# glgerard/MDBN

Measured on AMD Instinct MI355X. Metric: CD-k Gibbs steps/sec (samples/sec), GRBM 4096->1024 CD-1, higher is better.
Workload: dtype f32; 1 GPU; GRBM 4096->1024 CD-1, batch 512 per GPU, fp32, N(0,1) rows resident in HBM (BASELINE configs[1]); global_batch=512, k=1, n_data=32768, parallelism=dp1

## Files before the change

include/mdbn_hip.h:

```cpp
#ifndef MDBN_HIP_H
#define MDBN_HIP_H

#include <stddef.h>
#include <stdint.h>

#ifdef __cplusplus
extern "C" {
#endif

#define MDBN_OK       0
#define MDBN_EINVAL  (-1)
#define MDBN_EHIP    (-2)
#define MDBN_ENOSPC  (-3)

#define MDBN_VERSION 2

typedef struct mdbn_ctx mdbn_ctx;

typedef struct mdbn_rng {
    uint64_t seed;
    uint32_t stream_id;
    uint32_t step;
    uint32_t draw;
    uint32_t reserved;
    uint64_t row_offset;
} mdbn_rng;

typedef struct mdbn_cd_args {
    uint64_t     struct_size;
    const float *data;
    int64_t      n_data;
    const void  *indexes;
    int32_t      index_is_64;
    int32_t      gauss;
    int32_t      add_noise;
    int32_t      sample_stats;
    int32_t      keep_f32;
    int32_t      k;
    int64_t      B, V, H;
    int64_t      ldv, ldh;
    const float *W, *hbias, *vbias;
    float       *persistent;
    float       *V2;
    float       *P2;
    float       *hs;
    float       *vs;
    float       *stats;
    void        *workspace;
    int64_t      workspace_bytes;
    mdbn_rng     rng;
    float       *trace_h;
    float       *trace_v;
    void        *planes;
    int64_t      planes_bytes;
    void        *W_planes;
    int32_t      W_planes_valid;
    int32_t      comm_cus;
    const void  *next_indexes;
    void        *planes_alt;
    int32_t      x_buffer;
    int32_t      v0_ready;
    int32_t     *ahead_done;
} mdbn_cd_args;

typedef struct mdbn_update_args {
    uint64_t struct_size;
    float *W, *W_speed;
    const float *W0;
    float *hbias, *hbias_speed;
    float *vbias, *vbias_speed;
    int64_t V, H, ldv, ldh;
    const float *stats;
    float lr, lambda_1, lambda_2, weightcost, momentum;
    float batch_size;
    float n_rows;
    float cost_scale;
    float *cost_out;
    void *W_planes;
    int32_t phase;
    int32_t reserved;
} mdbn_update_args;

int  mdbn_version(void);
int  mdbn_last_error(char *buf, size_t n);
int  mdbn_source_hash(char *buf, size_t n);

int  mdbn_ctx_create(mdbn_ctx **out, int device);
int  mdbn_ctx_destroy(mdbn_ctx *ctx);

int  mdbn_bal_segment(int32_t tiles, int32_t stages, int32_t workgroups, int32_t w, int32_t k, int32_t *out);
int  mdbn_set_option(mdbn_ctx *ctx, const char *name, int64_t value);

int  mdbn_kernel_timing(mdbn_ctx *ctx, int enable);
int  mdbn_kernel_timing_read(mdbn_ctx *ctx, int64_t *n_launches, double *total_ms);
int  mdbn_kernel_timing_detail(mdbn_ctx *ctx, int64_t cap, double *ms, double *alg_flop,
                               double *pipe_flop, int32_t *kind, int64_t *n_launches);
int  mdbn_narrow_deep_launches(mdbn_ctx *ctx, int64_t *n_launches);

#define MDBN_MIN_WORKSPACE_BYTES 278528
int  mdbn_workspace_bytes(int64_t B, int64_t V, int64_t H, int64_t *bytes);
int  mdbn_workspace_bytes_ctx(mdbn_ctx *ctx, int64_t B, int64_t V, int64_t H, int64_t *bytes);
int  mdbn_workspace_bytes_ld(int64_t B, int64_t V, int64_t H, int64_t ldv, int64_t ldh, int64_t *bytes);
int  mdbn_workspace_bytes_ld_ctx(mdbn_ctx *ctx, int64_t B, int64_t V, int64_t H, int64_t ldv, int64_t ldh, int64_t *bytes);
int  mdbn_min_workspace_bytes(int64_t *bytes);
int  mdbn_padded_ld(int64_t cols, int64_t *ld);
int  mdbn_planes_bytes(int64_t B, int64_t ldv, int64_t ldh, int64_t *bytes);
int  mdbn_planes_alt_bytes(int64_t B, int64_t ldv, int64_t *bytes);
int  mdbn_ahead_bytes_ctx(mdbn_ctx *ctx, int64_t B, int64_t V, int64_t H, int64_t ldv, int64_t ldh, int64_t *bytes);
int  mdbn_planes_eligible(int64_t B, int64_t V, int64_t H, int64_t ldv, int64_t ldh, int32_t *eligible);
int  mdbn_planes_eligible_ctx(mdbn_ctx *ctx, int64_t B, int64_t V, int64_t H, int64_t ldv, int64_t ldh, int32_t *eligible);
int  mdbn_split_planes(mdbn_ctx *ctx, void *stream, const float *x, int64_t rows, int64_t ld, void *planes);
int  mdbn_stats_floats(int64_t V, int64_t ldv, int64_t ldh, int64_t *n);

int  mdbn_gather_rows(mdbn_ctx *ctx, void *stream, const float *src, int64_t n_rows,
                      int64_t cols, int64_t ld_src, const void *indexes, int index_is_64,
                      int64_t n_idx, float *dst, int64_t ld_dst);

int  mdbn_gather_rows_host(mdbn_ctx *ctx, void *stream, const float *src, int64_t n_rows,
                           int64_t cols, int64_t ld_src, const void *indexes, int index_is_64,
                           int64_t n_idx, float *dst, int64_t ld_dst, int workgroups, int threads);

int  mdbn_host_gather_rows(const float *table, int64_t n_rows, int64_t cols, int64_t ld,
                           const int64_t *indexes, int64_t n, float *out, int64_t ld_out, int threads);

typedef struct mdbn_feeder mdbn_feeder;
int  mdbn_feeder_create(mdbn_ctx *ctx, const float *table, int64_t n_rows, int64_t cols, int64_t ld,
                        int64_t max_rows, int slots, float *const *device_slots, int64_t ld_device,
                        int threads, mdbn_feeder **out);
int  mdbn_feeder_submit(mdbn_feeder *f, const int64_t *indexes, int64_t n, int64_t *ticket);
int  mdbn_feeder_acquire(mdbn_feeder *f, int64_t ticket, void *stream, int *slot);
int  mdbn_feeder_release(mdbn_feeder *f, int64_t ticket, void *stream);
int  mdbn_feeder_stats(mdbn_feeder *f, double *out5);
int  mdbn_feeder_cancel(mdbn_feeder *f);
int  mdbn_feeder_destroy(mdbn_feeder *f);

int  mdbn_propup_sample(mdbn_ctx *ctx, void *stream, const float *v, int64_t B, int64_t ldv,
                        const float *W, int64_t V, int64_t H, int64_t ldh, const float *hbias,
                        float *pre, float *mean, float mean_scale, float *sample,
                        const mdbn_rng *rng, void *workspace, int64_t workspace_bytes);

int  mdbn_propdown_sample(mdbn_ctx *ctx, void *stream, const float *h, int64_t B, int64_t ldh,
                          const float *W, int64_t V, int64_t H, int64_t ldv, const float *vbias,
                          int gauss, int add_noise, float *pre, float *mean, float *sample,
                          const mdbn_rng *rng, const float *v0, float *cost_sum,
                          void *workspace, int64_t workspace_bytes);

int  mdbn_comm_unique_id(char *id128);
int  mdbn_comm_init_rank(mdbn_ctx *ctx, const char *id128, int nranks, int rank);
int  mdbn_allreduce_stats(mdbn_ctx *ctx, void *stream, float *stats, int64_t n);
int  mdbn_comm_destroy(mdbn_ctx *ctx);

int  mdbn_gibbs_chain(mdbn_ctx *ctx, void *stream, float *v, int64_t B, int64_t ldv, const float *W,
                      int64_t V, int64_t H, int64_t ldh, const float *hbias, const float *vbias, int gauss,
                      int add_noise, int64_t n_steps, float *pre_h, float *h_mean, float *h_sample,
                      float *pre_v, float *v_mean, const mdbn_rng *rng, void *workspace,
                      int64_t workspace_bytes);

int  mdbn_cd_stats(mdbn_ctx *ctx, void *stream, const float *V2, const float *P2, int64_t B,
                   int64_t V, int64_t H, int64_t ldv, int64_t ldh, float *stats,
                   void *workspace, int64_t workspace_bytes);

int  mdbn_apply_update(mdbn_ctx *ctx, void *stream, const mdbn_update_args *a);

int  mdbn_cd_step(mdbn_ctx *ctx, void *stream, const mdbn_cd_args *a);

int  mdbn_cd_forward(mdbn_ctx *ctx, void *stream, const mdbn_cd_args *a);
int  mdbn_cd_statistics(mdbn_ctx *ctx, void *stream, const mdbn_cd_args *a, const mdbn_update_args *deferred);

int  mdbn_cd_train_step(mdbn_ctx *ctx, void *stream, const mdbn_cd_args *a,
                        const mdbn_update_args *upd);

int  mdbn_free_energy(mdbn_ctx *ctx, void *stream, const float *x, int64_t N, int64_t ldv,
                      const float *W, int64_t V, int64_t H, int64_t ldh, const float *hbias,
                      const float *vbias, int gauss, float *out,
                      void *workspace, int64_t workspace_bytes);

int  mdbn_ais_workspace_bytes(mdbn_ctx *ctx, int64_t M, int64_t V, int64_t H, int64_t n_betas, int path, int64_t *bytes);
int  mdbn_ais_run(mdbn_ctx *ctx, void *stream, const float *W, int64_t V, int64_t H, int64_t ldh,
                  const float *hbias, const float *vbias, const float *base_vbias, int gauss,
                  const float *betas, int64_t n_betas, int64_t M, int64_t ldv, float *v_state,
// ... 179 lines not shown
```

mdbn_amd/_lib.py:

```python
import ctypes as C
import os

HERE = os.path.dirname(os.path.abspath(__file__))
LIB_PATH = os.path.join(HERE, "libmdbn_hip.so")


class MdbnError(RuntimeError):
    pass


class Rng(C.Structure):
    _fields_ = [("seed", C.c_uint64), ("stream_id", C.c_uint32), ("step", C.c_uint32),
                ("draw", C.c_uint32), ("reserved", C.c_uint32), ("row_offset", C.c_uint64)]


class _Sized(C.Structure):

    def __init__(self, *a, **kw):
        super(_Sized, self).__init__(*a, **kw)
        self.struct_size = C.sizeof(type(self))


class CdArgs(_Sized):
    _fields_ = [("struct_size", C.c_uint64), ("data", C.c_void_p), ("n_data", C.c_int64), ("indexes", C.c_void_p),
                ("index_is_64", C.c_int32), ("gauss", C.c_int32), ("add_noise", C.c_int32),
                ("sample_stats", C.c_int32), ("keep_f32", C.c_int32), ("k", C.c_int32), ("B", C.c_int64), ("V", C.c_int64), ("H", C.c_int64),
                ("ldv", C.c_int64), ("ldh", C.c_int64),
                ("W", C.c_void_p), ("hbias", C.c_void_p), ("vbias", C.c_void_p),
                ("persistent", C.c_void_p),
                ("V2", C.c_void_p), ("P2", C.c_void_p), ("hs", C.c_void_p), ("vs", C.c_void_p),
                ("stats", C.c_void_p), ("workspace", C.c_void_p), ("workspace_bytes", C.c_int64),
                ("rng", Rng), ("trace_h", C.c_void_p), ("trace_v", C.c_void_p),
                ("planes", C.c_void_p), ("planes_bytes", C.c_int64), ("W_planes", C.c_void_p),
                ("W_planes_valid", C.c_int32), ("comm_cus", C.c_int32),
                ("next_indexes", C.c_void_p), ("planes_alt", C.c_void_p), ("x_buffer", C.c_int32),
                ("v0_ready", C.c_int32), ("ahead_done", C.POINTER(C.c_int32))]


class UpdateArgs(_Sized):
    _fields_ = [("struct_size", C.c_uint64), ("W", C.c_void_p), ("W_speed", C.c_void_p), ("W0", C.c_void_p),
                ("hbias", C.c_void_p), ("hbias_speed", C.c_void_p),
                ("vbias", C.c_void_p), ("vbias_speed", C.c_void_p),
                ("V", C.c_int64), ("H", C.c_int64), ("ldv", C.c_int64), ("ldh", C.c_int64),
                ("stats", C.c_void_p),
                ("lr", C.c_float), ("lambda_1", C.c_float), ("lambda_2", C.c_float),
                ("weightcost", C.c_float), ("momentum", C.c_float),
                ("batch_size", C.c_float), ("n_rows", C.c_float),
                ("cost_scale", C.c_float), ("cost_out", C.c_void_p), ("W_planes", C.c_void_p),
                ("phase", C.c_int32), ("reserved", C.c_int32)]


_i64, _i32, _f32, _vp = C.c_int64, C.c_int, C.c_float, C.c_void_p
_rngp = C.POINTER(Rng)

SIGNATURES = {
    "mdbn_version": [],
    "mdbn_last_error": [C.c_char_p, C.c_size_t],
    "mdbn_source_hash": [C.c_char_p, C.c_size_t],
    "mdbn_ctx_create": [C.POINTER(_vp), _i32],
    "mdbn_ctx_destroy": [_vp],
    "mdbn_set_option": [_vp, C.c_char_p, _i64],
    "mdbn_bal_segment": [_i32, _i32, _i32, _i32, _i32, C.POINTER(_i32)],
    "mdbn_kernel_timing": [_vp, _i32],
    "mdbn_kernel_timing_read": [_vp, C.POINTER(_i64), C.POINTER(C.c_double)],
    "mdbn_narrow_deep_launches": [_vp, C.POINTER(_i64)],
    "mdbn_kernel_timing_detail": [_vp, _i64, C.POINTER(C.c_double), C.POINTER(C.c_double),
                                  C.POINTER(C.c_double), C.POINTER(C.c_int32), C.POINTER(_i64)],
    "mdbn_workspace_bytes": [_i64, _i64, _i64, C.POINTER(_i64)],
    "mdbn_workspace_bytes_ctx": [_vp, _i64, _i64, _i64, C.POINTER(_i64)],
    "mdbn_workspace_bytes_ld": [_i64, _i64, _i64, _i64, _i64, C.POINTER(_i64)],
    "mdbn_workspace_bytes_ld_ctx": [_vp, _i64, _i64, _i64, _i64, _i64, C.POINTER(_i64)],
    "mdbn_min_workspace_bytes": [C.POINTER(_i64)],
    "mdbn_padded_ld": [_i64, C.POINTER(_i64)],
    "mdbn_planes_bytes": [_i64, _i64, _i64, C.POINTER(_i64)],
    "mdbn_planes_alt_bytes": [_i64, _i64, C.POINTER(_i64)],
    "mdbn_ahead_bytes_ctx": [_vp, _i64, _i64, _i64, _i64, _i64, C.POINTER(_i64)],
    "mdbn_planes_eligible": [_i64, _i64, _i64, _i64, _i64, C.POINTER(_i32)],
    "mdbn_planes_eligible_ctx": [_vp, _i64, _i64, _i64, _i64, _i64, C.POINTER(_i32)],
    "mdbn_split_planes": [_vp, _vp, _vp, _i64, _i64, _vp],
    "mdbn_stats_floats": [_i64, _i64, _i64, C.POINTER(_i64)],
    "mdbn_gather_rows": [_vp, _vp, _vp, _i64, _i64, _i64, _vp, _i32, _i64, _vp, _i64],
    "mdbn_gather_rows_host": [_vp, _vp, _vp, _i64, _i64, _i64, _vp, _i32, _i64, _vp, _i64, _i32, _i32],
    "mdbn_host_gather_rows": [_vp, _i64, _i64, _i64, _vp, _i64, _vp, _i64, _i32],
    "mdbn_feeder_create": [_vp, _vp, _i64, _i64, _i64, _i64, _i32, C.POINTER(_vp), _i64, _i32, C.POINTER(_vp)],
    "mdbn_feeder_submit": [_vp, _vp, _i64, C.POINTER(_i64)],
    "mdbn_feeder_acquire": [_vp, _i64, _vp, C.POINTER(_i32)],
    "mdbn_feeder_release": [_vp, _i64, _vp],
    "mdbn_feeder_stats": [_vp, C.POINTER(C.c_double)],
    "mdbn_feeder_cancel": [_vp],
    "mdbn_feeder_destroy": [_vp],
    "mdbn_propup_sample": [_vp, _vp, _vp, _i64, _i64, _vp, _i64, _i64, _i64, _vp,
                           _vp, _vp, _f32, _vp, _rngp, _vp, _i64],
    "mdbn_propdown_sample": [_vp, _vp, _vp, _i64, _i64, _vp, _i64, _i64, _i64, _vp, _i32, _i32,
                             _vp, _vp, _vp, _rngp, _vp, _vp, _vp, _i64],
    "mdbn_comm_unique_id": [C.c_char_p],
    "mdbn_comm_init_rank": [_vp, C.c_char_p, _i32, _i32],
    "mdbn_allreduce_stats": [_vp, _vp, _vp, _i64],
    "mdbn_comm_destroy": [_vp],
    "mdbn_gibbs_chain": [_vp, _vp, _vp, _i64, _i64, _vp, _i64, _i64, _i64, _vp, _vp, _i32, _i32, _i64,
                         _vp, _vp, _vp, _vp, _vp, _rngp, _vp, _i64],
    "mdbn_cd_stats": [_vp, _vp, _vp, _vp, _i64, _i64, _i64, _i64, _i64, _vp, _vp, _i64],
    "mdbn_apply_update": [_vp, _vp, C.POINTER(UpdateArgs)],
    "mdbn_cd_step": [_vp, _vp, C.POINTER(CdArgs)],
    "mdbn_cd_forward": [_vp, _vp, C.POINTER(CdArgs)],
    "mdbn_cd_statistics": [_vp, _vp, C.POINTER(CdArgs), C.POINTER(UpdateArgs)],
    "mdbn_cd_train_step": [_vp, _vp, C.POINTER(CdArgs), C.POINTER(UpdateArgs)],
    "mdbn_free_energy": [_vp, _vp, _vp, _i64, _i64, _vp, _i64, _i64, _i64, _vp, _vp, _i32, _vp,
                         _vp, _i64],
    "mdbn_ais_workspace_bytes": [_vp, _i64, _i64, _i64, _i64, _i32, C.POINTER(_i64)],
    "mdbn_ais_run": [_vp, _vp, _vp, _i64, _i64, _i64, _vp, _vp, _vp, _i32, _vp, _i64, _i64, _i64, _vp,
                     _vp, _vp, _vp, _i32, _rngp, _vp, _i64],
    "mdbn_ais_run_grouped": [_vp, _vp, _vp, _i64, _i64, _i64, _vp, _vp, _vp, _i32, _vp, _i64, _i64, _i64, _vp,
                             _vp, _vp, _vp, _i32, _rngp, _vp, _i64, _vp, _vp, _i64],
    "mdbn_ais_cond_workspace_bytes": [_vp, _i64, _i64, _i64, _i64, _i64, _i32, C.POINTER(_i64)],
    "mdbn_ais_cond_run": [_vp, _vp, _vp, _i64, _i64, _i64, _vp, _vp, _vp, _i32, _vp, _i64, _vp, _vp, _i64, _i64, _i64, _i64,
                          _vp, _vp, _vp, _vp, _i32, _rngp, _vp, _i64],
    "mdbn_ais_cond_run_grouped": [_vp, _vp, _vp, _i64, _i64, _i64, _vp, _vp, _vp, _vp, _i64, _vp, _vp, _i64, _i64, _i64, _i64,
                                  _vp, _vp, _vp, _vp, _i32, _rngp, _vp, _i64, _vp, _vp, _i64],
    "mdbn_gibbs_clamped_workspace_bytes": [_vp, _i64, _i64, _i64, _i32, C.POINTER(_i64)],
    "mdbn_gibbs_clamped": [_vp, _vp, _vp, _vp, _vp, _i64, _i64, _i64, _vp, _i64, _i64, _i64, _vp, _vp, _i32, _i32, _i64,
                           _i64, _vp, _vp, _vp, _vp, _vp, _vp, _vp, _i32, _i64, _rngp, _vp, _i64],
    "mdbn_gibbs_clamped_grouped": [_vp, _vp, _vp, _vp, _vp, _i64, _i64, _i64, _vp, _i64, _i64, _i64, _vp, _vp, _i64,
                                   _i64, _vp, _vp, _vp, _vp, _vp, _vp, _vp, _i32, _i64, _rngp, _vp, _i64, _vp, _vp, _i64],
    "mdbn_pt_workspace_bytes": [_vp, _i64, _i64, _i64, _i64, _i32, C.POINTER(_i64)],
    "mdbn_pt_run": [_vp, _vp, _vp, _i64, _i64, _i64, _vp, _vp, _vp, _i32, _vp, _i64, _i64, _i64, _vp, _vp, _vp,
                    _i64, _i64, _i64, _vp, _vp, _vp, _vp, _vp, _vp, _i32, _i64, _rngp, _vp, _i64],
    "mdbn_pt_run_z_workspace_bytes": [_vp, _i64, _i64, _i64, _i64, _i32, C.POINTER(_i64)],
    "mdbn_pt_run_z": [_vp, _vp, _vp, _i64, _i64, _i64, _vp, _vp, _vp, _i32, _vp, _i64, _i64, _i64, _vp, _vp, _vp,
                      _i64, _i64, _i64, _vp, _vp, _vp, _vp, _vp, _vp, _i32, _i64, _rngp, _vp, _i64, _vp, _vp],
    "mdbn_pt_run_grouped": [_vp, _vp, _vp, _i64, _i64, _i64, _vp, _vp, _vp, _i32, _vp, _i64, _i64, _i64, _vp, _vp, _vp,
                            _i64, _i64, _i64, _vp, _vp, _vp, _vp, _vp, _vp, _i32, _i64, _rngp, _vp, _i64, _vp, _vp,
                            _vp, _vp, _i64],
    "mdbn_rowll_workspace_bytes": [_vp, _i64, _i64, _i64, C.POINTER(_i64)],
    "mdbn_propdown_rowll": [_vp, _vp, _vp, _i64, _i64, _vp, _i64, _i64, _vp, _vp, _i64, _i64, _i32, _vp, _vp, _i64],
    "mdbn_rowll_grouped_workspace_bytes": [_vp, _i64, _i64, _i64, C.POINTER(_i64)],
    "mdbn_propdown_rowll_grouped": [_vp, _vp, _vp, _i64, _i64, _vp, _i64, _i64, _vp, _vp, _i64, _i64, _vp, _vp, _i64,
                                    _vp, _vp, _i64],
    "mdbn_sample_replicas": [_vp, _vp, _vp, _i64, _i64, _i64, _i64, _vp, _vp, _rngp],
    "mdbn_center_workspace_bytes": [_vp, _i64, _i64, C.POINTER(_i64)],
    "mdbn_center_offsets": [_vp, _vp, _vp, _i64, _vp, _i64, _i64, _i64, _i64, _f32, _vp, _vp],
    "mdbn_center_stats": [_vp, _vp, _vp, _i64, _i64, _i64, _i64, _vp, _vp, _f32, _vp, _i64],
    "mdbn_sparsity_activity": [_vp, _vp, _vp, _i64, _vp, _i64, _i64, _i64, _i64, _f32, _vp, _vp],
    "mdbn_sparsity_stats": [_vp, _vp, _vp, _i64, _i64, _i64, _i64, _vp, _vp, _f32, _f32, _f32],
    "mdbn_sigma_workspace_bytes": [_vp, _i64, _i64, C.POINTER(_i64)],
    "mdbn_sigma_scale_rows": [_vp, _vp, _vp, _i64, _i64, _vp, _i32, _i64, _i64, _vp, _f32, _vp, _i64],
    "mdbn_sigma_update": [_vp, _vp, _vp, _i64, _vp, _i64, _i64, _i64, _i64, _f32, _f32, _f32, _f32, _vp, _vp, _vp, _i64],
    "mdbn_group_softmax_workspace_bytes": [_vp, _i64, _i64, C.POINTER(_i64)],
    "mdbn_group_softmax_sample": [_vp, _vp, _vp, _i64, _i64, _i64, _vp, _vp, _i64, _vp, _vp, _vp, _rngp, _vp, _vp, _vp, _i64],
# ... 85 lines not shown
```

mdbn_amd/csrc/mdbn_capi.hip:

```cpp
#include <hip/hip_runtime.h>
#include <algorithm>
#include <cstdint>
#include <initializer_list>
#include <cstdarg>
#include <cstdio>
#include <cstdlib>
#include <cstring>
#include <string>
#include <utility>
#include <vector>
#include "mdbn_capi_internal.h"
#include "mdbn_kernels.h"
#include "mdbn_small.h"
#include "mdbn_thin.h"
#include "mdbn_gchain.h"

using namespace mdbn;
using namespace mdbn::capi;

static const Options g_default_options;
static GemmTiming g_no_timing;
static thread_local const Options* t_opt = &g_default_options;
static thread_local GemmTiming* t_timing = &g_no_timing;
#define g_timing (*t_timing)
// ... 26 lines not shown
#define g_opt_fused_finalize (t_opt->fused_finalize)
#define kMinSplitK (t_opt->min_splitk)

struct Plan {
    int tiles_m, tiles_n, splitk, kchunk, bn, bk;
    int skinny = 0;
    int mi = 1;
    int ni = 1;
    int cw = 1;
    int x6 = 0;
    int64_t slab_floats(int64_t M, int64_t ldc) const { return (int64_t)splitk * M * ldc; }
    void fill(GemmArgs& g) const
    {
        g.kchunk = kchunk; g.splitk = splitk; g.tiles_m = tiles_m; g.tiles_n = tiles_n; g.bn = bn; g.bk = bk;
        g.inner_m = tiles_m <= tiles_n;
        g.skinny = skinny; g.mi = mi; g.ni = ni; g.fused = 0; g.cw = cw; g.fin_enabled = 0; g.x6 = x6; g.x6_pw = g_opt_x6_pw;
    }
};

Plan plan_gemm(int64_t M, int64_t N, int64_t K)
{
    Plan p;
    p.tiles_m = (int)((M + 127) / 128);
    const int64_t t128 = (int64_t)p.tiles_m * ((N + 127) / 128);
    p.bn = (t128 * std::max<int64_t>(1, K / kMinSplitK) >= kTargetJobs) ? 128 : 64;
    p.tiles_n = (int)((N + p.bn - 1) / p.bn);
    const int64_t tiles = (int64_t)p.tiles_m * p.tiles_n;
    int64_t want = std::max<int64_t>(1, kTargetJobs / std::max<int64_t>(tiles, 1));
    int64_t maxsplit = std::max<int64_t>(1, K / kMinSplitK);
    int64_t sk = std::min(want, maxsplit);
    p.bk = (p.bn == 128 && g_opt_gemm_bk != 32 && (K + sk - 1) / sk >= 128) ? 64 : 32;
    int64_t kchunk = ((K + sk - 1) / sk + p.bk - 1) / p.bk * p.bk;
    if (kchunk < p.bk) kchunk = p.bk;
    sk = std::max<int64_t>(1, (K + kchunk - 1) / kchunk);
    p.splitk = (int)sk;
    p.kchunk = (int)kchunk;
    p.cw = g_opt_gemm_cw ? g_opt_gemm_cw : (p.bn == 128 && p.kchunk / p.bk <= 8 ? 2 : 1);
    return p;
}

#define g_opt_skinny_gemm (t_opt->skinny_gemm)
constexpr int kSkinnyTargetBlocks = 512;
constexpr int kSkinnyMinK = 256;
#define g_opt_skinny_fused_max_k (t_opt->skinny_fused_max_k)
#define g_opt_skinny_max_macs (t_opt->skinny_max_macs)

Plan plan_skinny(int64_t M, int64_t K, int64_t ldo, bool allow_split)
{
    Plan p;
    p.skinny = 1;
    p.mi = M <= 32 ? 1 : 2;
    p.tiles_m = (int)((M + 32 * p.mi - 1) / (32 * p.mi));
    p.tiles_n = (int)((ldo + 31) / 32);
    p.bn = 32; p.bk = 8;
    const int64_t blocks = (int64_t)p.tiles_m * p.tiles_n;
    const int64_t want = std::max<int64_t>(1, kSkinnyTargetBlocks / blocks);
    const bool one_launch = !allow_split || (K <= g_opt_skinny_fused_max_k && K <= 64 * blocks);
    const int64_t sk = one_launch ? 1 : std::min(want, std::max<int64_t>(1, K / kSkinnyMinK));
    int64_t kchunk = ((K + sk - 1) / sk + 63) / 64 * 64;
    p.kchunk = (int)kchunk;
    p.splitk = (int)std::max<int64_t>(1, (K + kchunk - 1) / kchunk);
    return p;
}

bool prefer_skinny(int64_t M, int64_t N, int64_t K)
{
    if (!g_opt_skinny_gemm) return false;
    if (M <= 64) return true;
    if (K > g_opt_skinny_fused_max_k) return false;
    const int64_t tiles_m = (M + 63) / 64, strips = (N + 31) / 32;
    if (K > 64 * tiles_m * strips) return false;
    return M * N * K <= (K <= 512 ? 3 : 1) * g_opt_skinny_max_macs;
}


#define g_opt_gemm_bf16x6 (t_opt->gemm_bf16x6)
#define g_opt_small_fused (t_opt->small_fused)
#define g_opt_thin_fused (t_opt->thin_fused)
#define g_opt_gchain (t_opt->gchain)
#define g_opt_gemm_planes (t_opt->gemm_planes)
#define g_opt_planes_mfma (t_opt->planes_mfma)
#define g_opt_early_w (t_opt->early_w)
#define g_opt_narrow_tiles (t_opt->narrow_tiles)
#define g_opt_slab_tail (t_opt->slab_tail)
#define g_opt_narrow_deep (t_opt->narrow_deep)
#define g_opt_feed_copy_streams (t_opt->feed_copy_streams)
#define g_opt_gather_ahead (t_opt->gather_ahead)
#define g_opt_bf16_inputs (t_opt->bf16_inputs)
#define g_opt_planes_min_work (t_opt->planes_min_work)
#define g_opt_comm_cus (t_opt->comm_cus)
#define g_opt_bal_blocks (t_opt->bal_blocks)
constexpr int kMaxBalBlocks = 256;

bool try_bf16x6(Plan& p, int64_t M, int64_t N, int64_t K, bool unsplit = false)
{
    if (p.skinny || K < 64) return false;
    const int64_t tm = (M + 127) / 128, tn = (N + 127) / 128, tiles = tm * tn;
    int64_t sk = 1;
    if (!unsplit) {
        sk = std::min(std::max<int64_t>(1, kTargetJobs / tiles), std::max<int64_t>(1, K / kMinSplitK));
    } else if (p.splitk != 1) {
        return false;
    }
    if (tiles * sk < g_opt_x6_min_jobs) return false;
    int64_t kchunk = ((K + sk - 1) / sk + 31) / 32 * 32;
    sk = (K + kchunk - 1) / kchunk;
    p.x6 = 1;
    p.bn = 128; p.bk = 32; p.cw = 1;
    p.tiles_m = (int)tm; p.tiles_n = (int)tn;
    p.splitk = (int)sk; p.kchunk = (int)kchunk;
    return true;
}

#define g_opt_stream_x6 (t_opt->stream_x6)
#define g_opt_stream_max_macs (t_opt->stream_max_macs)
#define g_opt_stream_mi (t_opt->stream_mi)
#define g_opt_stream_ni (t_opt->stream_ni)
constexpr int64_t kStreamMinTiles = 192;

bool stream_ok(int64_t M, int64_t N, int64_t K)
{
    return g_opt_stream_x6 && M > 64 && K >= 64 && M * N * K <= g_opt_stream_max_macs;
}

Plan plan_stream(int64_t M, int64_t K, int64_t ldo)
{
    Plan p = plan_skinny(M, K, ldo, false);
    const int64_t tiles32 = ((M + 31) / 32) * ((ldo + 31) / 32);
    p.mi = tiles32 >= 2 * kStreamMinTiles ? 2 : 1;
    p.ni = tiles32 >= 4 * kStreamMinTiles ? 2 : 1;
    if (g_opt_stream_mi) p.mi = g_opt_stream_mi;
    if (g_opt_stream_ni) p.ni = g_opt_stream_ni;
    if (p.ni == 2) p.mi = 2;
    p.tiles_m = (int)((M + 32 * p.mi - 1) / (32 * p.mi));
    p.x6 = 1;
    return p;
}

Plan plan_forward(int64_t M, int64_t N, int64_t K, int64_t ldo, bool stream = true)
{
    if (prefer_skinny(M, N, K)) {
        if (stream && g_opt_stream_x6 >= 2 && stream_ok(M, N, K)) return plan_stream(M, K, ldo);
        return plan_skinny(M, K, ldo, M <= 64);
    }
    if (stream && stream_ok(M, N, K)) return plan_stream(M, K, ldo);
    Plan p = plan_gemm(M, N, K);
    if (g_opt_gemm_bf16x6 & 2) try_bf16x6(p, M, N, K);
    return p;
}

Plan plan_stats(int64_t V, int64_t H, int64_t K2, int64_t ldh, bool stream = true)
{
    if (prefer_skinny(V, H, K2) && V > 64) {
        if (stream && g_opt_stream_x6 >= 2 && stream_ok(V, H, K2)) return plan_stream(V, K2, ldh);
        return plan_skinny(V, K2, ldh, false);
    }
    if (stream && stream_ok(V, H, K2)) return plan_stream(V, K2, ldh);
    Plan p = plan_gemm(V, H, K2);
    if (g_opt_gemm_bf16x6 & 1) try_bf16x6(p, V, H, K2, p.splitk == 1);
    return p;
}

static unsigned long long* g_stamps = nullptr;

template <class Launch>
hipError_t timed_launch(const GemmTiming::Meta& m, hipStream_t s, Launch launch)
// ... 46 lines not shown

static WsSizes ws_sizes_dense(int64_t B, int64_t V, int64_t H)
{
    const int64_t ldv = padded_ld(V), ldh = padded_ld(H);
    WsSizes s;
    const Plan up = plan_gemm(B, H, V), down = plan_gemm(B, V, H), st = plan_gemm(V, H, 2 * B);
    s.slab = std::max(up.slab_floats(B, ldh), down.slab_floats(B, ldv));
    {
        const Plan ups = plan_forward(B, H, V, ldh), downs = plan_forward(B, V, H, ldv);
        s.slab = std::max(s.slab, std::max(ups.slab_floats(B, ldh), downs.slab_floats(B, ldv)));
    }
    if (st.splitk > 1) s.slab = std::max(s.slab, st.slab_floats(V, ldh));
    {
        const Plan st2 = plan_stats(V, H, 2 * B, ldh);
        if (st2.splitk > 1) s.slab = std::max(s.slab, st2.slab_floats(V, ldh));
    }
    if (B % 128 == 0 && V % 128 == 0 && H % 128 == 0) {
        const int64_t tu = (B / 128) * (H / 128), td = (B / 128) * (V / 128);
        s.slab = std::max(s.slab, (kMaxBalBlocks / tu + 2) * B * ldh);
        s.slab = std::max(s.slab, (kMaxBalBlocks / td + 2) * B * ldv);
        s.slab = std::max<int64_t>(s.slab, (int64_t)kMaxBalBlocks * 2 * 16384);
    }
    if (small_shape_ok(B, V, H, 0) || small_shape_ok(B, V, H, 1))
        s.slab = std::max<int64_t>(s.slab, (int64_t)small_blocks(B) * ((V + 63) & ~int64_t(63)) * ldh);
    int64_t thin_cost = 0;
    {
        ThinGeom tg;
        if (thin_geom(B, V, H, ldv, ldh, kTargetJobs, tg)) {
            s.slab = std::max<int64_t>(s.slab, (int64_t)tg.G * tg.Bq * ldh);
            thin_cost = tg.G;
        }
    }
    int64_t gc_cost = 0;
    {
        GChainGeom gg;
        if (gchain_geom(B, V, H, ldv, ldh, 0, kTargetJobs, gg)) {
            s.slab = std::max<int64_t>(s.slab, gg.xbuf_floats);
            gc_cost = (int64_t)gg.nslab * gg.g;
        }
    }
    s.slab = std::max<int64_t>(s.slab, 4 * std::max(ldv, ldh) * 8);
    s.cost = cost_floats_for(B, std::max(ldv, ldh));
    if (small_shape_ok(B, V, H, 0) || small_shape_ok(B, V, H, 1)) s.cost = std::max<int64_t>(s.cost, (int64_t)small_blocks(B) * SM_NW + 64);
    s.cost = std::max<int64_t>(s.cost, thin_cost + 64);
    s.cost = std::max<int64_t>(s.cost, gc_cost + 64);
    const int ng = row_groups(B);
    s.colP = 2 * (int64_t)ng * ldh;
    s.colV = (int64_t)ng * ldv;
    return s;
}

WsSizes ws_sizes(int64_t B, int64_t V, int64_t H, int64_t ldv = 0, int64_t ldh = 0)
{
    WsSizes s = ws_sizes_dense(B, V, H);
    if (H % 128 != 0) {
        const WsSizes p = ws_sizes_dense(B, V, (H + 127) & ~int64_t(127));
        s.slab = std::max(s.slab, p.slab); s.cost = std::max(s.cost, p.cost);
        s.colP = std::max(s.colP, p.colP); s.colV = std::max(s.colV, p.colV);
    }
    const int64_t ng = row_groups(B);
    if (ldh > 0) {
        s.colP = std::max(s.colP, 2 * ng * ldh);
        const Plan st = plan_stats(V, H, 2 * B, ldh);
        if (st.splitk > 1) s.slab = std::max(s.slab, st.slab_floats(V, ldh));
    }
    if (ldv > 0) s.colV = std::max(s.colV, ng * ldv);
    if (ldv > 0 || ldh > 0) s.cost = std::max(s.cost, cost_floats_for(B, std::max(ldv, ldh)));
    return s;
}

hipError_t timed_gemm_planes(int la, int lb, const PlaneGemmArgs& g_in, hipStream_t s)
{
    PlaneGemmArgs g = g_in;
    g.stamps = g_stamps;
    g.ms = g_opt_planes_mfma;
    if (g_opt_bf16_inputs) g.ap = 0;
    g.slab_tail = g.slab_tail && g.ms == 16 && g.ap != 0;
    if (g.slab_tail && !slab_tail_ok(g, la, lb)) return hipErrorInvalidValue;
    const int pipe = g.ap == 3 ? 1 : (g.ap == 1 ? 2 : 3);
    return timed_launch(gemm_meta((g.bal ? 3000 : 2000) + 100 * pipe + 10 * g.fused + 2 * la + lb, pipe, g.M, g.N, g.K), s,
                        [&]() { return g.bal ? launch_gemm_planes_bal(la, lb, g, s) : launch_gemm_planes(la, lb, g, s); });
}

struct PlaneStep {
    unsigned short *Xp, *Pp, *hsp, *vsp;
    int64_t px, pp;
    unsigned short *Xother = nullptr, *Wp = nullptr;
    bool keep = false;
};
inline int64_t planes_elems(int64_t B, int64_t ldv, int64_t ldh) { return 6 * B * ldv + 6 * B * ldh + B * ldh + B * ldv; }

bool plane_plan(const Plan& p, int64_t M, int64_t N, int64_t K)
{
    return p.x6 && !p.skinny && M % 128 == 0 && N % 128 == 0 && p.kchunk % 32 == 0 && (int64_t)p.kchunk * p.splitk == K;
}

bool plane_shape_ok(int64_t B, int64_t V, int64_t H, int64_t ldv, int64_t ldh)
{
    if (!g_opt_gemm_planes) return false;
    if (B <= 0 || B % 128 || V % 128 || ldh % 128 || ldv != V || H > ldh || ldh - H >= 128 || B > 65535) return false;
    const int64_t He = ldh;
    if (g_opt_planes_min_work > 0 && (B * V * He < g_opt_planes_min_work || V * He < ((int64_t)1 << 21))) return false;
    return plane_plan(plan_forward(B, He, V, He, false), B, He, V) && plane_plan(plan_forward(B, V, He, V, false), B, V, He) &&
           plane_plan(plan_stats(V, He, 2 * B, He, false), V, He, 2 * B);
}

bool planes_eligible(const mdbn_cd_args* a)
{
    if (!a->planes || !a->W_planes) return false;
    if (a->persistent || a->sample_stats || (a->gauss && a->add_noise)) return false;
    const int64_t B = a->B, V = a->V, H = a->H;
    if (!plane_shape_ok(B, V, H, a->ldv, a->ldh)) return false;
    return a->planes_bytes >= 2 * planes_elems(B, a->ldv, a->ldh) && aligned16(a->planes) && aligned16(a->W_planes);
}

int bal_blocks(const mdbn_ctx* ctx, int comm_cus, int64_t tiles, int64_t stages)
{
    if (comm_cus <= 0) comm_cus = g_opt_comm_cus;
    if ((comm_cus <= 0 && g_opt_bal_blocks <= 0) || g_opt_planes_mfma != 16) return 0;
    int P = g_opt_bal_blocks > 0 ? g_opt_bal_blocks : std::min(ctx->num_cu - comm_cus, kMaxBalBlocks);
    if (P < 1) return 0;
    if (tiles < P && P % tiles != 0 && g_opt_bal_blocks <= 0) {
        const int aligned = (int)(tiles * (P / tiles));
        if (4ll * P <= 5ll * aligned) P = aligned;
    }
    return tiles * stages >= 4 * (int64_t)P ? P : 0;
}

int run_affine_planes(mdbn_ctx* ctx, int comm_cus, const unsigned short* A, int64_t lda, int64_t pa, int ap, int dir,
                      const unsigned short* Wp, int64_t V, int64_t H, int64_t ncols, int64_t rows, EpiArgs e, bool want_cost,
                      const Workspace& ws, hipStream_t s, int* n_cost_out)
{
    const int64_t Kdim = dir == 0 ? V : H, Ndim = dir == 0 ? H : V;
    PlaneGemmArgs g{};
    g.A = A; g.lda = lda; g.pa = pa; g.ap = ap;
    g.B = Wp; g.ldb = H; g.pb = V * H;
    g.M = (int)rows; g.N = (int)Ndim; g.K = (int)Kdim;
    g.tiles_m = (int)(rows / 128); g.tiles_n = (int)(Ndim / 128);
    {
        const Plan p = plan_forward(rows, Ndim, Kdim, e.ld, false);
        g.splitk = p.splitk; g.kchunk = p.kchunk;
    }
    int bal = bal_blocks(ctx, comm_cus, (int64_t)g.tiles_m * g.tiles_n, Kdim / 32), bal_slabs = 0;
    if (bal) {
        bal_slabs = bal_max_segments(g.tiles_m * g.tiles_n, (int)(Kdim / 32), bal);
        if ((int64_t)bal_slabs * rows * e.ld > ws.slab_floats) bal = 0;
        if ((int64_t)bal_slabs * rows * e.ld * 4 >= (int64_t)1 << 31) bal = 0;
    }
    if (!bal && g_opt_narrow_tiles && g_opt_fused_epilogue && dir == 1 && g.splitk == 2 && Ndim % 64 == 0 && g_opt_planes_mfma == 16 &&
        !g_opt_bf16_inputs && (ap == 1 || ap == 3) && (int64_t)g.tiles_m * (Ndim / 64) <= 2 * ctx->num_cu &&
        (!e.target || (e.ld_target % 4 == 0 && ((uintptr_t)e.target & 15) == 0))) {
        g.bn = 64; g.tiles_n = (int)(Ndim / 64); g.splitk = 1; g.kchunk = (int)Kdim;
        g.fused = 1; g.ms = 16;
        g.deep = g_opt_narrow_deep && narrow_deep_ok(g, LAY_K, LAY_K);
        if (g.deep) ++ctx->narrow_deep_launches;
    }
    const bool fuse = !bal && g_opt_fused_epilogue && g.splitk == 1;
    const int nb = fuse ? g.tiles_m * g.tiles_n : epilogue_blocks(rows, e.ld);
    e.rows = (int)rows; e.cols = (int)ncols;
    e.cost_partials = nullptr;
    if (want_cost) {
        if (nb > ws.cost_floats) return fail(MDBN_ENOSPC, "cost scratch exhausted");
        e.cost_partials = ws.cost_partials;
        if (n_cost_out) *n_cost_out = nb;
    }
    const int lb = dir == 0 ? LAY_MN : LAY_K;
    if (bal) {
        g.bal = bal; g.fused = 0; g.C = ws.slabs; g.ldc = e.ld; g.slab_stride = rows * e.ld;
        g.xcd_group = bal >= 4 * g.tiles_m * g.tiles_n ? 0 : 1;
        g.splitk = 1; g.kchunk = (int)Kdim; g.c_bytes = (int64_t)bal_slabs * rows * e.ld * 4;
        e.slabs = ws.slabs; e.slab_stride = g.slab_stride; e.nsplit = bal_slabs;
        e.bal_P = bal; e.bal_S = (int)(Kdim / 32); e.bal_tiles_m = g.tiles_m; e.bal_tiles_n = g.tiles_n;
        {
            const int tiles = g.tiles_m * g.tiles_n;
            bool uniform = true;
            for (int t = 0; t < tiles && uniform; ++t) uniform = bal_tile_slabs(t, tiles, e.bal_S, bal) == bal_slabs;
            if (uniform) e.bal_P = 0;
        }
        HIP_OK(timed_gemm_planes(LAY_K, lb, g, s));
        HIP_OK(launch_act_epilogue(e, s));
    } else if (fuse) {
        g.fused = 1; g.epi = e;
        HIP_OK(timed_gemm_planes(LAY_K, lb, g, s));
    } else {
        REQUIRE((int64_t)g.splitk * rows * e.ld <= ws.slab_floats, "internal: plane GEMM slabs exceed the workspace");
        g.fused = 0; g.C = ws.slabs; g.ldc = e.ld; g.slab_stride = rows * e.ld;
        e.slabs = ws.slabs; e.slab_stride = g.slab_stride; e.nsplit = g.splitk;
        g.slab_tail = g_opt_slab_tail && dir == 0;
        HIP_OK(timed_gemm_planes(LAY_K, lb, g, s));
        HIP_OK(launch_act_epilogue(e, s));
    }
    return MDBN_OK;
}

enum class StepPart { Whole, Forward, Statistics };

struct StatsView {
    float *S, *s_h, *s_v, *cost;
    StatsView(float* stats, int64_t V, int64_t ldv, int64_t ldh) : S(stats), s_h(S + V * ldh), s_v(s_h + ldh), cost(s_v + ldv) {}
};

bool plain_cd(const mdbn_cd_args* a) { return !a->persistent && !a->sample_stats && !(a->gauss && a->add_noise); }
bool keeps_f32(const mdbn_cd_args* a) { return a->keep_f32 != 0 || a->trace_h != nullptr || a->trace_v != nullptr; }

hipError_t launch_whole_update(const mdbn_update_args& u, hipStream_t s)
{
    return launch_update(u, s, nullptr, 1, 0, reinterpret_cast<unsigned short*>(u.W_planes));
}
mdbn_update_args whole_rule(const mdbn_update_args& u) { mdbn_update_args w = u; w.phase = 0; return w; }

int planes_setup(const mdbn_cd_args* a, PlaneStep& pb)
{
    const int64_t B = a->B, ldv = a->V, ldh = a->ldh;
    unsigned short* q = reinterpret_cast<unsigned short*>(a->planes);
    pb.Xp = q; pb.px = 2 * B * ldv; q += 6 * B * ldv;
    pb.Pp = q; pb.pp = 2 * B * ldh; q += 6 * B * ldh;
    pb.hsp = q; q += B * ldh;
    pb.vsp = q;
    if (a->planes_alt) {
        REQUIRE(aligned16(a->planes_alt), "planes_alt not 16-byte aligned");
        unsigned short* alt = reinterpret_cast<unsigned short*>(a->planes_alt);
        if (a->x_buffer) { pb.Xother = pb.Xp; pb.Xp = alt; } else pb.Xother = alt;
    } else {
        REQUIRE(a->x_buffer == 0, "x_buffer = 1 needs planes_alt");
    }
    pb.Wp = reinterpret_cast<unsigned short*>(a->W_planes);
    pb.keep = keeps_f32(a);
    return MDBN_OK;
}

int planes_forward(mdbn_ctx* ctx, hipStream_t s, const mdbn_cd_args* a, const Workspace& ws, const PlaneStep& pb, int* n_cost)
{
    const int64_t B = a->B, V = a->V, Hlive = a->H, ldv = V, ldh = a->ldh;
    const int64_t H = ldh;
    unsigned short* const Wp = pb.Wp;  const bool keep = pb.keep;
    float *v0 = a->V2, *nv = a->V2 + B * ldv, *ph = a->P2, *nh = a->P2 + B * ldh;
    if (!(a->v0_ready && !keep))
        HIP_OK(launch_gather_planes(a->data, a->n_data, ldv, ldv, a->indexes, a->index_is_64, B, keep ? v0 : nullptr, ldv, pb.Xp,
                                    pb.px, s));

    auto key = [&](uint32_t draw) { PhiloxKey k = make_key(a->rng, draw); return k; };
    {
        EpiArgs e{};
        e.ld = ldh; e.bias = a->hbias; e.mean = keep ? ph : nullptr; e.sample = keep ? a->hs : nullptr; e.mean_scale = 1.0f; e.gauss = 0;
        e.colsum = ws.colPpos; e.colsum_kind = 0; e.rng = key(0);
        e.mean_planes = pb.Pp; e.plane_stride = pb.pp; e.sample_plane = pb.hsp;
        CHECK(run_affine_planes(ctx, a->comm_cus, pb.Xp, ldv, pb.px, 3, 0, Wp, V, H, Hlive, B, e, false, ws, s, nullptr));
        if (a->trace_h) HIP_OK(hipMemcpyAsync(a->trace_h, a->hs, sizeof(float) * B * ldh, hipMemcpyDeviceToDevice, s));
    }
    for (int t = 1; t <= a->k; ++t) {
        const bool last = t == a->k;
        {
            EpiArgs e{};
            e.ld = ldv; e.bias = a->vbias; e.mean = keep ? nv : nullptr; e.mean_scale = 1.0f; e.gauss = a->gauss;
            e.sample = (a->gauss || !keep) ? nullptr : a->vs; e.rng = key((uint32_t)(2 * t - 1));
            e.mean_planes = pb.Xp + B * ldv; e.plane_stride = pb.px;
            e.sample_plane = a->gauss ? nullptr : pb.vsp;
            if (last) {
                e.colsum = ws.colV; e.colsum_kind = 1;
                if (keep) { e.target = v0; e.ld_target = ldv; }
                else {
                    e.target = a->data; e.ld_target = ldv; e.target_rows = a->n_data;
                    e.target_idx = a->indexes; e.target_idx64 = a->index_is_64;
                }
            }
            CHECK(run_affine_planes(ctx, a->comm_cus, pb.hsp, ldh, B * ldh, 1, 1, Wp, V, H, V, B, e, last, ws, s, last ? n_cost : nullptr));
            if (a->trace_v && !a->gauss)
                HIP_OK(hipMemcpyAsync(a->trace_v + (int64_t)(t - 1) * B * ldv, a->vs, sizeof(float) * B * ldv,
                                      hipMemcpyDeviceToDevice, s));
        }
        {
            const bool need_sample = !last;
            EpiArgs e{};
            e.ld = ldh; e.bias = a->hbias; e.mean = keep ? nh : nullptr; e.mean_scale = -1.0f; e.gauss = 0;
            e.sample = (need_sample && keep) ? a->hs : nullptr; e.rng = key((uint32_t)(2 * t));
            e.mean_planes = pb.Pp + B * ldh; e.plane_stride = pb.pp;
            e.sample_plane = need_sample ? pb.hsp : nullptr;
            if (last) { e.colsum = ws.colPneg; e.colsum_kind = 0; }
            if (a->gauss) CHECK(run_affine_planes(ctx, a->comm_cus, pb.Xp + B * ldv, ldv, pb.px, 3, 0, Wp, V, H, Hlive, B, e, false, ws, s, nullptr));
            else CHECK(run_affine_planes(ctx, a->comm_cus, pb.vsp, ldv, B * ldv, 1, 0, Wp, V, H, Hlive, B, e, false, ws, s, nullptr));
            if (a->trace_h && need_sample)
                HIP_OK(hipMemcpyAsync(a->trace_h + (int64_t)t * B * ldh, a->hs, sizeof(float) * B * ldh, hipMemcpyDeviceToDevice, s));
        }
    }
    return MDBN_OK;
}

int planes_statistics(mdbn_ctx* ctx, hipStream_t s, const mdbn_cd_args* a, const Workspace& ws, const PlaneStep& pb, int n_cost,
                      const mdbn_update_args* upd, const mdbn_update_args* defer)
{
    const int64_t B = a->B, V = a->V, Hlive = a->H, ldv = V, ldh = a->ldh, H = ldh;
    const StatsView st(a->stats, V, ldv, ldh);
    const Plan sp = plan_stats(V, H, 2 * B, ldh, false);
    PlaneGemmArgs g{};
    g.A = pb.Xp; g.lda = ldv; g.pa = pb.px; g.ap = 3;
    g.B = pb.Pp; g.ldb = ldh; g.pb = pb.pp;
    g.M = (int)V; g.N = (int)H; g.K = (int)(2 * B);
    g.tiles_m = (int)(V / 128); g.tiles_n = (int)(H / 128); g.splitk = sp.splitk; g.kchunk = sp.kchunk;
    g.fin_enabled = 0;
    int bal = sp.splitk == 1 ? bal_blocks(ctx, a->comm_cus, (int64_t)g.tiles_m * g.tiles_n, 2 * B / 32) : 0;
    if (bal && ((int64_t)bal * 2 * 16384 > ws.slab_floats || V * ldh * 4 >= (int64_t)1 << 31)) bal = 0;
    const bool fuse_upd = !bal && upd != nullptr && g_opt_fused_update && sp.splitk == 1;
    auto set_gather_ahead = [&]() {
        if (g.upd.early && g_opt_gather_ahead && a->next_indexes && pb.Xother && !pb.keep) {
            const int nwg = g.tiles_m * g.tiles_n, nt = (int)(2 * B / 32);
            const int rpw = (int)((B + nwg - 1) / nwg), passes = (int)((ldv / 8 + 255) / 256);
            if (rpw * passes <= 4 && 16 / (nt >= 20 ? 1 : 2) + 4 + 1 <= nt - 3) {
                g.ga.src = a->data; g.ga.n_rows = a->n_data; g.ga.ld_src = ldv;
                g.ga.idx = a->next_indexes; g.ga.idx64 = a->index_is_64;
                g.ga.B = (int)B; g.ga.rpw = rpw; g.ga.passes = passes;
                g.ga.P = pb.Xother; g.ga.plane_stride = pb.px; g.ga.ld = ldv;
                if (a->ahead_done) *a->ahead_done = 1;
            }
        }
    };
    if (fuse_upd) {
        BiasUpd bu;
        fill_bias_upd(bu, *upd, Hlive);
        g.fused = 2;
        g.fin_enabled = 1;
        g.fin = make_fin_args(ws.colPpos, ws.colPneg, ws.colV, row_groups(B), ldh, ldv, ws.cost_partials, n_cost, st.s_h, st.s_v,
                              st.cost, &bu);
        fill_upd(g.upd, *upd, V, ldh, pb.Wp);
        g.upd.early = g_opt_early_w && upd->lambda_1 == 0.f && (upd->weightcost == 0.f || upd->W0 != nullptr) &&
                      2 * B / 32 >= 12 && g_opt_planes_mfma == 16 && !g_opt_bf16_inputs;
        g.stats_tail = g_opt_slab_tail && g.upd.early == 1 && ldh < ((int64_t)1 << 21);
        set_gather_ahead();
        HIP_OK(timed_gemm_planes(LAY_MN, LAY_MN, g, s));
        return MDBN_OK;
    }
    if (sp.splitk == 1 && g_opt_fused_finalize) {
        g.fin_enabled = 1;
        g.fin = make_fin_args(ws.colPpos, ws.colPneg, ws.colV, row_groups(B), ldh, ldv, ws.cost_partials, n_cost, st.s_h, st.s_v,
                              st.cost, nullptr);
    } else {
        HIP_OK(launch_finalize_stats(ws.colPpos, ws.colPneg, ws.colV, row_groups(B), ldh, ldv, ws.cost_partials, n_cost, st.s_h,
                                     st.s_v, st.cost, nullptr, s));
    }
    g.fused = 0; g.ldc = ldh; g.slab_stride = V * ldh;
    if (defer) {
        const bool splitphase = g_opt_early_w && g_opt_planes_mfma == 16 && !g_opt_bf16_inputs && defer->phase == 3 &&
                                defer->lambda_1 == 0.f && (defer->weightcost == 0.f || defer->W0 != nullptr) &&
                                defer->stats != a->stats;
        const int64_t flat = bal ? (((V * ldh / 4 + bal - 1) / bal + 511) / 512) * 512 : 0;
        const bool inside = splitphase && (bal ? (flat <= 16 * 512 && (int64_t)g.tiles_m * g.tiles_n * (2 * B / 32) / bal >= 20)
                                               : (sp.splitk == 1 && 2 * B / 32 >= 20));
        g.upd.flat_per_wg = flat;
        if (inside) {
            fill_upd(g.upd, *defer, V, ldh, reinterpret_cast<unsigned short*>(defer->W_planes));
            g.upd.l1 = 0.f; g.upd.Sprev = defer->stats; g.upd.early = 2;
            const StatsView prev(const_cast<float*>(defer->stats), V, ldv, ldh);
            DeferredBias& d = g.db;
            d.on = 1; d.hb = defer->hbias; d.hbs = defer->hbias_speed; d.vb = defer->vbias; d.vbs = defer->vbias_speed;
            d.s_h = prev.s_h; d.s_v = prev.s_v; d.cost_sum = prev.cost; d.H = Hlive; d.V = V;
            d.lr = defer->lr; d.mu = defer->momentum; d.inv_rows = 1.0f / defer->n_rows;
            d.cost_scale = defer->cost_scale; d.cost_out = defer->cost_out;
            if (!bal) set_gather_ahead();
        } else {
            HIP_OK(launch_whole_update(*defer, s));
        }
    }
    if (bal) {
        g.xcd_group = 1;
        g.C = st.S; g.bal = bal; g.fused = 4; g.kchunk = (int)(2 * B); g.c_bytes = V * ldh * 4;
        g.scratch = ws.slabs;
        HIP_OK(timed_gemm_planes(LAY_MN, LAY_MN, g, s));
    } else if (sp.splitk == 1) {
        g.C = st.S;
        HIP_OK(timed_gemm_planes(LAY_MN, LAY_MN, g, s));
    } else {
        REQUIRE(sp.slab_floats(V, ldh) <= ws.slab_floats, "internal: statistic slabs exceed workspace");
        g.C = ws.slabs;
        HIP_OK(timed_gemm_planes(LAY_MN, LAY_MN, g, s));
        if (upd && g_opt_fused_update) {
            HIP_OK(launch_update(whole_rule(*upd), s, ws.slabs, sp.splitk, g.slab_stride, pb.Wp));
            return MDBN_OK;
        }
        HIP_OK(launch_sum_slabs(ws.slabs, sp.splitk, g.slab_stride, V * ldh, st.S, s));
    }
    if (upd) HIP_OK(launch_update(whole_rule(*upd), s, nullptr, 1, 0, pb.Wp));
    return MDBN_OK;
}

}

namespace mdbn {
namespace capi {

int fail(int code, const char* fmt, ...)
{
    char buf[512];
    va_list ap;
    va_start(ap, fmt);
    vsnprintf(buf, sizeof buf, fmt, ap);
    va_end(ap);
    g_err = buf;
    return code;
}

PhiloxKey make_key(const mdbn_rng& r, uint32_t draw)
{
    PhiloxKey k;
    k.k0 = (uint32_t)r.seed;
    k.k1 = (uint32_t)(r.seed >> 32) ^ r.stream_id;
    k.step = r.step;
    k.draw = draw;
    k.row_offset = r.row_offset;
    return k;
}

int64_t dense_workspace_bytes(int64_t B, int64_t V, int64_t H) { return ws_sizes(B, V, H).total_bytes(); }

constexpr int64_t kPropCostFloats = 1 << 16;
constexpr int64_t kPropMinBytes = 4 * (kPropCostFloats + 4096);
static_assert(kPropMinBytes == MDBN_MIN_WORKSPACE_BYTES, "mdbn_hip.h states the minimum of the propagation calls");

int carve(void* ws, int64_t bytes, int64_t B, int64_t V, int64_t H, Workspace& out, bool need_stats, int64_t ldv, int64_t ldh)
{
    REQUIRE(ws != nullptr && aligned16(ws), "workspace must be a 16-byte aligned device pointer");
    const WsSizes s = ws_sizes(B, V, H, ldv, ldh);
// ... 105 lines not shown
    e.mu = u.momentum; e.inv_bs = 1.0f / u.batch_size;
    e.Wp = Wp; e.wp_stride = V * ldh;
}

void fill_bias_upd(BiasUpd& b, const mdbn_update_args& u, int64_t H)
{
    b.hb = u.hbias; b.hbs = u.hbias_speed; b.vb = u.vbias; b.vbs = u.vbias_speed;
    b.H = H; b.V = u.V; b.lr = u.lr; b.mu = u.momentum; b.inv_rows = 1.0f / u.n_rows;
    b.cost_scale = u.cost_scale; b.cost_out = u.cost_out;
}

}
}

extern "C" {

int mdbn_version(void) { return MDBN_VERSION; }

#ifndef MDBN_SRC_HASH
#define MDBN_SRC_HASH "unknown"
#endif
static const char mdbn_source_hash_tag[] __attribute__((used)) = "MDBN_SOURCE_HASH_TAG=" MDBN_SRC_HASH;
int mdbn_source_hash(char* buf, size_t n)
{
    if (!buf || n == 0) return MDBN_EINVAL;
    snprintf(buf, n, "%s", mdbn_source_hash_tag + sizeof("MDBN_SOURCE_HASH_TAG=") - 1);
    return MDBN_OK;
}

int mdbn_last_error(char* buf, size_t n)
{
    if (!buf || n == 0) return MDBN_EINVAL;
    snprintf(buf, n, "%s", g_err.c_str());
    return MDBN_OK;
}

int mdbn_ctx_create(mdbn_ctx** out, int device)
{
    REQUIRE(out != nullptr, "out is NULL");
    int count = 0;
    HIP_OK(hipGetDeviceCount(&count));
    REQUIRE(device >= 0 && device < count, "device %d out of range (%d visible)", device, count);
    hipDeviceProp_t prop;
    HIP_OK(hipGetDeviceProperties(&prop, device));
    if (strncmp(prop.gcnArchName, "gfx950", 6) != 0)
        return fail(MDBN_EHIP, "device %d is %s; this library is built for gfx950 only", device, prop.gcnArchName);
    mdbn_ctx* c = new mdbn_ctx;
    c->device = device;
    c->num_cu = prop.multiProcessorCount;
    if (const char* e = getenv("MDBN_NARROW_DEEP")) c->opt.narrow_deep = atoi(e) != 0;
    *out = c;
    return MDBN_OK;
}

int mdbn_ctx_destroy(mdbn_ctx* ctx)
{
    CtxScope ctx_scope(ctx);
    if (ctx) {
        if (ctx->ev_fork) (void)hipEventDestroy(ctx->ev_fork);
        if (ctx->ev_join) (void)hipEventDestroy(ctx->ev_join);
        if (ctx->side) (void)hipStreamDestroy(ctx->side);
        if (ctx->comm) (void)mdbn_comm_destroy(ctx);
        if (ctx->gc_flags) (void)hipFree(ctx->gc_flags);
    }
    delete ctx;
    return MDBN_OK;
}

#ifdef MDBN_STAMP
int mdbn_debug_set_stamps(void* p) { g_stamps = (unsigned long long*)p; return MDBN_OK; }
#endif

int mdbn_bal_segment(int32_t tiles, int32_t stages, int32_t workgroups, int32_t w, int32_t k, int32_t* out)
{
    REQUIRE(out != nullptr, "out is NULL");
    int tile, s0, s1, nseg, nt;
    if (bal_segment_host(tiles, stages, workgroups, w, k, &tile, &s0, &s1, &nseg, &nt) != 0)
        return fail(MDBN_EINVAL, "bad arguments");
    out[0] = tile; out[1] = s0; out[2] = s1; out[3] = nseg; out[4] = nt;
    out[5] = tile >= 0 ? bal_tile_slabs(tile, tiles, stages, workgroups) : 0;
    return MDBN_OK;
}

static bool set_plane_kernel_option(mdbn_ctx* ctx, const char* name, int64_t value)
{
    if (strcmp(name, "slab_tail") == 0) {
        ctx->opt.slab_tail = value != 0;
        return true;
    }
    return false;
}

int mdbn_set_option(mdbn_ctx* ctx, const char* name, int64_t value)
{
    CtxScope ctx_scope(ctx);
    REQUIRE(ctx != nullptr && name != nullptr, "NULL argument");
    if (set_plane_kernel_option(ctx, name, value)) return MDBN_OK;
    if (strcmp(name, "gemm_bk") == 0) {
        REQUIRE(value == 0 || value == 32 || value == 64, "gemm_bk must be 0 (auto), 32 or 64");
        ctx->opt.gemm_bk = (int)value;
        return MDBN_OK;
    }
    if (strcmp(name, "epilogue_threads") == 0) {
        if (value != 0 && value != 64 && value != 128 && value != 256) return fail(MDBN_EINVAL, "epilogue_threads must be 0, 64, 128 or 256");
        ctx->opt.epilogue_threads = (int)value;
        return MDBN_OK;
    }
    if (strcmp(name, "epilogue_cw") == 0) {
        REQUIRE(value == 0 || value == 1 || value == 2 || value == 4, "epilogue_cw must be 0 (auto), 1, 2 or 4");
        ctx->opt.epilogue_cw = (int)value;
        return MDBN_OK;
    }
    if (strcmp(name, "skinny_gemm") == 0) {
        ctx->opt.skinny_gemm = value != 0;
        return MDBN_OK;
    }
    if (strcmp(name, "thin_fused") == 0) {
        ctx->opt.thin_fused = value != 0;
        return MDBN_OK;
    }
    if (strcmp(name, "gchain") == 0) {
        ctx->opt.gchain = value != 0;
        return MDBN_OK;
    }
    if (strcmp(name, "skinny_fused_max_k") == 0) {
        REQUIRE(value >= 0 && value <= INT32_MAX, "skinny_fused_max_k must be in [0, 2^31)");
        ctx->opt.skinny_fused_max_k = (int)value;
        return MDBN_OK;
    }
    if (strcmp(name, "x6_min_jobs") == 0) {
        REQUIRE(value >= 0 && value <= INT32_MAX, "x6_min_jobs must be in [0, 2^31)");
        ctx->opt.x6_min_jobs = (int)value;
        return MDBN_OK;
    }
    if (strcmp(name, "x6_producer_waves") == 0) {
        if (value != 2 && value != 4) return fail(MDBN_EINVAL, "x6_producer_waves must be 2 or 4");
        ctx->opt.x6_pw = (int)value;
        return MDBN_OK;
    }
    if (strcmp(name, "gemm_min_splitk") == 0) {
        if (value < 32 || value > INT32_MAX) return fail(MDBN_EINVAL, "gemm_min_splitk must be in [32, 2^31)");
        ctx->opt.min_splitk = (int)value;
        return MDBN_OK;
    }
    if (strcmp(name, "gemm_cw") == 0) {
        if (value < 0 || value > 2) return fail(MDBN_EINVAL, "gemm_cw must be 0 (auto), 1 or 2");
        ctx->opt.gemm_cw = (int)value;
        return MDBN_OK;
    }
    if (strcmp(name, "stream_x6") == 0) {
        REQUIRE(value == 0 || value == 1 || value == 2, "stream_x6 must be 0, 1 or 2");
        ctx->opt.stream_x6 = (int)value;
        return MDBN_OK;
    }
    if (strcmp(name, "stream_max_macs") == 0) {
        REQUIRE(value >= 0, "stream_max_macs must be >= 0");
        ctx->opt.stream_max_macs = value;
        return MDBN_OK;
    }
    if (strcmp(name, "stream_mi") == 0) {
        REQUIRE(value == 0 || value == 1 || value == 2, "stream_mi must be 0, 1 or 2");
        ctx->opt.stream_mi = (int)value;
        return MDBN_OK;
    }
    if (strcmp(name, "stream_ni") == 0) {
        REQUIRE(value == 0 || value == 1 || value == 2, "stream_ni must be 0, 1 or 2");
        ctx->opt.stream_ni = (int)value;
        return MDBN_OK;
    }
    if (strcmp(name, "skinny_max_macs") == 0) {
        REQUIRE(value >= 0 && value < ((int64_t)1 << 61), "skinny_max_macs must be in [0, 2^61)");
        ctx->opt.skinny_max_macs = value;
        return MDBN_OK;
    }
    if (strcmp(name, "gemm_bf16x6") == 0) {
        REQUIRE(value >= 0 && value <= 3, "gemm_bf16x6 must be in 0..3 (bit 0 statistics, bit 1 forward passes)");
        ctx->opt.gemm_bf16x6 = (int)value;
        return MDBN_OK;
    }
    if (strcmp(name, "planes_min_work") == 0) {
// ... 2 lines not shown
        return MDBN_OK;
    }
    if (strcmp(name, "bf16_inputs") == 0) {
        ctx->opt.bf16_inputs = value != 0;
        return MDBN_OK;
    }
    if (strcmp(name, "planes_mfma") == 0) {
        if (value != 16 && value != 32) return fail(MDBN_EINVAL, "planes_mfma must be 16 or 32");
        ctx->opt.planes_mfma = (int)value;
        return MDBN_OK;
    }
    if (strcmp(name, "narrow_tiles") == 0) {
        ctx->opt.narrow_tiles = value != 0;
        return MDBN_OK;
    }
    if (strcmp(name, "feed_copy_streams") == 0) {
        REQUIRE(value == 1 || value == 2, "feed_copy_streams must be 1 or 2");
        ctx->opt.feed_copy_streams = value;
        return MDBN_OK;
    }
    if (strcmp(name, "gather_ahead") == 0) {
        ctx->opt.gather_ahead = value != 0;
        return MDBN_OK;
    }
    if (strcmp(name, "early_w") == 0) {
        ctx->opt.early_w = value != 0;
        return MDBN_OK;
    }
    if (strcmp(name, "bal_blocks") == 0) {
        if (value < 0 || value > kMaxBalBlocks) return fail(MDBN_EINVAL, "bal_blocks must be in [0, %d]", kMaxBalBlocks);
        ctx->opt.bal_blocks = (int)value;
        return MDBN_OK;
    }
    if (strcmp(name, "comm_cus") == 0) {
        if (value < 0 || value > 192) return fail(MDBN_EINVAL, "comm_cus must be in [0, 192]");
        ctx->opt.comm_cus = (int)value;
        return MDBN_OK;
    }
    if (strcmp(name, "small_fin_lanes") == 0) {
        REQUIRE(value == 0 || value == 1 || value == 2 || value == 4 || value == 8 || value == 16, "small_fin_lanes must be 0, 1, 2, 4, 8 or 16");
        ctx->opt.small_fin_lanes = (int)value;
        return MDBN_OK;
    }
    if (strcmp(name, "small_fused") == 0) {
        ctx->opt.small_fused = value != 0;
        return MDBN_OK;
    }
    if (strcmp(name, "gemm_planes") == 0) {
        ctx->opt.gemm_planes = value != 0;
        return MDBN_OK;
    }
    if (strcmp(name, "fused_finalize") == 0) {
        ctx->opt.fused_finalize = value != 0;
        return MDBN_OK;
    }
    if (strcmp(name, "fused_update") == 0) {
        ctx->opt.fused_update = value != 0;
        return MDBN_OK;
    }
    if (strcmp(name, "fused_epilogue") == 0) {
        ctx->opt.fused_epilogue = value != 0;
        return MDBN_OK;
    }
    if (strcmp(name, "update_overlap") == 0) {
        ctx->opt.update_overlap = value != 0;
        return MDBN_OK;
    }
    return fail(MDBN_EINVAL, "unknown option %s", name);
}

int mdbn_kernel_timing(mdbn_ctx* ctx, int enable)
{
    CtxScope ctx_scope(ctx);
    REQUIRE(ctx != nullptr, "ctx is NULL");
    g_timing.enabled = enable != 0;
    g_timing.used = 0;
    return MDBN_OK;
}

int mdbn_narrow_deep_launches(mdbn_ctx* ctx, int64_t* n_launches)
{
    REQUIRE(ctx && n_launches, "NULL argument");
    *n_launches = ctx->narrow_deep_launches;
    return MDBN_OK;
}

int mdbn_kernel_timing_read(mdbn_ctx* ctx, int64_t* n_launches, double* total_ms)
{
    CtxScope ctx_scope(ctx);
    REQUIRE(ctx && n_launches && total_ms, "NULL argument");
    double tot = 0.0;
    for (size_t i = 0; i < g_timing.used; ++i) {
        HIP_OK(hipEventSynchronize(g_timing.pool[i].second));
        float ms = 0.f;
        HIP_OK(hipEventElapsedTime(&ms, g_timing.pool[i].first, g_timing.pool[i].second));
        tot += ms;
    }
    *n_launches = (int64_t)g_timing.used;
    *total_ms = tot;
    return MDBN_OK;
}

int mdbn_kernel_timing_detail(mdbn_ctx* ctx, int64_t cap, double* ms, double* alg_flop, double* pipe_flop,
                              int32_t* kind, int64_t* n_launches)
{
    CtxScope ctx_scope(ctx);
    REQUIRE(ctx && n_launches && (cap == 0 || (ms && alg_flop && pipe_flop && kind)), "NULL argument");
    const int64_t n = std::min<int64_t>(cap, (int64_t)g_timing.used);
    for (int64_t i = 0; i < n; ++i) {
        HIP_OK(hipEventSynchronize(g_timing.pool[i].second));
        float t = 0.f;
        HIP_OK(hipEventElapsedTime(&t, g_timing.pool[i].first, g_timing.pool[i].second));
        ms[i] = t;
        alg_flop[i] = g_timing.meta[i].alg_flop;
        pipe_flop[i] = g_timing.meta[i].pipe_flop;
        kind[i] = g_timing.meta[i].kind;
    }
    *n_launches = (int64_t)g_timing.used;
    return MDBN_OK;
}

int mdbn_workspace_bytes(int64_t B, int64_t V, int64_t H, int64_t* bytes)
{
    REQUIRE(bytes != nullptr && B > 0 && V > 0 && H > 0, "bad arguments");
    *bytes = std::max(ws_sizes(B, V, H).total_bytes(), kPropMinBytes);
    return MDBN_OK;
}

int mdbn_workspace_bytes_ld(int64_t B, int64_t V, int64_t H, int64_t ldv, int64_t ldh, int64_t* bytes)
{
    REQUIRE(bytes != nullptr && B > 0 && V > 0 && H > 0, "bad arguments");
    REQUIRE(ldv >= V && ldh >= H && ldv % 4 == 0 && ldh % 4 == 0, "leading dims must be multiples of 4, >= V / H");
    *bytes = std::max(ws_sizes(B, V, H, ldv, ldh).total_bytes(), kPropMinBytes);
    return MDBN_OK;
}

int mdbn_min_workspace_bytes(int64_t* bytes)
{
    REQUIRE(bytes != nullptr, "bytes is NULL");
    *bytes = kPropMinBytes;
    return MDBN_OK;
}

int mdbn_workspace_bytes_ld_ctx(mdbn_ctx* ctx, int64_t B, int64_t V, int64_t H, int64_t ldv, int64_t ldh, int64_t* bytes)
{
    CtxScope ctx_scope(ctx);
    REQUIRE(ctx != nullptr, "ctx is NULL");
    return mdbn_workspace_bytes_ld(B, V, H, ldv, ldh, bytes);
}

int mdbn_workspace_bytes_ctx(mdbn_ctx* ctx, int64_t B, int64_t V, int64_t H, int64_t* bytes)
{
    CtxScope ctx_scope(ctx);
    REQUIRE(ctx != nullptr, "ctx is NULL");
    return mdbn_workspace_bytes(B, V, H, bytes);
}

int mdbn_padded_ld(int64_t cols, int64_t* ld)
{
    REQUIRE(ld != nullptr && cols > 0, "bad arguments");
    *ld = padded_ld(cols);
    return MDBN_OK;
}

int mdbn_planes_bytes(int64_t B, int64_t ldv, int64_t ldh, int64_t* bytes)
{
// ... 495 lines not shown
    const bool fuse_upd = upd && !overlap && g_opt_fused_update && p.splitk == 1;
    BiasUpd bu;
    if (fuse_upd) fill_bias_upd(bu, u, H);
    const bool fin_in_gemm = !overlap && g_opt_fused_finalize;
    if (!overlap && !fin_in_gemm)
        HIP_OK(launch_finalize_stats(ws.colPpos, ws.colPneg, ws.colV, row_groups(B), ldh, ldv, ws.cost_partials,
                                     n_cost, st.s_h, st.s_v, st.cost, fuse_upd ? &bu : nullptr, s));
    GemmArgs g{};
    g.A = a->V2; g.lda = ldv; g.B = a->P2; g.ldb = ldh;
    g.ldc = ldh; g.slab_stride = V * ldh;
    g.M = (int)V; g.N = (int)H; g.K = (int)(2 * B); g.Nst = (int)ldh;
    p.fill(g);
    g.fin_enabled = fin_in_gemm;
    if (fin_in_gemm)
        g.fin = make_fin_args(ws.colPpos, ws.colPneg, ws.colV, row_groups(B), ldh, ldv, ws.cost_partials, n_cost,
                              st.s_h, st.s_v, st.cost, fuse_upd ? &bu : nullptr);
    if (fuse_upd) {
        g.C = nullptr;
        g.fused = 2;
        fill_upd(g.upd, u, V, ldh, reinterpret_cast<unsigned short*>(u.W_planes));
        HIP_OK(timed_gemm(LAY_MN, LAY_MN, g, s));
        return MDBN_OK;
    }
    if (p.splitk == 1) {
        g.C = st.S;
        HIP_OK(timed_gemm(LAY_MN, LAY_MN, g, s));
    } else {
        REQUIRE(p.slab_floats(V, ldh) <= ws.slab_floats, "internal: statistic slabs exceed workspace");
        g.C = ws.slabs;
        HIP_OK(timed_gemm(LAY_MN, LAY_MN, g, s));
        if (upd && !overlap && g_opt_fused_update) {
            HIP_OK(launch_update(whole_rule(u), s, ws.slabs, p.splitk, g.slab_stride, reinterpret_cast<unsigned short*>(u.W_planes)));
            return MDBN_OK;
        }
        HIP_OK(launch_sum_slabs(ws.slabs, p.splitk, g.slab_stride, V * ldh, st.S, s));
    }
    if (upd && !overlap) HIP_OK(launch_whole_update(whole_rule(u), s));
    if (overlap) {
        HIP_OK(hipStreamWaitEvent(s, ctx->ev_join, 0));
        u.phase = 1;
        HIP_OK(launch_update(u, s, nullptr, 1, 0, nullptr));
    }
    return MDBN_OK;
}

enum class StepPath { OneLaunch, Thin, Planes, GroupChain, Dense };

static int cd_step_impl(mdbn_ctx* ctx, void* stream, const mdbn_cd_args* a, const mdbn_update_args* upd, StepPart part,
                        const mdbn_update_args* defer)
{
    REQUIRE(ctx != nullptr && a != nullptr, "NULL argument");
    REQUIRE(a->struct_size == sizeof(mdbn_cd_args),
            "mdbn_cd_args.struct_size is %llu, this library's struct has %llu bytes (built against another mdbn_hip.h?)",
            (unsigned long long)a->struct_size, (unsigned long long)sizeof(mdbn_cd_args));
    const int64_t B = a->B, V = a->V, H = a->H, ldv = a->ldv, ldh = a->ldh;
    REQUIRE(B > 0 && V > 0 && H > 0 && a->k >= 1, "bad shape / k");
    REQUIRE(a->comm_cus >= 0 && a->comm_cus <= 192, "comm_cus must be in [0, 192]");
    REQUIRE(ldv >= V && ldh >= H && ldv % 4 == 0 && ldh % 4 == 0, "leading dims must be multiples of 4, >= V / H");
    CHECK(check_mat(a->data, ldv, V, "data"));
    CHECK(check_mat(a->W, ldh, H, "W"));
    CHECK(check_mat(a->V2, ldv, V, "V2"));
    CHECK(check_mat(a->P2, ldh, H, "P2"));
    CHECK(check_mat(a->hs, ldh, H, "hs"));
    REQUIRE(a->hbias && a->vbias, "bias pointers are NULL");
    REQUIRE(a->stats != nullptr && aligned16(a->stats), "stats not aligned");
    REQUIRE(a->gauss || a->vs != nullptr, "Bernoulli RBM needs the vs buffer");
    REQUIRE(!(a->sample_stats && a->gauss && a->add_noise), "sample statistics of a noisy GRBM are not supported");
    REQUIRE(a->vs == nullptr || aligned16(a->vs), "vs not aligned");
    REQUIRE(a->persistent == nullptr || aligned16(a->persistent), "persistent not aligned");
    REQUIRE(a->indexes != nullptr || B <= a->n_data, "identity minibatch longer than data");
    Workspace ws;
    CHECK(carve(a->workspace, a->workspace_bytes, B, V, H, ws, true, ldv, ldh));
    hipStream_t s = (hipStream_t)stream;
    if (a->ahead_done) *a->ahead_done = 0;
    if (upd) {
        REQUIRE(upd->stats == a->stats && upd->W == a->W && upd->ldh == ldh && upd->ldv == ldv && upd->V == V && upd->H == H,
                "update arguments do not match the step's buffers");
        REQUIRE(upd->W_planes == nullptr || upd->W_planes == a->W_planes, "update and step disagree about W_planes");
    }
    if (a->W_planes && !a->W_planes_valid) {
        REQUIRE(aligned16(a->W_planes), "W_planes not 16-byte aligned");
        HIP_OK(launch_split_planes(a->W, V, ldh, reinterpret_cast<unsigned short*>(a->W_planes), V * ldh, s));
    }
    int n_cost = 0;
    if (part == StepPart::Statistics) {
        REQUIRE(ctx->pending_stats == a->stats && ctx->pending_n_cost >= 0, "mdbn_cd_statistics must follow mdbn_cd_forward of the same step");
        n_cost = ctx->pending_n_cost;
    }
    ctx->pending_n_cost = -1; ctx->pending_stats = nullptr;
    if (defer) {
        REQUIRE(upd == nullptr && part != StepPart::Forward, "a deferred update goes with the statistics half of a step without its own update");
        REQUIRE(defer->W == a->W && defer->ldh == ldh && defer->ldv == ldv && defer->V == V && defer->H == H,
                "deferred update does not match the step's parameters");
    }
    const bool overlap_upd = upd && g_opt_update_overlap;
    StepPath path = StepPath::Dense;
    ThinStep thin;  PlaneStep planes;  GChainGeom gg;
    if (!overlap_upd && small_eligible(a, ws)) path = StepPath::OneLaunch;
    else if (!overlap_upd && thin_eligible(ctx, a, ws, thin.tg)) { path = StepPath::Thin; CHECK(thin_setup(a, thin)); }
    else if (!overlap_upd && planes_eligible(a)) { path = StepPath::Planes; CHECK(planes_setup(a, planes)); }
    else if (gchain_eligible(ctx, a, ws, gg)) path = StepPath::GroupChain;

    if (part != StepPart::Statistics) {
        switch (path) {
        case StepPath::OneLaunch:  CHECK(small_forward(s, a, ws, &n_cost)); break;
        case StepPath::Thin:       CHECK(thin_forward(s, a, ws, thin, &n_cost)); break;
        case StepPath::Planes:     CHECK(planes_forward(ctx, s, a, ws, planes, &n_cost)); break;
        case StepPath::GroupChain: CHECK(gchain_forward(ctx, s, a, ws, gg, &n_cost)); break;
        case StepPath::Dense:      CHECK(dense_forward(s, a, ws, &n_cost)); break;
        }
    }
    if (part == StepPart::Forward) {
        ctx->pending_n_cost = n_cost; ctx->pending_stats = a->stats;
        return MDBN_OK;
    }
    if (defer && path != StepPath::Planes) HIP_OK(launch_whole_update(*defer, s));
    switch (path) {
    case StepPath::OneLaunch:  return small_statistics(s, a, ws, n_cost, upd);
    case StepPath::Thin:       return thin_statistics(s, a, ws, thin, n_cost, upd);
    case StepPath::Planes:     return planes_statistics(ctx, s, a, ws, planes, n_cost, upd, defer);
    case StepPath::GroupChain:
    case StepPath::Dense:      break;
    }
    return dense_statistics(ctx, s, a, ws, n_cost, upd);
}

int mdbn_cd_step(mdbn_ctx* ctx, void* stream, const mdbn_cd_args* a)
{
    CtxScope ctx_scope(ctx);
    return cd_step_impl(ctx, stream, a, nullptr, StepPart::Whole, nullptr);
}

int mdbn_cd_forward(mdbn_ctx* ctx, void* stream, const mdbn_cd_args* a)
{
    CtxScope ctx_scope(ctx);
    return cd_step_impl(ctx, stream, a, nullptr, StepPart::Forward, nullptr);
}

int mdbn_cd_statistics(mdbn_ctx* ctx, void* stream, const mdbn_cd_args* a, const mdbn_update_args* deferred)
{
    CtxScope ctx_scope(ctx);
    if (deferred) {
        CHECK(check_update_args(deferred));
        REQUIRE(deferred->phase == 3 || deferred->phase == 0, "a deferred update is phase 3 (or the whole rule, phase 0)");
    }
    return cd_step_impl(ctx, stream, a, nullptr, StepPart::Statistics, deferred);
}

int mdbn_cd_train_step(mdbn_ctx* ctx, void* stream, const mdbn_cd_args* a, const mdbn_update_args* upd)
{
    CtxScope ctx_scope(ctx);
    REQUIRE(upd != nullptr, "update arguments are NULL");
    CHECK(check_update_args(upd));
    return cd_step_impl(ctx, stream, a, upd, StepPart::Whole, nullptr);
}

int mdbn_free_energy(mdbn_ctx* ctx, void* stream, const float* x, int64_t N, int64_t ldv, const float* W,
                     int64_t V, int64_t H, int64_t ldh, const float* hbias, const float* vbias, int gauss,
                     float* out, void* workspace, int64_t workspace_bytes)
{
    CtxScope ctx_scope(ctx);
    REQUIRE(ctx != nullptr, "ctx is NULL");
    REQUIRE(N > 0 && V > 0 && H > 0, "bad shape");
    CHECK(check_mat(x, ldv, V, "x"));
    CHECK(check_mat(W, ldh, H, "W"));
    REQUIRE(hbias && vbias && out, "NULL pointer");
    Workspace ws;
    CHECK(carve(workspace, workspace_bytes, N, V, H, ws, false));
    hipStream_t s = (hipStream_t)stream;
    int64_t r0 = 0;
    while (r0 < N) {
        int64_t R = N - r0;
        Plan p = plan_gemm(R, H, V);
        while (p.slab_floats(R, ldh) > ws.slab_floats) {
            if (R <= 4) return fail(MDBN_ENOSPC, "workspace cannot hold one 4-row slab");
            R = std::max<int64_t>(4, (R / 2 + 3) & ~int64_t(3));
            p = plan_gemm(R, H, V);
        }
        GemmArgs g{};
        g.A = x + r0 * ldv; g.lda = ldv; g.B = W; g.ldb = ldh; g.C = ws.slabs; g.ldc = ldh;
        g.slab_stride = R * ldh;
        g.M = (int)R; g.N = (int)H; g.K = (int)V; g.Nst = (int)ldh;
        p.fill(g);
        g.fused = 0;
        HIP_OK(timed_gemm(LAY_K, LAY_MN, g, s));
        HIP_OK(launch_free_energy(ws.slabs, p.splitk, g.slab_stride, ldh, (int)H, hbias, x + r0 * ldv, ldv,
                                  (int)V, vbias, gauss, R, out + r0, s));
        r0 += R;
    }
    return MDBN_OK;
}

int mdbn_round_flip(mdbn_ctx* ctx, void* stream, const float* x, int64_t rows, int64_t cols, int64_t ld, int64_t flip_col,
                    float* out)
{
    CtxScope ctx_scope(ctx);
    REQUIRE(ctx && x && out && rows >= 0 && cols > 0 && ld >= cols && flip_col < cols, "bad arguments");
    HIP_OK(launch_round_flip(x, out, rows, cols, ld, flip_col, (hipStream_t)stream));
    return MDBN_OK;
}

int mdbn_pl_cost(mdbn_ctx* ctx, void* stream, const float* fe, const float* fe_flip, int64_t rows, int64_t n_visible,
                 float* cost_out)
// ... 74 lines not shown
```

mdbn_amd/csrc/mdbn_capi_internal.h:

```cpp
#pragma once
#include <hip/hip_runtime.h>
#include <cstdint>
#include <utility>
#include <vector>
#include "mdbn_kernels.h"

namespace mdbn {
struct UpdownGeom;

namespace capi {

struct Options {
    int gemm_bk = 0;
    int x6_min_jobs = 48;
    int x6_pw = 4;
    int gemm_cw = 0;
    int update_overlap = 0;
    int fused_epilogue = 1;
    int fused_update = 1;
    int fused_finalize = 1;
    int skinny_gemm = 1;
    int skinny_fused_max_k = 1024;
    int64_t skinny_max_macs = 32ll << 20;
    int stream_x6 = 2;
    int64_t stream_max_macs = (int64_t)1 << 30;
    int stream_mi = 0;
    int stream_ni = 0;
    int gemm_bf16x6 = 3;
    int small_fused = 1;
    int thin_fused = 1;
    int gchain = 0;
    int gemm_planes = 1;
    int planes_mfma = 16;
    int early_w = 1;
    int narrow_tiles = 1;
    int slab_tail = 1;
    int narrow_deep = 1;
    int feed_copy_streams = 1;
    int gather_ahead = 1;
    int bf16_inputs = 0;
    int64_t planes_min_work = (int64_t)1 << 30;
    int comm_cus = 0;
    int bal_blocks = 0;
    int min_splitk = 128;
    int epilogue_cw = 0;
    int epilogue_threads = 0;
    int small_fin_lanes = 0;
};

struct GemmTiming {
    bool enabled = false;
    std::vector<std::pair<hipEvent_t, hipEvent_t>> pool;
    struct Meta { int kind; double alg_flop, pipe_flop; };
    std::vector<Meta> meta;
    size_t used = 0;
};

}
}

struct mdbn_ctx {
    int device;
    int num_cu;
    mdbn::capi::Options opt;
    mdbn::capi::GemmTiming timing;
    int64_t narrow_deep_launches = 0;
    int pending_n_cost = -1;
    const void* pending_stats = nullptr;
    void* comm = nullptr;
    int comm_ranks = 0;
    hipStream_t side = nullptr;
    hipEvent_t ev_fork = nullptr, ev_join = nullptr;
    unsigned* gc_flags = nullptr;
    unsigned gc_seq = 1;
};

namespace mdbn {
namespace capi {

struct CtxScope {
    const Options* prev_opt; GemmTiming* prev_timing;
    explicit CtxScope(mdbn_ctx* c);
    ~CtxScope();
    CtxScope(const CtxScope&) = delete;
    CtxScope& operator=(const CtxScope&) = delete;
};

int fail(int code, const char* fmt, ...) __attribute__((format(printf, 2, 3)));

#define HIP_OK(expr)                                                                    \
    do {                                                                                \
        hipError_t _e = (expr);                                                         \
        if (_e != hipSuccess)                                                           \
            return fail(MDBN_EHIP, "%s failed: %s (%s:%d)", #expr, hipGetErrorString(_e), \
                        __FILE__, __LINE__);                                            \
    } while (0)

#define REQUIRE(cond, ...)                                 \
    do {                                                   \
        if (!(cond)) return fail(MDBN_EINVAL, __VA_ARGS__); \
    } while (0)

#define CHECK(expr) do { int _rc = (expr); if (_rc != MDBN_OK) return _rc; } while (0)

constexpr int kTargetJobs = 256;

inline int64_t ru4(int64_t x) { return (x + 3) & ~int64_t(3); }
inline int64_t padded_ld(int64_t cols) { return ru4(cols); }
inline int64_t ru64(int64_t x) { return (x + 63) & ~int64_t(63); }
inline bool aligned16(const void* p) { return (reinterpret_cast<uintptr_t>(p) & 15u) == 0; }

int check_mat(const void* p, int64_t ld, int64_t cols, const char* name);
int check_groups(const int32_t* dev, const int32_t* host, int64_t n_groups, int64_t V, int& lo, int& hi);
PhiloxKey make_key(const mdbn_rng& r, uint32_t draw);

struct Workspace {
    float* slabs;
    int64_t slab_floats;
    float* cost_partials;
    int64_t cost_floats;
    float* colPpos;
    float* colPneg;
    float* colV;
};

int64_t dense_workspace_bytes(int64_t B, int64_t V, int64_t H);
int carve(void* ws, int64_t bytes, int64_t B, int64_t V, int64_t H, Workspace& out, bool need_stats, int64_t ldv = 0, int64_t ldh = 0);

struct Affine {
    const float* x = nullptr; int64_t rows = 0, ldx = 0;
    const float* W = nullptr; int64_t V = 0, H = 0, ldw = 0;
    int dir = 0;
    const float* bias = nullptr;
    float* pre = nullptr; float* mean = nullptr; float* sample = nullptr; int64_t ldo = 0;
    float mean_scale = 1.0f; int gauss = 0;
    const float* target = nullptr; int64_t ld_target = 0;
    bool want_cost = false;
    const mdbn_rng* rng = nullptr; uint32_t draw = 0u;
    float* colsum = nullptr; int colsum_kind = 0;
    bool x_binary = false;
    Affine(const float* x, int64_t rows, int64_t ldx, const float* W, int64_t V, int64_t H, int64_t ldw, const float* hbias)
        : x(x), rows(rows), ldx(ldx), W(W), V(V), H(H), ldw(ldw), dir(0), bias(hbias), ldo(ldw) {}
    Affine(const float* x, int64_t rows, int64_t ldx, const float* W, int64_t V, int64_t H, int64_t ldw, const float* vbias,
           int64_t ldo, int gauss) : x(x), rows(rows), ldx(ldx), W(W), V(V), H(H), ldw(ldw), dir(1), bias(vbias), ldo(ldo), gauss(gauss) {}
};

int run_affine(const Affine& a, const Workspace& ws, hipStream_t s, int* n_cost_out);

void fill_upd(UpdEpi& e, const mdbn_update_args& u, int64_t V, int64_t ldh, unsigned short* Wp);
void fill_bias_upd(BiasUpd& b, const mdbn_update_args& u, int64_t H);
// ... 13 lines not shown
```

mdbn_amd/csrc/mdbn_device.h:

```cpp
#pragma once
#include <hip/hip_runtime.h>
#include <stdint.h>
#include "philox.h"
#include "mdbn_kernels.h"

namespace mdbn {

__device__ __forceinline__ float comp(const float4& v, int j)
{
    return j == 0 ? v.x : j == 1 ? v.y : j == 2 ? v.z : v.w;
}
__device__ __forceinline__ void setc(float4& v, int j, float x)
{
    if (j == 0) v.x = x; else if (j == 1) v.y = x; else if (j == 2) v.z = x; else v.w = x;
}

__device__ __forceinline__ float upd_grad(float st, float inv_bs, float wc, float w0)
{
#pragma clang fp contract(off)
    const float a = st * inv_bs, b = wc * w0;
    return a - b;
}
__device__ __forceinline__ float upd_speed(float g, float sp, float mu)
{
#pragma clang fp contract(off)
    const float d = sp - g;
    const float e = d * mu;
    return g + e;
}
__device__ __forceinline__ float upd_param(float w, float m, float sp, float lr)
{
#pragma clang fp contract(off)
    const float a = w * m, b = sp * lr;
    return a + b;
}
__device__ __forceinline__ float upd_scale(float x, float s)
{
#pragma clang fp contract(off)
    return x * s;
}
__device__ __forceinline__ float upd_decay(float lr, float l2)
{
#pragma clang fp contract(off)
    const float a = 2.0f * lr;
    const float b = a * l2;
    return 1.0f - b;
}
__device__ __forceinline__ float upd_two_lr_l1(float lr, float l1)
{
#pragma clang fp contract(off)
    const float a = 2.0f * lr;
    return a * l1;
}
__device__ __forceinline__ float upd_shrink(float two_lr_l1, float w)
{
#pragma clang fp contract(off)
    const float d = fabsf(w) + 0.001f;
    const float q = __fdiv_rn(two_lr_l1, d);
    return 1.0f + q;
}

__device__ __forceinline__ void update_rule4(const float4& w, const float4& sp, const float4& st, const float4& wc0,
                                             float inv_bs, float wc, float decay, float l1, float two_lr_l1,
                                             float mu, float lr, float4& wn, float4& sn)
{
#pragma unroll
    for (int j = 0; j < 4; ++j) {
        const float wj = comp(w, j), spj = comp(sp, j);
        float g = upd_grad(comp(st, j), inv_bs, wc, comp(wc0, j));
        float m = decay;
        if (l1 != 0.0f) {
            const float shrink = upd_shrink(two_lr_l1, wj);
            g = __fdiv_rn(g, shrink);
            m = __fdiv_rn(decay, shrink);
        }
        setc(sn, j, upd_speed(g, spj, mu));
        setc(wn, j, upd_param(wj, m, spj, lr));
    }
}

__device__ __forceinline__ int fin_units(const FinArgs& f) { return (int)((f.ldh + f.ldv + 15) / 16); }

__device__ __forceinline__ void finalize_column(const FinArgs& f, int64_t i, float t)
{
    if (i < f.ldh) f.s_h[i] = t;
    else if (i < f.ldh + f.ldv) f.s_v[i - f.ldh] = t;
    if (f.do_bias) {
        const BiasUpd& bu = f.bu;
        if (i < bu.H) {
            const float sp = bu.hbs[i], p0 = bu.hb[i];
            bu.hbs[i] = upd_speed(upd_scale(t, bu.inv_rows), sp, bu.mu);
            bu.hb[i] = upd_param(p0, 1.0f, sp, bu.lr);
        } else if (i >= f.ldh && i - f.ldh < bu.V) {
            const int64_t j = i - f.ldh;
            const float sp = bu.vbs[j], p0 = bu.vb[j];
            bu.vbs[j] = upd_speed(upd_scale(t, bu.inv_rows), sp, bu.mu);
            bu.vb[j] = upd_param(p0, 1.0f, sp, bu.lr);
        }
    }
}

__device__ __forceinline__ void finalize_unit(const FinArgs& f, int unit, int lane)
{
    const int n_units = fin_units(f);
    if (unit < n_units) {
        const int cl = lane >> 2, qd = lane & 3;
        const int64_t i = (int64_t)unit * 16 + cl;
        const int per = (f.ngroups + 3) / 4;
        const int gbeg = qd * per, gend = min(f.ngroups, gbeg + per);
        float a = 0.f;
#ifndef MDBN_FIN_BATCH
#define MDBN_FIN_BATCH 0
#endif
#if !MDBN_FIN_BATCH
        if (i < f.ldh) {
#pragma unroll 16
            for (int g = gbeg; g < gend; ++g) a += f.posP[(int64_t)g * f.ldh + i] + f.negP[(int64_t)g * f.ldh + i];
        } else if (i < f.ldh + f.ldv) {
            const int64_t j = i - f.ldh;
#pragma unroll 16
            for (int g = gbeg; g < gend; ++g) a += f.partV[(int64_t)g * f.ldv + j];
        }
#else
        if (i < f.ldh) {
            for (int g0 = gbeg; g0 < gend; g0 += 8) {
                float p[8], q[8];
#pragma unroll
                for (int u = 0; u < 8; ++u) {
                    const int64_t g = min(g0 + u, gend - 1);
                    p[u] = f.posP[g * f.ldh + i]; q[u] = f.negP[g * f.ldh + i];
                }
#pragma unroll
                for (int u = 0; u < 8; ++u) a += g0 + u < gend ? p[u] + q[u] : 0.f;
            }
        } else if (i < f.ldh + f.ldv) {
            const int64_t j = i - f.ldh;
            for (int g0 = gbeg; g0 < gend; g0 += 8) {
                float p[8];
#pragma unroll
                for (int u = 0; u < 8; ++u) p[u] = f.partV[(int64_t)min(g0 + u, gend - 1) * f.ldv + j];
#pragma unroll
                for (int u = 0; u < 8; ++u) a += g0 + u < gend ? p[u] : 0.f;
            }
        }
#endif
        const int l0 = lane & ~3;
        const float r0 = __shfl(a, l0, 64), r1 = __shfl(a, l0 + 1, 64), r2 = __shfl(a, l0 + 2, 64), r3 = __shfl(a, l0 + 3, 64);
        const float t = (r0 + r1) + (r2 + r3);
        if (qd == 0) finalize_column(f, i, t);
    } else if (unit == n_units && f.cost_partials) {
        float a = 0.f;
        for (int k0 = lane; k0 < f.n_cost; k0 += 64 * 8) {
            float v[8];
#pragma unroll
            for (int u = 0; u < 8; ++u) v[u] = k0 + 64 * u < f.n_cost ? f.cost_partials[k0 + 64 * u] : 0.f;
#pragma unroll
            for (int u = 0; u < 8; ++u) a += v[u];
        }
#pragma unroll
        for (int off = 32; off > 0; off >>= 1) a += __shfl_down(a, off, 64);
        if (lane == 0) {
            f.cost[0] = a; f.cost[1] = 0.f; f.cost[2] = 0.f; f.cost[3] = 0.f;
            if (f.do_bias && f.bu.cost_out) f.bu.cost_out[0] = a * f.bu.cost_scale;
        }
    }
}


__device__ __forceinline__ int64_t epi_target_row(const EpiArgs& e, int64_t row)
{
    if (!e.target_idx) return row;
    int64_t s = e.target_idx64 ? reinterpret_cast<const int64_t*>(e.target_idx)[row]
                               : (int64_t)reinterpret_cast<const int32_t*>(e.target_idx)[row];
    if (s < 0) s += e.target_rows;
    return s < 0 ? 0 : (s >= e.target_rows ? e.target_rows - 1 : s);
}

__device__ __forceinline__ void epi_target_rows4(const EpiArgs& e, int r0, int64_t (&srow)[4])
{
    int64_t raw[4];
#pragma unroll
    for (int j = 0; j < 4; ++j) raw[j] = r0 + j < e.rows ? r0 + j : e.rows - 1;
    if (!e.target_idx) {
#pragma unroll
        for (int j = 0; j < 4; ++j) srow[j] = raw[j];
        return;
    }
    if (e.target_idx64) {
        const int64_t* ix = reinterpret_cast<const int64_t*>(e.target_idx);
#pragma unroll
        for (int j = 0; j < 4; ++j) raw[j] = ix[raw[j]];
    } else {
        const int32_t* ix = reinterpret_cast<const int32_t*>(e.target_idx);
#pragma unroll
        for (int j = 0; j < 4; ++j) raw[j] = (int64_t)ix[raw[j]];
    }
// ... 30 lines not shown
    if (lane == 0) red[wave] = v;
    __syncthreads();
    float t = 0.f;
    const int nw = (blockDim.x + 63) >> 6;
    for (int k = 0; k < nw; ++k) t += red[k];
    return t;
}

__device__ __forceinline__ void philox_rows4(const PhiloxKey& k, uint32_t draw, uint64_t g0,
                                             uint32_t col, uint32_t (&w)[4])
{
    uint32_t lo[4];
    philox4x32_10(col, (uint32_t)(g0 >> 2), draw, k.step, k.k0, k.k1, lo);
    const uint32_t ph = (uint32_t)(g0 & 3);
    if (ph == 0) {
        w[0] = lo[0]; w[1] = lo[1]; w[2] = lo[2]; w[3] = lo[3];
    } else {
        uint32_t hi[4];
        philox4x32_10(col, (uint32_t)(g0 >> 2) + 1u, draw, k.step, k.k0, k.k1, hi);
#pragma unroll
        for (int r = 0; r < 4; ++r) {
            uint32_t v = 0;
#pragma unroll
            for (int j = 0; j < 8; ++j) {
                const uint32_t cand = j < 4 ? lo[j & 3] : hi[j & 3];
                v = (ph + (uint32_t)r == (uint32_t)j) ? cand : v;
            }
            w[r] = v;
        }
    }
}

__device__ __forceinline__ void split3(float a, unsigned short& p1, unsigned short& p2, unsigned short& p3)
{
    const unsigned ua = __builtin_bit_cast(unsigned, a);
    const float ra = a - __builtin_bit_cast(float, ua & 0xffff0000u);
    const unsigned va = __builtin_bit_cast(unsigned, ra);
    const float sa = ra - __builtin_bit_cast(float, va & 0xffff0000u);
    p1 = (unsigned short)(ua >> 16); p2 = (unsigned short)(va >> 16);
    p3 = (unsigned short)(__builtin_bit_cast(unsigned, sa) >> 16);
}

__device__ __forceinline__ void store_planes4(unsigned short* P, int64_t plane_stride, int64_t off, const float4& v)
{
    unsigned short q[3][4];
    split3(v.x, q[0][0], q[1][0], q[2][0]);
    split3(v.y, q[0][1], q[1][1], q[2][1]);
    split3(v.z, q[0][2], q[1][2], q[2][2]);
    split3(v.w, q[0][3], q[1][3], q[2][3]);
#pragma unroll
    for (int p = 0; p < 3; ++p) {
        uint2 w;
        w.x = q[p][0] | ((unsigned)q[p][1] << 16);
        w.y = q[p][2] | ((unsigned)q[p][3] << 16);
        *reinterpret_cast<uint2*>(P + p * plane_stride + off) = w;
    }
}

__device__ __forceinline__ void act_quad_targets(const EpiArgs& e, int r0, int col, bool live, float (&tg4)[4])
{
#pragma unroll
    for (int j = 0; j < 4; ++j) tg4[j] = 0.f;
    if (e.target && live) {
        int64_t srow[4];
        epi_target_rows4(e, r0, srow);
#pragma unroll
        for (int j = 0; j < 4; ++j) tg4[j] = e.target[srow[j] * e.ld_target + col];
    }
}

template <int MODE = -1>
__device__ __forceinline__ void act_quad_tg(const EpiArgs& e, float x0, float x1, float x2, float x3, int r0, int col, bool live, float& cost,
                                            const float (&tg4)[4])
{
    const bool is_gauss = MODE < 0 ? e.gauss != 0 : (MODE & 2) != 0;
    const bool need_u = MODE < 0 ? (e.sample != nullptr || e.sample_plane != nullptr) : (MODE & 1) != 0;
    const bool need_z = need_u && is_gauss;
    uint32_t wa[4] = {0u, 0u, 0u, 0u}, wb[4] = {0u, 0u, 0u, 0u};
    if (need_u) {
        const uint64_t g0 = e.rng.row_offset + (uint64_t)r0;
        philox_rows4(e.rng, e.rng.draw, g0, (uint32_t)col, wa);
        if (need_z) philox_rows4(e.rng, e.rng.draw | MDBN_NORMAL_BIT, g0, (uint32_t)col, wb);
    }
    float csum = 0.f;
#pragma unroll
    for (int j = 0; j < 4; ++j) {
        const int row = r0 + j;
        float xj = j == 0 ? x0 : (j == 1 ? x1 : (j == 2 ? x2 : x3));
        if (row < e.rows) {
            const int64_t off = (int64_t)row * e.ld + col;
            float m, sv = 0.f;
            if (is_gauss) {
                m = xj;
                if (need_u) {
                    const float u1 = philox_u01(wa[j]), u2 = philox_u01(wb[j]);
                    sv = m + sqrtf(-2.0f * logf(u1)) * cosf(6.28318530717958647692f * u2);
                }
            } else {
                m = sigmoidf_(xj);
                if (need_u) sv = philox_u01(wa[j]) < m ? 1.0f : 0.0f;
            }
            float tg = 0.f;
            if (e.target && live) {
                tg = tg4[j];
                if (is_gauss) { const float d = sigmoidf_(xj) - tg; cost += d * d; }
                else cost += tg * softplusf_(-xj) + (1.0f - tg) * softplusf_(xj);
            }
            if (!live) { m = 0.f; sv = 0.f; xj = 0.f; }
            const float ms = m * e.mean_scale;
            if (e.pre) e.pre[off] = xj;
            if (e.mean) e.mean[off] = ms;
            if (e.sample) e.sample[off] = sv;
            if (e.mean_planes) {
                unsigned short p1, p2, p3;
                split3(ms, p1, p2, p3);
                e.mean_planes[off] = p1; e.mean_planes[e.plane_stride + off] = p2; e.mean_planes[2 * e.plane_stride + off] = p3;
            }
            if (e.sample_plane) e.sample_plane[off] = (unsigned short)(__builtin_bit_cast(unsigned, sv) >> 16);
            if (live) csum += e.colsum_kind == 0 ? ms : (e.colsum_kind == 1 ? tg - m : tg - sv);
        }
    }
    if (e.colsum) e.colsum[(int64_t)(r0 >> 2) * e.ld + col] = csum;
}

template <int MODE = -1>
__device__ __forceinline__ void act_quad(const EpiArgs& e, float x0, float x1, float x2, float x3, int r0, int col, bool live, float& cost)
{
    float tg4[4];
    act_quad_targets(e, r0, col, live, tg4);
    act_quad_tg<MODE>(e, x0, x1, x2, x3, r0, col, live, cost, tg4);
}

template <int BM, int BN, int NT = 512>
__device__ __forceinline__ void fused_tile_epilogue(const EpiArgs& e, float* T, int m0, int n0, int cost_slot = -1)
{
    constexpr int LDT = BN + 8;
    const int c = threadIdx.x & (BN - 1), rg0 = threadIdx.x / BN;
    const int col = n0 + c;
    const bool live = col < e.cols, incol = col < (int)e.ld;
    const float bias = live ? e.bias[col] : 0.f;
    float cost = 0.f;
#pragma unroll 1
    for (int rg = rg0; rg < BM / 4; rg += NT / BN) {
        const int r0 = m0 + 4 * rg;
        if (r0 >= e.rows || !incol) continue;
        float x[4];
#pragma unroll
        for (int j = 0; j < 4; ++j) x[j] = T[(4 * rg + j) * LDT + c] + bias;
        act_quad(e, x[0], x[1], x[2], x[3], r0, col, live, cost);
    }
    if (e.cost_partials) {
        const float tot = block_sum(cost, T + BM * LDT);
        if (threadIdx.x == 0) e.cost_partials[cost_slot < 0 ? (int)blockIdx.x : cost_slot] = tot;
    }
}


template <int NT, bool GAUSS, bool SAMPLE>
__device__ __forceinline__ void fused_tile_epilogue_4x4_t(const EpiArgs& e, float* T, int m0, int n0,
                                                          unsigned long long* stamps )
{
    constexpr int BM = 128, BN = 64, LDT = BN + 8;
    static_assert(NT == 512, "one 4 x 4 block per thread");
    const int cq = threadIdx.x & 15, rg = threadIdx.x >> 4;
    const int col0 = n0 + 4 * cq, r0 = m0 + 4 * rg;
    float cost = 0.f;
    if (r0 < e.rows && col0 < (int)e.ld) {
        float4 tg[4];
        const bool want_tg = e.target != nullptr;
        if (want_tg) {
            int64_t srow[4];
            epi_target_rows4(e, r0, srow);
#pragma unroll
            for (int j = 0; j < 4; ++j) tg[j] = *reinterpret_cast<const float4*>(e.target + srow[j] * e.ld_target + col0);
        }
        const float4 b4 = make_float4(col0 < e.cols ? e.bias[col0] : 0.f, col0 + 1 < e.cols ? e.bias[col0 + 1] : 0.f,
                                      col0 + 2 < e.cols ? e.bias[col0 + 2] : 0.f, col0 + 3 < e.cols ? e.bias[col0 + 3] : 0.f);
        float4 x[4];
#pragma unroll
        for (int j = 0; j < 4; ++j) {
            x[j] = *reinterpret_cast<const float4*>(T + (4 * rg + j) * LDT + 4 * cq);
            x[j].x += b4.x; x[j].y += b4.y; x[j].z += b4.z; x[j].w += b4.w;
        }
        constexpr bool need_u = SAMPLE, need_z = SAMPLE && GAUSS;
        float4 ms[4], sv[4], pre[4];
        float4 cs = make_float4(0.f, 0.f, 0.f, 0.f);
        if (stamps && threadIdx.x == 0) {
            asm volatile("s_waitcnt vmcnt(0) lgkmcnt(0)" ::: "memory");
            stamps[0] = wall_clock64();
        }
#pragma unroll
        for (int c = 0; c < 4; ++c) {
            const int col = col0 + c;
            const bool live = col < e.cols;
            uint32_t wa[4] = {0u, 0u, 0u, 0u}, wb[4] = {0u, 0u, 0u, 0u};
            if constexpr (need_u) {
                const uint64_t g0 = e.rng.row_offset + (uint64_t)r0;
                philox_rows4(e.rng, e.rng.draw, g0, (uint32_t)col, wa);
                if constexpr (need_z) philox_rows4(e.rng, e.rng.draw | MDBN_NORMAL_BIT, g0, (uint32_t)col, wb);
            }
            float csum = 0.f;
#pragma unroll
            for (int j = 0; j < 4; ++j) {
                float xj = comp(x[j], c);
                float m, s1 = 0.f;
                if constexpr (GAUSS) {
                    m = xj;
                    if constexpr (need_u) {
                        const float u1 = philox_u01(wa[j]), u2 = philox_u01(wb[j]);
                        s1 = m + sqrtf(-2.0f * logf(u1)) * cosf(6.28318530717958647692f * u2);
                    }
                } else {
                    m = sigmoidf_(xj);
                    if constexpr (need_u) s1 = philox_u01(wa[j]) < m ? 1.0f : 0.0f;
                }
                float t1 = 0.f;
                if (want_tg && live && r0 + j < e.rows) {
                    t1 = comp(tg[j], c);
                    if constexpr (GAUSS) { const float d = sigmoidf_(xj) - t1; cost += d * d; }
                    else cost += t1 * softplusf_(-xj) + (1.0f - t1) * softplusf_(xj);
                }
                if (!live) { m = 0.f; s1 = 0.f; xj = 0.f; }
                const float m1 = m * e.mean_scale;
                setc(ms[j], c, m1); setc(sv[j], c, s1); setc(pre[j], c, xj);
                if (live && r0 + j < e.rows) csum += e.colsum_kind == 0 ? m1 : (e.colsum_kind == 1 ? t1 - m : t1 - s1);
            }
            setc(cs, c, csum);
        }
        if (stamps && threadIdx.x == 0) { asm volatile("" :: "v"(cs.x), "v"(ms[3].w)); stamps[1] = wall_clock64(); }
#pragma unroll
        for (int j = 0; j < 4; ++j) {
            if (r0 + j >= e.rows) break;
            const int64_t off = (int64_t)(r0 + j) * e.ld + col0;
            if (e.pre) *reinterpret_cast<float4*>(e.pre + off) = pre[j];
            if (e.mean) *reinterpret_cast<float4*>(e.mean + off) = ms[j];
            if (e.sample) *reinterpret_cast<float4*>(e.sample + off) = sv[j];
            if (e.mean_planes) store_planes4(e.mean_planes, e.plane_stride, off, ms[j]);
            if (e.sample_plane) {
                uint2 w;
                w.x = (__builtin_bit_cast(unsigned, sv[j].x) >> 16) | (__builtin_bit_cast(unsigned, sv[j].y) & 0xffff0000u);
                w.y = (__builtin_bit_cast(unsigned, sv[j].z) >> 16) | (__builtin_bit_cast(unsigned, sv[j].w) & 0xffff0000u);
                *reinterpret_cast<uint2*>(e.sample_plane + off) = w;
            }
        }
        if (e.colsum) *reinterpret_cast<float4*>(e.colsum + (int64_t)(r0 >> 2) * e.ld + col0) = cs;
        if (stamps && threadIdx.x == 0) {
            asm volatile("s_waitcnt vmcnt(0)" ::: "memory");
            stamps[2] = wall_clock64();
        }
    }
    if (e.cost_partials) {
        const float tot = block_sum(cost, T + BM * LDT);
        if (threadIdx.x == 0) e.cost_partials[blockIdx.x] = tot;
    }
}

template <int NT = 512>
__device__ __forceinline__ void fused_tile_epilogue_4x4(const EpiArgs& e, float* T, int m0, int n0,
                                                        unsigned long long* stamps = nullptr)
{
    const bool sample = e.sample != nullptr || e.sample_plane != nullptr;
    if (e.gauss) {
        if (sample) fused_tile_epilogue_4x4_t<NT, true, true>(e, T, m0, n0, stamps);
        else fused_tile_epilogue_4x4_t<NT, true, false>(e, T, m0, n0, stamps);
    } else {
        if (sample) fused_tile_epilogue_4x4_t<NT, false, true>(e, T, m0, n0, stamps);
        else fused_tile_epilogue_4x4_t<NT, false, false>(e, T, m0, n0, stamps);
    }
}

#ifndef FUSED_UPD_RB
#define FUSED_UPD_RB 4
#endif
template <int BM, int BN, int NT = 512>
__device__ __forceinline__ void fused_update_epilogue(const UpdEpi& u, const float* T, int m0, int n0)
{
    constexpr int LDT = BN + 8, C4 = BN / 4, RSTEP = NT / C4, RB = FUSED_UPD_RB;
    const int c4 = threadIdx.x % C4, rr = threadIdx.x / C4;
    const int col = n0 + 4 * c4;
    if (col >= (int)u.ld) return;
    const float two_lr_l1 = upd_two_lr_l1(u.lr, u.l1);
    const float decay = upd_decay(u.lr, u.l2);
#pragma unroll 1
    for (int r = rr; r < BM; r += RSTEP * RB) {
        float4 w[RB], sp[RB], w0[RB];
        const float* w0base = u.W0 ? u.W0 : u.W;
#pragma unroll
        for (int b = 0; b < RB; ++b) {
            const int rowc = min(m0 + min(r + b * RSTEP, BM - 1), u.rows - 1);
            const int64_t off = (int64_t)rowc * u.ld + col;
            w[b] = *reinterpret_cast<const float4*>(u.W + off);
            sp[b] = *reinterpret_cast<const float4*>(u.Ws + off);
            w0[b] = *reinterpret_cast<const float4*>(w0base + off);
        }
        __builtin_amdgcn_sched_barrier(0);
#pragma unroll
        for (int b = 0; b < RB; ++b) {
            const int row = m0 + r + b * RSTEP;
            if (r + b * RSTEP < BM && row < u.rows) {
                const int64_t off = (int64_t)row * u.ld + col;
                const float4 st = *reinterpret_cast<const float4*>(T + (r + b * RSTEP) * LDT + 4 * c4);
                float4 wn, sn;
                update_rule4(w[b], sp[b], st, w0[b], u.inv_bs, u.wc, decay, u.l1, two_lr_l1, u.mu, u.lr, wn, sn);
                *reinterpret_cast<float4*>(u.W + off) = wn;
                *reinterpret_cast<float4*>(u.Ws + off) = sn;
                if (u.Wp) store_planes4(u.Wp, u.wp_stride, off, wn);
            }
        }
    }
}

}
```

mdbn_amd/csrc/mdbn_kernels.h:

```cpp
#pragma once
#include <hip/hip_runtime.h>
#include <stdint.h>
#include "philox.h"
#include "../../include/mdbn_hip.h"

namespace mdbn {

enum { LAY_K = 0, LAY_MN = 1 };

struct EpiArgs {
    const float* slabs;
    int64_t slab_stride;
    int nsplit;
    int rows, cols;
    int64_t ld;
    const float* bias;
    float* pre;
    float* mean;
    float* sample;
    float mean_scale;
    int gauss;
    const float* target;
    int64_t ld_target;
    const void* target_idx;
    int target_idx64;
    int64_t target_rows;
    float* cost_partials;
    float* colsum;
    int colsum_kind;
    PhiloxKey rng;
    unsigned short* mean_planes;
    int64_t plane_stride;
    unsigned short* sample_plane;
    int bal_P, bal_S, bal_tiles_m, bal_tiles_n;
};

struct UpdEpi {
    float* W; float* Ws; const float* W0;
    int64_t ld;
    int rows;
    float lr, l1, l2, wc, mu, inv_bs;
    unsigned short* Wp;
    int64_t wp_stride;
    const float* Sprev;
    int64_t flat_per_wg;
    int early;
};

struct DeferredBias {
    int on;
    float* hb; float* hbs; float* vb; float* vbs;
    const float* s_h; const float* s_v; const float* cost_sum;
    int64_t H, V;
    float lr, mu, inv_rows, cost_scale;
    float* cost_out;
};

struct BiasUpd {
    float* hb; float* hbs; float* vb; float* vbs;
    int64_t H, V;
    float lr, mu, inv_rows, cost_scale;
    float* cost_out;
};

struct FinArgs {
    const float* posP; const float* negP; const float* partV;
    int ngroups;
    int64_t ldh, ldv;
    const float* cost_partials; int n_cost;
    float* s_h; float* s_v; float* cost;
    BiasUpd bu; int do_bias;
};

struct GemmArgs {
    const float* A;
    const float* B;
    float* C;
    int64_t lda, ldb, ldc;
    int64_t slab_stride;
    int M, N, K;
    int Nst;
    int kchunk;
    int splitk, tiles_m, tiles_n;
    int bn;
    int bk;
    int inner_m;
    int x6;
    int x6_pw;
    int cw;
    unsigned long long* stamps;
    int skinny;
    int mi;
    int ni;
    int fused;
    EpiArgs epi;
    UpdEpi upd;
    int fin_enabled;
    FinArgs fin;
};



struct GatherAhead {
    const float* src; int64_t n_rows, ld_src;
    const void* idx; int idx64;
    int B, rpw, passes;
    unsigned short* P; int64_t plane_stride, ld;
};

struct PlaneGemmArgs {
    const unsigned short* A; int64_t lda, pa;
    const unsigned short* B; int64_t ldb, pb;
    float* C; int64_t ldc, slab_stride;
    int M, N, K, kchunk, splitk, tiles_m, tiles_n;
    int ap;
    int ms;
    int bn;
    int fused;
    int slab_tail;
    unsigned long long* stamps;
    int bal;
    int xcd_group;
    float* scratch;
    int64_t c_bytes;
    EpiArgs epi;
    UpdEpi upd;
    int fin_enabled;
    int stats_tail;
    int deep;
    FinArgs fin;
    GatherAhead ga;
    DeferredBias db;
};

__host__ __device__ inline int bal_first_unit(int w, int P, int64_t U) { return (int)(((int64_t)w * U) / P); }
__host__ __device__ inline int bal_block_of(int64_t u, int P, int64_t U) { return (int)(((u + 1) * P - 1) / U); }
__host__ __device__ inline int bal_rem_blocks(int tiles, int S, int P)
{
    const int64_t Ur = (int64_t)(tiles - (tiles / P) * P) * S;
    return Ur < P ? (int)Ur : P;
}
__host__ __device__ inline int bal_tile_slabs(int t, int tiles, int S, int P)
{
    const int Tf = (tiles / P) * P;
    if (t < Tf) return 1;
    const int64_t Ur = (int64_t)(tiles - Tf) * S, u0 = (int64_t)(t - Tf) * S;
    const int Pr = bal_rem_blocks(tiles, S, P);
    return bal_block_of(u0 + S - 1, Pr, Ur) - bal_block_of(u0, Pr, Ur) + 1;
}
hipError_t launch_gemm_planes(int la, int lb, const PlaneGemmArgs& g, hipStream_t s);
bool slab_tail_ok(const PlaneGemmArgs& g, int la, int lb);
bool stats_tail_ok(const PlaneGemmArgs& g, int la, int lb);
bool narrow_deep_ok(const PlaneGemmArgs& g, int la, int lb);
hipError_t launch_gemm_planes_bal(int la, int lb, const PlaneGemmArgs& g, hipStream_t s);
int bal_max_segments(int tiles, int stages, int P);
int bal_segment_host(int tiles, int S, int P, int w, int k, int* tile, int* s0, int* s1, int* nseg, int* nt);
hipError_t launch_split_planes(const float* X, int64_t rows, int64_t ld, unsigned short* P, int64_t plane_stride, hipStream_t s);
hipError_t launch_gather_planes(const float* src, int64_t n_rows, int64_t cols_ld, int64_t ld_src, const void* idx, int idx64,
                                int64_t n_idx, float* dst, int64_t ld_dst, unsigned short* P, int64_t plane_stride, hipStream_t s);

int epilogue_blocks(int64_t rows, int64_t ld);
int epilogue_cw(int64_t rows, int64_t ld);
void set_epilogue_cw(int cw);
void set_epilogue_threads(int t);
inline int row_groups(int64_t B) { return (int)((B + 3) / 4); }

hipError_t launch_gemm(int la, int lb, const GemmArgs& g, hipStream_t s);
hipError_t launch_act_epilogue(const EpiArgs& e, hipStream_t s);
hipError_t launch_sum_slabs(const float* slabs, int nsplit, int64_t slab_stride, int64_t n,
                            float* out, hipStream_t s);
hipError_t launch_gather_slim(const float* src, int64_t n_rows, int64_t cols_ld, int64_t ld_src, const void* idx, int idx64,
                              int64_t n_idx, float* dst, int64_t ld_dst, int blocks, int threads, hipStream_t s);
hipError_t launch_gather(const float* src, int64_t n_rows, int64_t cols_ld, int64_t ld_src,
                         const void* idx, int idx64, int64_t n_idx, float* dst, int64_t ld_dst,
                         hipStream_t s);
hipError_t launch_colsum_groups(const float* X, const float* Y, int rows, int64_t ld, float* out, hipStream_t s);
FinArgs make_fin_args(const float* posP, const float* negP, const float* partV, int ngroups, int64_t ldh, int64_t ldv,
                      const float* cost_partials, int n_cost, float* s_h, float* s_v, float* cost,
                      const BiasUpd* bias_update);
hipError_t launch_finalize_stats(const float* posP, const float* negP, const float* partV, int ngroups,
                                 int64_t ldh, int64_t ldv, const float* cost_partials, int n_cost,
                                 float* s_h, float* s_v, float* cost, const BiasUpd* bias_update, hipStream_t s);
hipError_t launch_update(const mdbn_update_args& a, hipStream_t s, const float* slabs = nullptr, int nslab = 1,
                         int64_t slab_stride = 0, unsigned short* Wp = nullptr);
hipError_t launch_free_energy(const float* slabs, int nsplit, int64_t slab_stride, int64_t ldh, int H,
                              const float* hbias, const float* x, int64_t ldv, int V, const float* vbias,
                              int gauss, int64_t rows, float* out, hipStream_t s);
hipError_t launch_round_flip(const float* x, float* out, int64_t rows, int64_t cols, int64_t ld, int64_t flip_col, hipStream_t s);
hipError_t launch_pl_cost(const float* fe, const float* fe_flip, int64_t rows, float n_visible, float* out, hipStream_t s);
hipError_t launch_recon_cost(const float* pre, int64_t ldp, const float* tgt, int64_t ldt, int64_t rows, int64_t cols, int gauss,
                             float scale, float* partials, int n_partials, float* out, hipStream_t s);
hipError_t launch_tanh(float* x, int64_t rows, int64_t cols, int64_t ld, hipStream_t s);
hipError_t launch_count_nonfinite(const float* x, int64_t n, int* count, hipStream_t s);
hipError_t launch_narrow_bf16(const float* x, unsigned short* y, int64_t n, hipStream_t s);
hipError_t launch_widen_bf16(const unsigned short* y, float* x, int64_t n, hipStream_t s);
hipError_t launch_rng_fill(float* out, int64_t rows, int64_t cols, int64_t ld, const PhiloxKey& k,
                           int normal, hipStream_t s);

}
```

mdbn_amd/csrc/mdbn_kernels.hip:

```cpp
#include <hip/hip_runtime.h>
#include <algorithm>
#include <cstring>
#include <stdint.h>
#include "philox.h"
#include "mdbn_kernels.h"
#include "mdbn_device.h"
#include "mdbn_skinny.h"

namespace mdbn {


constexpr int NTHREADS = 256;

template <int LAY, int ROWS, int KB, bool GUARD>
__device__ __forceinline__ void load_tile(const float* __restrict__ P, int64_t ld, int MN, int K,
                                          int mn0, int k0, float4 (&r)[ROWS * KB / 1024])
{
    const int tid = threadIdx.x & (NTHREADS - 1);
    if constexpr (LAY == LAY_K) {
        constexpr int TPRK = KB / 4, RPPK = NTHREADS / TPRK;
        const int c = tid % TPRK, rr = tid / TPRK;
        const int kq = k0 + 4 * c;
        const float* src = P + (int64_t)(mn0 + rr) * ld + kq;
#pragma unroll
// ... 864 lines not shown

template <int LA, int LB, int MI, int FUSED>
static hipError_t launch_skinny_t(const GemmArgs& g, hipStream_t s)
{
    constexpr int lds_bytes = (SKINNY_WAVES * 32 * MI * SKINNY_LDT + 8) * (int)sizeof(float);
    static bool attr_set = false;
    auto kern = skinny_gemm_kernel<LA, LB, MI, FUSED>;
    if (!attr_set && lds_bytes > 64 * 1024) {
        hipError_t e = hipFuncSetAttribute(reinterpret_cast<const void*>(kern),
                                           hipFuncAttributeMaxDynamicSharedMemorySize, lds_bytes);
        if (e != hipSuccess) return e;
        attr_set = true;
    }
    hipLaunchKernelGGL(kern, dim3(g.tiles_n * g.tiles_m * g.splitk), dim3(64 * SKINNY_WAVES), lds_bytes, s, g);
    return hipGetLastError();
}

hipError_t launch_skinny_gemm(int la, int lb, const GemmArgs& g, hipStream_t s)
{
    if (g.M < 1 || (g.mi != 1 && g.mi != 2) || (int64_t)g.tiles_m * 32 * g.mi < g.M || g.kchunk % 8 != 0 ||
        (g.fused && g.splitk != 1))
        return hipErrorInvalidValue;
#define SKINNY_CASE(LAV, LBV, MIV, FV) \
    if (la == LAV && lb == LBV && g.mi == MIV && g.fused == FV) return launch_skinny_t<LAV, LBV, MIV, FV>(g, s)
    SKINNY_CASE(LAY_K, LAY_K, 1, 0);  SKINNY_CASE(LAY_K, LAY_K, 1, 1);
    SKINNY_CASE(LAY_K, LAY_K, 2, 0);  SKINNY_CASE(LAY_K, LAY_K, 2, 1);
    SKINNY_CASE(LAY_K, LAY_MN, 1, 0); SKINNY_CASE(LAY_K, LAY_MN, 1, 1);
    SKINNY_CASE(LAY_K, LAY_MN, 2, 0); SKINNY_CASE(LAY_K, LAY_MN, 2, 1);
    SKINNY_CASE(LAY_MN, LAY_MN, 2, 0); SKINNY_CASE(LAY_MN, LAY_MN, 2, 2);
#undef SKINNY_CASE
    return hipErrorInvalidValue;
}

template <int CW> struct VecIO;
template <> struct VecIO<4> {
    static __device__ __forceinline__ void load(const float* p, float (&v)[4]) { const float4 t = *reinterpret_cast<const float4*>(p); v[0] = t.x; v[1] = t.y; v[2] = t.z; v[3] = t.w; }
    static __device__ __forceinline__ void store(float* p, const float (&v)[4]) { *reinterpret_cast<float4*>(p) = make_float4(v[0], v[1], v[2], v[3]); }
};
template <> struct VecIO<2> {
    static __device__ __forceinline__ void load(const float* p, float (&v)[2]) { const float2 t = *reinterpret_cast<const float2*>(p); v[0] = t.x; v[1] = t.y; }
    static __device__ __forceinline__ void store(float* p, const float (&v)[2]) { *reinterpret_cast<float2*>(p) = make_float2(v[0], v[1]); }
};
template <> struct VecIO<1> {
    static __device__ __forceinline__ void load(const float* p, float (&v)[1]) { v[0] = *p; }
    static __device__ __forceinline__ void store(float* p, const float (&v)[1]) { *p = v[0]; }
};

template <int NS, int CW, int MODE = -1>
__global__ __launch_bounds__(256) void act_epilogue_kernel(EpiArgs e)
{
    __shared__ float red[4];
    asm volatile("" :: "s"(e.slabs), "s"(e.slab_stride), "s"(e.nsplit), "s"(e.rows), "s"(e.cols), "s"(e.ld), "s"(e.bias),
                 "s"(e.target), "s"(e.ld_target), "s"(e.target_idx), "s"(e.mean_planes), "s"(e.plane_stride), "s"(e.sample_plane),
                 "s"(e.colsum), "s"(e.target_idx64), "s"((int)blockDim.x));
    const bool is_gauss = MODE < 0 ? e.gauss != 0 : (MODE & 2) != 0;
    const int ldc = (int)(e.ld / CW);
    const int64_t idx = (int64_t)blockIdx.x * blockDim.x + threadIdx.x;
    const int rg = (int)(idx / ldc), cq = (int)(idx - (int64_t)rg * ldc);
    const int r0 = rg * 4, c0 = cq * CW;
    float cost = 0.f;
    if (r0 < e.rows) {
        float bias[CW];
#pragma unroll
        for (int j = 0; j < CW; ++j) bias[j] = c0 + j < e.cols ? e.bias[c0 + j] : 0.f;
        float pre[4][CW];
        const float* base = e.slabs + (int64_t)r0 * e.ld + c0;
        double acc[4][CW];
#pragma unroll
        for (int r = 0; r < 4; ++r)
#pragma unroll
            for (int j = 0; j < CW; ++j) acc[r][j] = 0.0;
        const int rlast = e.rows - 1 - r0;
        float tgt4[4][CW];
#pragma unroll
        for (int r = 0; r < 4; ++r)
#pragma unroll
            for (int j = 0; j < CW; ++j) tgt4[r][j] = 0.f;
        if (e.target) {
            int64_t srow[4];
            epi_target_rows4(e, r0, srow);
#pragma unroll
            for (int r = 0; r < 4; ++r) VecIO<CW>::load(e.target + srow[r] * e.ld_target + c0, tgt4[r]);
        }
        if (NS > 0) {
            constexpr int RB = NS * CW >= 64 ? 1 : (NS * CW >= 32 ? 2 : 4);
#pragma unroll
            for (int rb = 0; rb < 4; rb += RB) {
                float v[RB][NS > 0 ? NS : 1][CW];
#pragma unroll
                for (int r = 0; r < RB; ++r)
#pragma unroll
                    for (int sidx = 0; sidx < NS; ++sidx)
                        VecIO<CW>::load(base + (int64_t)min(rb + r, rlast) * e.ld + (int64_t)sidx * e.slab_stride, v[r][sidx]);
                __builtin_amdgcn_sched_barrier(0);
#pragma unroll
                for (int r = 0; r < RB; ++r)
#pragma unroll
                    for (int sidx = 0; sidx < NS; ++sidx)
#pragma unroll
                        for (int j = 0; j < CW; ++j) acc[rb + r][j] += rb + r <= rlast ? (double)v[r][sidx][j] : 0.0;
            }
        } else {
            constexpr int SB = 16 / CW;
            int nsplit = e.nsplit;
            if (e.bal_P) {
                const int tm = r0 >> 7, tn = c0 >> 7;
                const int t = e.bal_tiles_m <= e.bal_tiles_n ? tn * e.bal_tiles_m + tm : tm * e.bal_tiles_n + tn;
                nsplit = bal_tile_slabs(t, e.bal_tiles_m * e.bal_tiles_n, e.bal_S, e.bal_P);
            }
            for (int s0 = 0; s0 < nsplit; s0 += SB) {
                float v[4][SB][CW];
#pragma unroll
                for (int r = 0; r < 4; ++r)
#pragma unroll
                    for (int u = 0; u < SB; ++u)
                        VecIO<CW>::load(base + (int64_t)min(r, rlast) * e.ld + (int64_t)min(s0 + u, nsplit - 1) * e.slab_stride, v[r][u]);
                __builtin_amdgcn_sched_barrier(0);
#pragma unroll
                for (int r = 0; r < 4; ++r)
#pragma unroll
                    for (int u = 0; u < SB; ++u)
#pragma unroll
                        for (int j = 0; j < CW; ++j) acc[r][j] += (r <= rlast && s0 + u < nsplit) ? (double)v[r][u][j] : 0.0;
            }
        }
#pragma unroll
        for (int r = 0; r < 4; ++r)
#pragma unroll
            for (int j = 0; j < CW; ++j) pre[r][j] = (float)acc[r][j] + bias[j];
        uint32_t wa[CW][4], wb[CW][4];
        const bool need_u = MODE < 0 ? (e.sample != nullptr || e.sample_plane != nullptr) : (MODE & 1) != 0;
        const bool need_z = need_u && is_gauss;
        if (need_u) {
            const uint64_t g0 = e.rng.row_offset + (uint64_t)r0;
#pragma unroll
            for (int j = 0; j < CW; ++j) {
                philox_rows4(e.rng, e.rng.draw, g0, (uint32_t)(c0 + j), wa[j]);
                if (need_z) philox_rows4(e.rng, e.rng.draw | MDBN_NORMAL_BIT, g0, (uint32_t)(c0 + j), wb[j]);
            }
        }
        float csum[CW];
#pragma unroll
        for (int j = 0; j < CW; ++j) csum[j] = 0.f;
#pragma unroll
        for (int r = 0; r < 4; ++r) {
            if (r0 + r >= e.rows) continue;
            const int64_t off = (int64_t)(r0 + r) * e.ld + c0;
            float mean[CW], samp[CW], tgt[CW];
#pragma unroll
            for (int j = 0; j < CW; ++j) tgt[j] = tgt4[r][j];
#pragma unroll
            for (int j = 0; j < CW; ++j) {
                const bool live = c0 + j < e.cols;
                const float x = pre[r][j];
                float m, sv = 0.f;
                if (is_gauss) {
                    m = x;
                    if (need_u) {
                        const float u1 = philox_u01(wa[j][r]), u2 = philox_u01(wb[j][r]);
                        sv = m + sqrtf(-2.0f * logf(u1)) * cosf(6.28318530717958647692f * u2);
                    }
                } else {
                    m = sigmoidf_(x);
                    if (need_u) sv = philox_u01(wa[j][r]) < m ? 1.0f : 0.0f;
                }
                if (e.target && live) {
                    if (is_gauss) { const float d = sigmoidf_(x) - tgt[j]; cost += d * d; }
                    else cost += tgt[j] * softplusf_(-x) + (1.0f - tgt[j]) * softplusf_(x);
                }
                if (!live) { m = 0.f; sv = 0.f; pre[r][j] = 0.f; }
                const float ms = m * e.mean_scale;
                mean[j] = ms;
                samp[j] = sv;
                if (live) csum[j] += e.colsum_kind == 0 ? ms : (e.colsum_kind == 1 ? tgt[j] - m : tgt[j] - sv);
            }
            if (e.pre) VecIO<CW>::store(e.pre + off, pre[r]);
            if (e.mean) VecIO<CW>::store(e.mean + off, mean);
            if (e.sample) VecIO<CW>::store(e.sample + off, samp);
            if (e.mean_planes || e.sample_plane) {
                unsigned short q[4][CW];
#pragma unroll
                for (int j = 0; j < CW; ++j) {
                    split3(mean[j], q[0][j], q[1][j], q[2][j]);
                    q[3][j] = (unsigned short)(__builtin_bit_cast(unsigned, samp[j]) >> 16);
                }
#pragma unroll
                for (int pl = 0; pl < 4; ++pl) {
                    unsigned short* dst = pl < 3 ? (e.mean_planes ? e.mean_planes + pl * e.plane_stride + off : nullptr)
                                                 : (e.sample_plane ? e.sample_plane + off : nullptr);
                    if (!dst) continue;
                    if constexpr (CW == 4) {
                        uint2 w; w.x = q[pl][0] | ((unsigned)q[pl][1] << 16); w.y = q[pl][2] | ((unsigned)q[pl][3] << 16);
                        *reinterpret_cast<uint2*>(dst) = w;
                    } else if constexpr (CW == 2) {
                        *reinterpret_cast<unsigned*>(dst) = q[pl][0] | ((unsigned)q[pl][1] << 16);
                    } else {
                        dst[0] = q[pl][0];
                    }
                }
            }
        }
        if (e.colsum) VecIO<CW>::store(e.colsum + (int64_t)rg * e.ld + c0, csum);
    }
    if (e.cost_partials) {
        const float tot = block_sum(cost, red);
        if (threadIdx.x == 0) e.cost_partials[blockIdx.x] = tot;
    }
}

static int g_epilogue_cw = 0;
void set_epilogue_cw(int cw) { g_epilogue_cw = cw; }

int epilogue_cw(int64_t rows, int64_t ld)
{
    if (g_epilogue_cw) return g_epilogue_cw;
    const int64_t quads = (rows + 3) / 4;
    if (quads * (ld / 4) >= 8 * 256 * 256) return 4;
    return quads * (ld / 2) >= 64 * 256 ? 2 : 1;
}

static int g_epilogue_threads = 0;
void set_epilogue_threads(int t) { g_epilogue_threads = t; }
static int epilogue_threads(int64_t rows, int64_t ld)
{
    if (g_epilogue_threads) return g_epilogue_threads;
    const int64_t n = ((rows + 3) / 4) * (ld / epilogue_cw(rows, ld));
    return n <= 64 * 256 ? 64 : 256;
}

int epilogue_blocks(int64_t rows, int64_t ld)
{
    const int cw = epilogue_cw(rows, ld), t = epilogue_threads(rows, ld);
    const int64_t n = ((rows + 3) / 4) * (ld / cw);
    return (int)((n + t - 1) / t);
}

template <int CW>
static void launch_act_epilogue_cw(const EpiArgs& e, hipStream_t s)
{
    const int64_t n = ((int64_t)(e.rows + 3) / 4) * (e.ld / CW);
    const int t = epilogue_threads(e.rows, e.ld);
    const dim3 grid((unsigned)((n + t - 1) / t)), block(t);
    const int mode = (e.gauss ? 2 : 0) | ((e.sample != nullptr || e.sample_plane != nullptr) ? 1 : 0);
    if (mode != 3 && (e.bal_P || (e.nsplit != 6 && e.nsplit != 7))) {
        const int ns = e.bal_P ? 0 : (e.nsplit == 8 || e.nsplit == 2 || e.nsplit == 16 || e.nsplit == 3 || e.nsplit == 4) ? e.nsplit : 0;
#define EPI_MODE_CASE(NSV, MV) \
    if (ns == NSV && mode == MV) { hipLaunchKernelGGL((act_epilogue_kernel<NSV, CW, MV>), grid, block, 0, s, e); return; }
#define EPI_MODE_CASES(NSV) EPI_MODE_CASE(NSV, 0) EPI_MODE_CASE(NSV, 1) EPI_MODE_CASE(NSV, 2)
        EPI_MODE_CASES(8) EPI_MODE_CASES(2) EPI_MODE_CASES(16) EPI_MODE_CASES(3) EPI_MODE_CASES(4)
#undef EPI_MODE_CASES
#undef EPI_MODE_CASE
    }
    switch (e.bal_P ? 0 : e.nsplit) {
        case 1: hipLaunchKernelGGL((act_epilogue_kernel<1, CW>), grid, block, 0, s, e); break;
        case 2: hipLaunchKernelGGL((act_epilogue_kernel<2, CW>), grid, block, 0, s, e); break;
        case 4: hipLaunchKernelGGL((act_epilogue_kernel<4, CW>), grid, block, 0, s, e); break;
        case 8: hipLaunchKernelGGL((act_epilogue_kernel<8, CW>), grid, block, 0, s, e); break;
        case 7: hipLaunchKernelGGL((act_epilogue_kernel<7, CW>), grid, block, 0, s, e); break;
        case 6: hipLaunchKernelGGL((act_epilogue_kernel<6, CW>), grid, block, 0, s, e); break;
        default: hipLaunchKernelGGL((act_epilogue_kernel<0, CW>), grid, block, 0, s, e); break;
    }
}

hipError_t launch_act_epilogue(const EpiArgs& e, hipStream_t s)
{
    switch (epilogue_cw(e.rows, e.ld)) {
        case 4: launch_act_epilogue_cw<4>(e, s); break;
        case 2: launch_act_epilogue_cw<2>(e, s); break;
        default: launch_act_epilogue_cw<1>(e, s); break;
    }
    return hipGetLastError();
}

__global__ __launch_bounds__(256) void sum_slabs_kernel(const float* __restrict__ slabs, int nsplit,
                                                        int64_t slab_stride, int64_t n4,
                                                        float* __restrict__ out)
{
    for (int64_t i = (int64_t)blockIdx.x * blockDim.x + threadIdx.x; i < n4;
         i += (int64_t)gridDim.x * blockDim.x) {
        float4 a = make_float4(0.f, 0.f, 0.f, 0.f);
        for (int s0 = 0; s0 < nsplit; s0 += 8) {
            float4 v[8];
#pragma unroll
            for (int u = 0; u < 8; ++u)
// ... 10 lines not shown
                            float* out, hipStream_t s)
{
    const int64_t n4 = n >> 2;
    const int grid = (int)std::min<int64_t>((n4 + 255) / 256, 2048);
    hipLaunchKernelGGL(sum_slabs_kernel, dim3(grid), dim3(256), 0, s, slabs, nsplit, slab_stride, n4, out);
    return hipGetLastError();
}

__global__ __launch_bounds__(256) void gather_rows_kernel(const float* __restrict__ src, int64_t n_rows,
                                                          int64_t ld_src, const void* __restrict__ idx,
                                                          int idx64, int64_t ld4, float* __restrict__ dst,
                                                          int64_t ld_dst)
{
    const int64_t r = blockIdx.y;
    const int64_t c = (int64_t)blockIdx.x * blockDim.x + threadIdx.x;
    if (c >= ld4) return;
    int64_t s = r;
    if (idx) s = idx64 ? reinterpret_cast<const int64_t*>(idx)[r] : (int64_t)reinterpret_cast<const int32_t*>(idx)[r];
    if (s < 0) s += n_rows;
    s = s < 0 ? 0 : (s >= n_rows ? n_rows - 1 : s);
    reinterpret_cast<float4*>(dst + r * ld_dst)[c] = reinterpret_cast<const float4*>(src + s * ld_src)[c];
}

hipError_t launch_gather(const float* src, int64_t n_rows, int64_t cols_ld, int64_t ld_src,
                         const void* idx, int idx64, int64_t n_idx, float* dst, int64_t ld_dst,
                         hipStream_t s)
{
    if (n_idx <= 0) return hipSuccess;
    const int64_t ld4 = cols_ld >> 2;
    const int64_t rows_per_launch = 65535;
    for (int64_t r0 = 0; r0 < n_idx; r0 += rows_per_launch) {
        const int64_t nr = std::min(rows_per_launch, n_idx - r0);
        const void* ip = idx ? (idx64 ? (const void*)(reinterpret_cast<const int64_t*>(idx) + r0)
                                      : (const void*)(reinterpret_cast<const int32_t*>(idx) + r0))
                             : nullptr;
        const float* sp = idx ? src : src + r0 * ld_src;
        hipLaunchKernelGGL(gather_rows_kernel, dim3((unsigned)((ld4 + 255) / 256), (unsigned)nr), dim3(256), 0, s,
                           sp, idx ? n_rows : n_rows - r0, ld_src, ip, idx64, ld4, dst + r0 * ld_dst, ld_dst);
    }
    return hipGetLastError();
}

__global__ __launch_bounds__(256) void gather_rows_slim_kernel(const float* __restrict__ src, int64_t n_rows, int64_t ld_src,
                                                               const void* __restrict__ idx, int idx64, int64_t ld4,
                                                               int64_t n_idx, float* __restrict__ dst, int64_t ld_dst)
{
    const int nt = blockDim.x;
    for (int64_t r = blockIdx.x; r < n_idx; r += gridDim.x) {
        int64_t s = r;
        if (idx) s = idx64 ? reinterpret_cast<const int64_t*>(idx)[r] : (int64_t)reinterpret_cast<const int32_t*>(idx)[r];
        if (s < 0) s += n_rows;
        s = s < 0 ? 0 : (s >= n_rows ? n_rows - 1 : s);
        const float4* in = reinterpret_cast<const float4*>(src + s * ld_src);
        float4* out = reinterpret_cast<float4*>(dst + r * ld_dst);
        for (int64_t c0 = threadIdx.x; c0 < ld4; c0 += 4 * nt) {
            float4 v[4];
#pragma unroll
            for (int u = 0; u < 4; ++u)
                if (c0 + u * nt < ld4) v[u] = in[c0 + u * nt];
#pragma unroll
            for (int u = 0; u < 4; ++u)
                if (c0 + u * nt < ld4) out[c0 + u * nt] = v[u];
        }
    }
}

hipError_t launch_gather_slim(const float* src, int64_t n_rows, int64_t cols_ld, int64_t ld_src, const void* idx, int idx64,
                              int64_t n_idx, float* dst, int64_t ld_dst, int blocks, int threads, hipStream_t s)
{
    if (n_idx <= 0) return hipSuccess;
    blocks = (int)std::min<int64_t>(std::max(1, std::min(blocks, 1024)), n_idx);
    hipLaunchKernelGGL(gather_rows_slim_kernel, dim3(blocks), dim3(threads), 0, s, src, n_rows, ld_src, idx, idx64, cols_ld >> 2,
                       n_idx, dst, ld_dst);
    return hipGetLastError();
}

__global__ __launch_bounds__(256) void finalize_stats_kernel(FinArgs f)
{
    finalize_unit(f, (int)blockIdx.x * 4 + (int)(threadIdx.x >> 6), threadIdx.x & 63);
}

FinArgs make_fin_args(const float* posP, const float* negP, const float* partV, int ngroups, int64_t ldh, int64_t ldv,
                      const float* cost_partials, int n_cost, float* s_h, float* s_v, float* cost,
                      const BiasUpd* bias_update)
{
    FinArgs f;
    memset(&f, 0, sizeof f);
    f.posP = posP; f.negP = negP; f.partV = partV; f.ngroups = ngroups; f.ldh = ldh; f.ldv = ldv;
    f.cost_partials = cost_partials; f.n_cost = n_cost; f.s_h = s_h; f.s_v = s_v; f.cost = cost;
    if (bias_update) { f.bu = *bias_update; f.do_bias = 1; }
    return f;
}

hipError_t launch_finalize_stats(const float* posP, const float* negP, const float* partV, int ngroups,
                                 int64_t ldh, int64_t ldv, const float* cost_partials, int n_cost,
                                 float* s_h, float* s_v, float* cost, const BiasUpd* bias_update, hipStream_t s)
{
    const FinArgs f = make_fin_args(posP, negP, partV, ngroups, ldh, ldv, cost_partials, n_cost, s_h, s_v, cost,
                                    bias_update);
    const int units = (int)((ldh + ldv + 15) / 16) + 1;
    hipLaunchKernelGGL(finalize_stats_kernel, dim3((units + 3) / 4), dim3(256), 0, s, f);
    return hipGetLastError();
}

__global__ __launch_bounds__(256) void colsum_groups_kernel(const float* __restrict__ X, const float* __restrict__ Y,
                                                            int rows, int64_t ld, float* __restrict__ out)
{
    const int ld4 = (int)(ld >> 2);
    const int64_t idx = (int64_t)blockIdx.x * blockDim.x + threadIdx.x;
    const int rg = (int)(idx / ld4), cq = (int)(idx - (int64_t)rg * ld4);
    if (rg * 4 >= rows) return;
    float4 a = make_float4(0.f, 0.f, 0.f, 0.f);
    for (int r = rg * 4; r < min(rows, rg * 4 + 4); ++r) {
        const float4 v = *reinterpret_cast<const float4*>(X + (int64_t)r * ld + cq * 4);
        a.x += v.x; a.y += v.y; a.z += v.z; a.w += v.w;
        if (Y) {
            const float4 y = *reinterpret_cast<const float4*>(Y + (int64_t)r * ld + cq * 4);
            a.x -= y.x; a.y -= y.y; a.z -= y.z; a.w -= y.w;
        }
    }
    *reinterpret_cast<float4*>(out + (int64_t)rg * ld + cq * 4) = a;
}

hipError_t launch_colsum_groups(const float* X, const float* Y, int rows, int64_t ld, float* out, hipStream_t s)
{
    hipLaunchKernelGGL(colsum_groups_kernel, dim3(epilogue_blocks(rows, ld)), dim3(256), 0, s, X, Y, rows, ld, out);
    return hipGetLastError();
}

template <bool DO_SPEED, bool DO_PARAMS, bool NEWSPEED = false>
__global__ __launch_bounds__(256) void update_kernel(float4* __restrict__ W, float4* __restrict__ Ws,
                                                     const float4* __restrict__ W0, const float4* __restrict__ S,
                                                     int64_t n4, float lr, float l1, float l2, float wc,
                                                     float mu, float inv_bs,
                                                     float* __restrict__ hb, float* __restrict__ hbs,
                                                     const float* __restrict__ s_h, int64_t H,
                                                     float* __restrict__ vb, float* __restrict__ vbs,
                                                     const float* __restrict__ s_v, int64_t V, float inv_rows,
                                                     const float* __restrict__ cost_sum, float cost_scale,
                                                     float* __restrict__ cost_out, int nslab, int64_t slab_stride4,
                                                     unsigned short* __restrict__ Wp)
{
    constexpr bool do_speed = DO_SPEED, do_params = DO_PARAMS;
    {
        const int64_t i = (int64_t)blockIdx.x * blockDim.x + threadIdx.x;
        if (i < H) {
            float sp = hbs[i];
            if (do_speed) {
                const float sn = upd_speed(upd_scale(s_h[i], inv_rows), sp, mu);
                hbs[i] = sn;
                if (NEWSPEED) sp = sn;
            }
            if (do_params) hb[i] = upd_param(hb[i], 1.0f, sp, lr);
        } else if (i < H + V) {
            const int64_t j = i - H;
            float sp = vbs[j];
            if (do_speed) {
                const float sn = upd_speed(upd_scale(s_v[j], inv_rows), sp, mu);
                vbs[j] = sn;
                if (NEWSPEED) sp = sn;
            }
            if (do_params) vb[j] = upd_param(vb[j], 1.0f, sp, lr);
        }
        if (i == 0 && cost_out && do_speed) cost_out[0] = cost_sum[0] * cost_scale;
    }
    const float two_lr_l1 = upd_two_lr_l1(lr, l1);
    const float decay = upd_decay(lr, l2);
    for (int64_t i = (int64_t)blockIdx.x * blockDim.x + threadIdx.x; i < n4;
         i += (int64_t)gridDim.x * blockDim.x) {
        const float4 sp = Ws[i];
        if constexpr (DO_SPEED && DO_PARAMS && NEWSPEED) {
            const float4 w = W[i], st = S[i];
            const float4 w0 = wc != 0.0f ? W0[i] : make_float4(0.f, 0.f, 0.f, 0.f);
            float4 sn, wn;
#pragma unroll
            for (int j = 0; j < 4; ++j) {
                const float snj = upd_speed(upd_grad(comp(st, j), inv_bs, wc, comp(w0, j)), comp(sp, j), mu);
                setc(sn, j, snj);
                setc(wn, j, upd_param(comp(w, j), decay, snj, lr));
            }
            Ws[i] = sn;
            W[i] = wn;
// ... 299 lines not shown
```

mdbn_amd/csrc/mdbn_planes.hip:

```cpp
#include <hip/hip_runtime.h>
#include <algorithm>
#include <stdint.h>
#include "mdbn_kernels.h"
#include "mdbn_device.h"
#include "mdbn_planes_image.h"

namespace mdbn {

typedef __bf16 pbf16x8 __attribute__((ext_vector_type(8)));
typedef short ps16x4 __attribute__((ext_vector_type(4)));
typedef short ps16x8 __attribute__((ext_vector_type(8)));
typedef float pf32x16 __attribute__((ext_vector_type(16)));
typedef float pf32x4 __attribute__((ext_vector_type(4)));
typedef unsigned int pu32x4b __attribute__((ext_vector_type(4)));
typedef unsigned int pu32x2b __attribute__((ext_vector_type(2)));

#ifndef PL_ARGS_EARLY
#define PL_ARGS_EARLY 1
#endif
#ifndef PL_SIDE_WT
#define PL_SIDE_WT 0
#endif
constexpr int PL_PLANE = 8192, PL_STAGE = 6 * PL_PLANE, PL_NSTAGE = 3, PL_LW = 4;

// ... 388 lines not shown
            : __builtin_amdgcn_mfma_f32_16x16x32_bf16(X, Y, T, c0_, c1_, c2_))
#define MMQ_CHAIN(T, FA, FB, a, b, C0)                                                        \
    do {                                                                                      \
        T = (C0);                                                                             \
        if constexpr (AP == 3) {                                 \
            T = PL_MF16(FA[2][a], FB[0][b], T, 0, 0, 0);      \
            T = PL_MF16(FA[0][a], FB[2][b], T, 0, 0, 0);      \
            T = PL_MF16(FA[1][a], FB[1][b], T, 0, 0, 0);      \
            T = PL_MF16(FA[1][a], FB[0][b], T, 0, 0, 0);      \
            T = PL_MF16(FA[0][a], FB[1][b], T, 0, 0, 0);      \
            T = PL_MF16(FA[0][a], FB[0][b], T, 0, 0, 0);      \
        } else if constexpr (AP == 1) {    \
            T = PL_MF16(FA[0][a], FB[2][b], T, 0, 0, 0);      \
            T = PL_MF16(FA[0][a], FB[1][b], T, 0, 0, 0);      \
            T = PL_MF16(FA[0][a], FB[0][b], T, 0, 0, 0);      \
        } else {                                    \
            T = PL_MF16(FA[0][a], FB[0][b], T, 0, 0, 0);      \
        }                                                                                     \
    } while (0)
#if PL_STAGE_ACC
#define MMQ(FA, FB, AH, BH)                                                                   \
    do {                                                                                      \
        if constexpr (AP == 0 || !(LA == LAY_K && LB == LAY_MN)) {                            \
            _Pragma("unroll") for (int a = 0; a < 2; ++a)                                     \
                _Pragma("unroll") for (int b = 0; b < NBH; ++b) {                             \
                    pf32x4a& c = acc[2 * (AH) + a][NBH * (BH) + b];                           \
                    MMQ_CHAIN(c, FA, FB, a, b, c);                                            \
                }                                                                             \
        } else {                                                                              \
            pf32x4a tq[2 * NBH];                                                              \
            _Pragma("unroll") for (int i = 0; i <= 2 * NBH; ++i) {                            \
                if (i < 2 * NBH) MMQ_CHAIN(tq[i], FA, FB, i / NBH, i % NBH, (pf32x4a{0.f, 0.f, 0.f, 0.f})); \
                if (i > 0) acc[2 * (AH) + (i - 1) / NBH][NBH * (BH) + (i - 1) % NBH] += tq[i - 1]; \
            }                                                                                 \
        }                                                                                     \
    } while (0)
#else
#define MMQ(FA, FB, AH, BH)                                                                   \
    _Pragma("unroll") for (int a = 0; a < 2; ++a)                                             \
        _Pragma("unroll") for (int b = 0; b < NBH; ++b) {                                     \
            pf32x4a& c = acc[2 * (AH) + a][NBH * (BH) + b];                                   \
            MMQ_CHAIN(c, FA, FB, a, b, c);                                                    \
        }
#endif
#define ORD(NR)                                                                               \
    _Pragma("unroll") for (int i_ = 0; i_ < ((NR) < NM ? (NR) : NM); ++i_) {                  \
        __builtin_amdgcn_sched_group_barrier(0x100, 1, 0);                                    \
        __builtin_amdgcn_sched_group_barrier(0x008, 1, 0);                                    \
    }                                                                                         \
    if ((NR) > NM) __builtin_amdgcn_sched_group_barrier(0x100, (NR) - NM, 0);                 \
    if (NM > (NR)) __builtin_amdgcn_sched_group_barrier(0x008, NM - (NR), 0);
#define PIN(FA, NPL)                                                                          \
    _Pragma("unroll") for (int pl = 0; pl < (NPL); ++pl)                                      \
        _Pragma("unroll") for (int i = 0; i < 2; ++i) asm volatile("" :: "v"(FA[pl][i]));
#define PINB(FB, NPL)                                                                         \
    _Pragma("unroll") for (int pl = 0; pl < (NPL); ++pl)                                      \
        _Pragma("unroll") for (int i = 0; i < NBH; ++i) asm volatile("" :: "v"(FB[pl][i]));
#define PL_STAGE_EVEN(BASE, NEXT, BARRIER)                                                    \
    do {                                                                                      \
        RD_B(Bhi, BASE, 1); MMQ(Alo, Blo, 0, 0); ORD(RB);                                     \
        RD_A(Ahi, BASE, 1); MMQ(Alo, Bhi, 0, 1); ORD(RA);                                     \
        PINB(Bhi, NB); PIN(Ahi, NA);                                                          \
        BARRIER;                      \
        RD_A(Alo, NEXT, 0); MMQ(Ahi, Bhi, 1, 1); ORD(RA);                                     \
        RD_B(Bhi, NEXT, 1); MMQ(Ahi, Blo, 1, 0); ORD(RB);                                     \
    } while (0)
#define PL_STAGE_ODD(BASE, NEXT, BARRIER)                                                     \
    do {                                                                                      \
        RD_B(Blo, BASE, 0); MMQ(Alo, Bhi, 0, 1); ORD(RB);                                     \
        RD_A(Ahi, BASE, 1); MMQ(Alo, Blo, 0, 0); ORD(RA);                                     \
        PINB(Blo, NB); PIN(Ahi, NA);                                                          \
        BARRIER;                                                                              \
        RD_A(Alo, NEXT, 0); MMQ(Ahi, Blo, 1, 0); ORD(RA);                                     \
        RD_B(Blo, NEXT, 0); MMQ(Ahi, Bhi, 1, 1); ORD(RB);                                     \
    } while (0)
#define PL_RAW_BARRIER() asm volatile("s_waitcnt lgkmcnt(0)\n\ts_barrier" ::: "memory")
#ifndef PL_MAIN_BARRIER
#ifdef MDBN_STAMP
#define PL_MAIN_BARRIER() do { const long long t_ = clock64(); __syncthreads(); bar_wait += clock64() - t_; } while (0)
#else
#define PL_MAIN_BARRIER() __syncthreads()
#endif
#endif
#define PL_CONSUME_CONSTS() PL_CONSUME_CONSTS_SW(false)
#define PL_CONSUME_CONSTS_SW(SW)                                                              \
    constexpr bool PL_SWP = (SW);                                                             \
    constexpr int NA = AP == 3 ? 3 : 1, NB = AP == 0 ? 1 : 3;       \
    constexpr int RA = 2 * NA * (LA == LAY_MN ? 2 : 1), RB = NBH * NB * (LB == LAY_MN ? 2 : 1), \
                  NM = 2 * NBH * (AP == 3 ? 6 : (AP == 1 ? 3 : 1));

template <int LA, int LB, int AP, int NBH = 2>
__device__ __forceinline__ void pl_consume16(char* smem, int nt, int lane, int wm, int wn, pf32x4a (&acc)[4][2 * NBH],
                                             bool open_barrier = true, long long* bar_wait_out = nullptr)
{
    long long bar_wait = 0;
    (void)bar_wait;
    int offA[4][2], offB[4][2];
    pl_offsets16<LA, LB>(lane, wm, wn, offA, offB);
    PL_CONSUME_CONSTS();
    pbf16x8 Alo[3][2], Ahi[3][2], Blo[3][2], Bhi[3][2];
    if (open_barrier) __syncthreads();
    RD_A(Alo, smem, 0);
    RD_B(Blo, smem, 0);
    for (int it = 0; it < nt; it += 2) {
        {
            const char* base = smem + (it % PL_NSTAGE) * PL_STAGE;
            const char* next = smem + ((it + 1) % PL_NSTAGE) * PL_STAGE;
            PL_STAGE_EVEN(base, next, PL_MAIN_BARRIER());
        }
        if (it + 1 < nt) {
            const char* base = smem + ((it + 1) % PL_NSTAGE) * PL_STAGE;
            const char* next = smem + ((it + 2) % PL_NSTAGE) * PL_STAGE;
            PL_STAGE_ODD(base, next, PL_MAIN_BARRIER());
        }
    }
    if (bar_wait_out) *bar_wait_out = bar_wait;
}

template <int AP>
__device__ __forceinline__ void pl_consume16_deep(char* smem, int nt, int lane, int wm, int wn, pf32x4a (&acc)[4][2],
                                                  long long* bar_wait_out = nullptr)
{
    static_assert(AP == 1, "64-deep stages hold one plane of A (three would need 72 KB a slot)");
    long long bar_wait = 0;
    (void)bar_wait;
    int offA[4][2], offB[2][2];
#pragma unroll
    for (int kh = 0; kh < 2; ++kh) {
#pragma unroll
        for (int b = 0; b < 4; ++b) offA[b][kh] = deep_image::plane_base(true, 0) + deep_image::frag_offset(wm + 16 * b, kh, lane);
#pragma unroll
        for (int b = 0; b < 2; ++b) offB[b][kh] = deep_image::frag_offset(wn + 16 * b, kh, lane);
    }
    pbf16x8 A0[4], B0[3][2], A1[4], B1[3][2];
#define DP_RD(FA, FB, BASE, KH)                                                               \
    do {                                                                                      \
        _Pragma("unroll") for (int b = 0; b < 4; ++b) FA[b] = *reinterpret_cast<const pbf16x8*>((BASE) + offA[b][KH]); \
        _Pragma("unroll") for (int pl = 0; pl < 3; ++pl)                                      \
            _Pragma("unroll") for (int b = 0; b < 2; ++b)                                     \
                FB[pl][b] = *reinterpret_cast<const pbf16x8*>((BASE) + deep_image::plane_base(false, pl) + offB[b][KH]); \
    } while (0)
#define DP_MM(FA, FB)                                                                         \
    _Pragma("unroll") for (int pl = 2; pl >= 0; --pl)                                         \
        _Pragma("unroll") for (int a = 0; a < 4; ++a)                                         \
            _Pragma("unroll") for (int b = 0; b < 2; ++b)                                     \
                acc[a][b] = __builtin_amdgcn_mfma_f32_16x16x32_bf16(FA[a], FB[pl][b], acc[a][b], 0, 0, 0);
#define DP_ORD()                                                                              \
    _Pragma("unroll") for (int i_ = 0; i_ < 10; ++i_) {                                       \
        __builtin_amdgcn_sched_group_barrier(0x100, 1, 0);                                    \
        __builtin_amdgcn_sched_group_barrier(0x008, 1, 0);                                    \
    }                                                                                         \
    __builtin_amdgcn_sched_group_barrier(0x008, 14, 0);
#define DP_PIN(FA, FB)                                                                        \
    do {                                                                                      \
        _Pragma("unroll") for (int b = 0; b < 4; ++b) asm volatile("" :: "v"(FA[b]));         \
        _Pragma("unroll") for (int pl = 0; pl < 3; ++pl)                                      \
            _Pragma("unroll") for (int b = 0; b < 2; ++b) asm volatile("" :: "v"(FB[pl][b])); \
    } while (0)
    DP_RD(A0, B0, smem, 0);
    for (int it = 0; it < nt; ++it) {
        const char* base = smem + (it % PL_NSTAGE) * PL_STAGE;
        const char* next = smem + ((it + 1) % PL_NSTAGE) * PL_STAGE;
        DP_RD(A1, B1, base, 1); DP_MM(A0, B0); DP_ORD();
        __builtin_amdgcn_sched_barrier(0);
        DP_PIN(A1, B1);
        PL_MAIN_BARRIER();
        DP_RD(A0, B0, next, 0); DP_MM(A1, B1); DP_ORD();
    }
#undef DP_RD
#undef DP_MM
#undef DP_ORD
#undef DP_PIN
    if (bar_wait_out) *bar_wait_out = bar_wait;
}

template <int LA, int LB, int AP, int FUSED, int MS, int BN = 128, int KD = 32>
__global__ __launch_bounds__(64 * (4 + PL_LW)) void gemm_planes_kernel(PlaneGemmArgs g)
{
    static_assert(BN == 128 || (BN == 64 && MS == 16 && FUSED == 1 && LB == LAY_K), "64-column tiles: unsplit ROW-operand forward pass");
    static_assert(KD == 32 || (KD == 64 && BN == 64 && AP == 1 && LA == LAY_K), "64-deep stages: narrow one-plane forward pass");
    extern __shared__ __attribute__((aligned(16))) char smem[];
#if PL_ARGS_EARLY
    asm volatile("" :: "s"(g.A), "s"(g.lda), "s"(g.pa), "s"(g.B), "s"(g.ldb), "s"(g.pb), "s"(g.C), "s"(g.ldc), "s"(g.slab_stride),
                 "s"(g.kchunk), "s"(g.tiles_m), "s"(g.tiles_n), "s"((int)gridDim.x));
#endif
    const int nwg = gridDim.x, bid = blockIdx.x;
    const int xcd = bid & 7, slot = bid >> 3;
    const int qq = nwg >> 3, rem = nwg & 7;
    const int w = (xcd < rem ? xcd * (qq + 1) : rem * (qq + 1) + (xcd - rem) * qq) + slot;
    const int tiles = g.tiles_m * g.tiles_n;
    const int ks = w / tiles, t = w - ks * tiles;
    int tm, tn;
    if (g.tiles_m <= g.tiles_n) { tn = t / g.tiles_m; tm = t - tn * g.tiles_m; }
    else { tm = t / g.tiles_n; tn = t - tm * g.tiles_n; }
    const int m0 = tm * 128, n0 = tn * BN;
    const int kbeg = ks * g.kchunk;
    const int nt = g.kchunk / KD;
    const int wave = __builtin_amdgcn_readfirstlane(threadIdx.x >> 6);
    const int lane = threadIdx.x & 63;

    EarlySpeed es;
    (void)es;
    if (wave >= 4) {
        pl_loader<LA, LB, AP, MS, (FUSED == 2 || (FUSED == 0 && LA == LAY_MN && LB == LAY_MN && AP == 3)) && MS == 16, BN, KD>(
            g, smem, wave - 4, lane, m0, n0, kbeg, nt, &es);
        if constexpr (FUSED == 0) return;
    } else {
        const int r = lane & 31, h = lane >> 5;
        const int wm = (wave >> 1) * 64, wn = (wave & 1) * (BN / 2);
        if constexpr (FUSED == 0 && LA == LAY_MN && LB == LAY_MN) {
            if (g.db.on) deferred_bias_update(g.db, wave, lane);
        }
        if constexpr ((FUSED == 2 || FUSED == 0) && LA == LAY_MN && LB == LAY_MN) {
            if (g.fin_enabled) {
                const int nu = fin_units(g.fin);
                for (int unit = wave * (int)gridDim.x + (int)blockIdx.x; unit <= nu; unit += 4 * (int)gridDim.x)
                    finalize_unit(g.fin, unit, lane);
            }
        }
        if constexpr (MS == 16) {
            constexpr int NBH = BN / 64, NBB = 2 * NBH;
            pf32x4a acc[4][NBB];
#pragma unroll
            for (int a = 0; a < 4; ++a)
#pragma unroll
                for (int b = 0; b < NBB; ++b) acc[a][b] = pf32x4a{0.f, 0.f, 0.f, 0.f};
#ifdef MDBN_STAMP
#define PL_MSTAMP(SLOT)                                                                       \
    do {                                                                                      \
        if (PL_STAMP_COND && g.stamps && wave == 0 && lane == 0)                              \
            g.stamps[(int64_t)blockIdx.x * 16 + (SLOT)] = wall_clock64();                     \
    } while (0)
#else
#define PL_MSTAMP(SLOT) do {} while (0)
#endif
            PL_MSTAMP(8);
            __syncthreads();
            PL_MSTAMP(9);
#ifdef MDBN_STAMP
            if (PL_STAMP_COND && g.stamps && wave == 0 && lane == 0)
                g.stamps[(int64_t)blockIdx.x * 16 + 13] = clock64();
#endif
#ifdef MDBN_STAMP
            long long bw = 0;
            if constexpr (KD == 64) pl_consume16_deep<AP>(smem, nt, lane, wm, wn, acc, &bw);
            else pl_consume16<LA, LB, AP, NBH>(smem, nt, lane, wm, wn, acc, false, &bw);
#else
            if constexpr (KD == 64) pl_consume16_deep<AP>(smem, nt, lane, wm, wn, acc);
            else pl_consume16<LA, LB, AP, NBH>(smem, nt, lane, wm, wn, acc, false);
#endif
            PL_MSTAMP(10);
#ifdef MDBN_STAMP
            if (PL_STAMP_COND && g.stamps && wave == 0 && lane == 0) {
                g.stamps[(int64_t)blockIdx.x * 16 + 14] = clock64();
                g.stamps[(int64_t)blockIdx.x * 16 + 15] = bw;
            }
#endif
            const int c16 = lane & 15, q4 = lane >> 4;
            if constexpr (FUSED != 0) {
                float* T = reinterpret_cast<float*>(smem);
                constexpr int LDT = BN + 8;
#pragma unroll
                for (int a = 0; a < 4; ++a)
#pragma unroll
                    for (int b = 0; b < NBB; ++b)
#pragma unroll
                        for (int e = 0; e < 4; ++e)
                            T[(wm + 16 * a + 4 * q4 + e) * LDT + wn + 16 * b + c16] = acc[a][b][e];
            } else {
                float* C = g.C + (int64_t)ks * g.slab_stride;
#pragma unroll
                for (int a = 0; a < 4; ++a)
#pragma unroll
                    for (int b = 0; b < NBB; ++b)
#pragma unroll
                        for (int e = 0; e < 4; ++e)
                            C[(int64_t)(m0 + wm + 16 * a + 4 * q4 + e) * g.ldc + n0 + wn + 16 * b + c16] = acc[a][b][e];
                PL_MSTAMP(11);
#ifdef MDBN_STAMP
                asm volatile("s_waitcnt vmcnt(0)" ::: "memory");
#endif
                PL_MSTAMP(12);
                return;
            }
        } else {
        int offA[2][2][2], offB[2][2][2];
#pragma unroll
        for (int b = 0; b < 2; ++b)
#pragma unroll
            for (int s = 0; s < 2; ++s) {
                const int gq = (lane >> 4) & 1, i = lane & 15, q = i >> 2, p = i & 3;
                {
                    const int row = wm + 32 * b + r;
                    if (LA == LAY_K) {
                        offA[b][s][0] = row * 64 + ((((2 * s + h) ^ ((row >> 2) & 3))) << 4);
                        offA[b][s][1] = 0;
                    } else {
                        const int ch = (wm + 32 * b) / 8 + 2 * gq + (p >> 1);
#pragma unroll
                        for (int tt = 0; tt < 2; ++tt)
                            offA[b][s][tt] = (16 * s + 8 * h + 4 * tt + q) * 256 + ((ch ^ (q << 2)) << 4) + 8 * (p & 1);
                    }
                }
                {
                    const int row = wn + 32 * b + r;
                    if (LB == LAY_K) {
                        offB[b][s][0] = row * 64 + ((((2 * s + h) ^ ((row >> 2) & 3))) << 4);
                        offB[b][s][1] = 0;
                    } else {
                        const int ch = (wn + 32 * b) / 8 + 2 * gq + (p >> 1);
#pragma unroll
                        for (int tt = 0; tt < 2; ++tt)
                            offB[b][s][tt] = (16 * s + 8 * h + 4 * tt + q) * 256 + ((ch ^ (q << 2)) << 4) + 8 * (p & 1);
                    }
                }
            }
        pf32x16 acc[2][2];
#pragma unroll
        for (int a = 0; a < 2; ++a)
#pragma unroll
            for (int b = 0; b < 2; ++b)
#pragma unroll
                for (int e = 0; e < 16; ++e) acc[a][b][e] = 0.f;

        pbf16x8 f0a[3][2], f0b[3][2], f1a[3][2], f1b[3][2];
#define PL_FRAGS(FA, FB, BASE, S)                                                             \
    _Pragma("unroll") for (int pl = 0; pl < 3; ++pl)                                          \
        _Pragma("unroll") for (int a = 0; a < 2; ++a) {                                       \
            if (pl < AP) FA[pl][a] = pl_frag<LA>((BASE) + pl * PL_PLANE, offA[a][S][0], offA[a][S][1]); \
            FB[pl][a] = pl_frag<LB>((BASE) + (3 + pl) * PL_PLANE, offB[a][S][0], offB[a][S][1]); \
        }
#define PL_CHAIN(T, FA, FB, a, b)                                                                \
    do {                                                                                      \
        if constexpr (AP == 3) {                                 \
            T = __builtin_amdgcn_mfma_f32_32x32x16_bf16(FA[2][a], FB[0][b], T, 0, 0, 0);      \
            T = __builtin_amdgcn_mfma_f32_32x32x16_bf16(FA[0][a], FB[2][b], T, 0, 0, 0);      \
            T = __builtin_amdgcn_mfma_f32_32x32x16_bf16(FA[1][a], FB[1][b], T, 0, 0, 0);      \
            T = __builtin_amdgcn_mfma_f32_32x32x16_bf16(FA[1][a], FB[0][b], T, 0, 0, 0);      \
// ... 914 lines not shown
```

mdbn_amd/engine.py:

```python
import ctypes as C
import os as _os
from collections import namedtuple

import numpy
import torch

from . import _lib


def round_up4(n):
    return (int(n) + 3) & ~3


def padded_ld(cols):
    return round_up4(cols)


_default_engine = None


def get_engine():
    global _default_engine
    if _default_engine is None:
        _default_engine = HipEngine()
# ... 1191 lines not shown
        _lib.check(self.lib.mdbn_updown_gen_step_grouped(
            self.ctx, self._stream(), self._p(x_lo), self._p(x_hi), n, C.byref(u), self._p(cost), p, self._p(ws), ws.numel() * 4,
            self._p(groups.tensor), C.c_void_p(groups.host.ctypes.data), groups.n_groups), "mdbn_updown_gen_step_grouped")
        self._w_serial += 1
        self._w_planes_written(G)
        return cost

    def updown_rec_step(self, y_lo, y_hi, r, W, W_speed, hbias, hbias_speed, lr, lambda_1, lambda_2, weightcost, momentum,
                        batch_size, n_rows, path="auto"):
        y_lo = self.as_matrix(y_lo)
        n, V = (int(v) for v in y_lo.shape)
        H, ldh = int(W.shape[1]), W.stride(0)
        if W.shape[0] != V or tuple(y_hi.shape) != (n, H) or tuple(r.shape) != (n, H):
            raise ValueError("y_lo %r, y_hi %r, r %r and W %r do not fit" % (tuple(y_lo.shape), tuple(y_hi.shape), tuple(r.shape), tuple(W.shape)))
        y_hi, r = self._padded(y_hi, n, H, ldh), self._padded(r, n, H, ldh)
        u, ws, p = self._updown_call("rec", n, W, W_speed, hbias, hbias_speed, y_lo.stride(0),
                                     (lr, lambda_1, lambda_2, weightcost, momentum, batch_size, n_rows), 1.0, path)
        _lib.check(self.lib.mdbn_updown_rec_step(self.ctx, self._stream(), self._p(y_lo), self._p(y_hi), self._p(r), n, C.byref(u), p,
                                                 self._p(ws), ws.numel() * 4), "mdbn_updown_rec_step")
        self._w_serial += 1
        self._w_planes_written(W)
        return None

    def round_flip(self, x, flip_col=-1):
        x = self.as_matrix(x)
        out = self.alloc_matrix(x.shape[0], x.shape[1], x.stride(0))
        if x.shape[0]:
            _lib.check(self.lib.mdbn_round_flip(self.ctx, self._stream(), self._p(x), x.shape[0], x.shape[1],
                                                x.stride(0), int(flip_col), self._p(out)), "mdbn_round_flip")
        return out

    def pl_cost(self, fe, fe_flip, n_visible):
        out = torch.zeros(1, dtype=torch.float32, device=self.device)
        _lib.check(self.lib.mdbn_pl_cost(self.ctx, self._stream(), self._p(fe), self._p(fe_flip), fe.numel(),
                                         int(n_visible), self._p(out)), "mdbn_pl_cost")
        return out[0]

    def recon_cost(self, pre, target, gauss):
        pre, target = self.as_matrix(pre), self.as_matrix(target)
        assert pre.shape == target.shape
        out = torch.zeros(1, dtype=torch.float32, device=self.device)
        ws = self.workspace(1, 1, 1)
        _lib.check(self.lib.mdbn_recon_cost(self.ctx, self._stream(), self._p(pre), pre.stride(0), self._p(target),
                                            target.stride(0), pre.shape[0], pre.shape[1], int(bool(gauss)),
                                            self._p(out), self._p(ws), ws.numel() * 4), "mdbn_recon_cost")
        return out[0]

    def tanh_(self, x):
        x = self.as_matrix(x)
        _lib.check(self.lib.mdbn_tanh(self.ctx, self._stream(), self._p(x), x.shape[0], x.shape[1], x.stride(0)),
                   "mdbn_tanh")
        return x

    def count_nonfinite(self, *tensors):
        count = torch.zeros(1, dtype=torch.int32, device=self.device)
        for t in tensors:
            base = t._base if t._base is not None else t
            _lib.check(self.lib.mdbn_count_nonfinite(self.ctx, self._stream(), self._p(base), base.numel(),
                                                     self._p(count)), "mdbn_count_nonfinite")
        return int(count.item())

    def rng_uniform(self, rows, cols, rng, normal=False):
        out = self.alloc_matrix(rows, cols)
        r = rng.c()
        fn = self.lib.mdbn_rng_normal if normal else self.lib.mdbn_rng_uniform
        _lib.check(fn(self.ctx, self._stream(), self._p(out), rows, cols, out.stride(0), C.byref(r)),
                   "mdbn_rng_*")
        return out

    def kernel_timing(self, enable):
        _lib.check(self.lib.mdbn_kernel_timing(self.ctx, int(bool(enable))), "mdbn_kernel_timing")

    def kernel_timing_read(self):
        n, ms = C.c_int64(), C.c_double()
        _lib.check(self.lib.mdbn_kernel_timing_read(self.ctx, C.byref(n), C.byref(ms)),
                   "mdbn_kernel_timing_read")
        return n.value, ms.value

    def narrow_deep_launches(self):
        n = C.c_int64()
        _lib.check(self.lib.mdbn_narrow_deep_launches(self.ctx, C.byref(n)), "mdbn_narrow_deep_launches")
        return n.value

    def kernel_timing_detail(self, cap=8192):
        ms, alg, pipe = (C.c_double * cap)(), (C.c_double * cap)(), (C.c_double * cap)()
        kind, n = (C.c_int32 * cap)(), C.c_int64()
        _lib.check(self.lib.mdbn_kernel_timing_detail(self.ctx, cap, ms, alg, pipe, kind, C.byref(n)),
                   "mdbn_kernel_timing_detail")
        m = min(cap, n.value)
        return [(ms[i], alg[i], pipe[i], kind[i]) for i in range(m)]

    def narrow_bf16(self, src, out=None):
        if out is None or out.numel() != src.numel():
            out = torch.empty(src.numel(), dtype=torch.bfloat16, device=self.device)
        _lib.check(self.lib.mdbn_f32_to_bf16(self.ctx, self._stream(), self._p(src), C.c_void_p(out.data_ptr()), src.numel()),
                   "mdbn_f32_to_bf16")
        return out

    def widen_bf16(self, wire, dst):
        _lib.check(self.lib.mdbn_bf16_to_f32(self.ctx, self._stream(), C.c_void_p(wire.data_ptr()), self._p(dst), dst.numel()),
                   "mdbn_bf16_to_f32")
        return dst

    def cost_values(self, costs):
        out, blocks = [0.0] * len(costs), {}
        for i, c in enumerate(costs):
            base = c._base if getattr(c, "_base", None) is not None else c
            blocks.setdefault(id(base), (base, []))[1].append((i, c.storage_offset() - base.storage_offset()))
        for base, items in blocks.values():
            host = base.detach().reshape(-1).cpu().numpy()
            for i, off in items:
                out[i] = float(host[off])
        return out

    def synchronize(self):
        torch.cuda.synchronize(self.device)
```

Before: 4.013 million samples/s.

## Pre-reduce bias column sums in epilogues to shrink the finalize pass

```diff
diff --git a/include/mdbn_hip.h b/include/mdbn_hip.h
--- a/include/mdbn_hip.h
+++ b/include/mdbn_hip.h
@@ -96,6 +96,9 @@
 int  mdbn_kernel_timing_detail(mdbn_ctx *ctx, int64_t cap, double *ms, double *alg_flop,
                                double *pipe_flop, int32_t *kind, int64_t *n_launches);
 int  mdbn_narrow_deep_launches(mdbn_ctx *ctx, int64_t *n_launches);
+int  mdbn_bias_partial_steps(mdbn_ctx *ctx, int64_t *pair_sum_steps, int64_t *quarter_sum_steps);
+int  mdbn_debug_finalize_units(void *stream, const float *posP, const float *negP, const float *partV, int32_t v_quarters,
+                               int32_t ngroups, int64_t ldh, int64_t ldv, float *s_h, float *s_v);
 
 #define MDBN_MIN_WORKSPACE_BYTES 278528
 int  mdbn_workspace_bytes(int64_t B, int64_t V, int64_t H, int64_t *bytes);
diff --git a/mdbn_amd/_lib.py b/mdbn_amd/_lib.py
--- a/mdbn_amd/_lib.py
+++ b/mdbn_amd/_lib.py
@@ -64,6 +64,8 @@
     "mdbn_kernel_timing": [_vp, _i32],
     "mdbn_kernel_timing_read": [_vp, C.POINTER(_i64), C.POINTER(C.c_double)],
     "mdbn_narrow_deep_launches": [_vp, C.POINTER(_i64)],
+    "mdbn_bias_partial_steps": [_vp, C.POINTER(_i64), C.POINTER(_i64)],
+    "mdbn_debug_finalize_units": [_vp, _vp, _vp, _vp, _i32, _i32, _i64, _i64, _vp, _vp],
     "mdbn_kernel_timing_detail": [_vp, _i64, C.POINTER(C.c_double), C.POINTER(C.c_double),
                                   C.POINTER(C.c_double), C.POINTER(C.c_int32), C.POINTER(_i64)],
     "mdbn_workspace_bytes": [_i64, _i64, _i64, C.POINTER(_i64)],
diff --git a/mdbn_amd/csrc/mdbn_capi.hip b/mdbn_amd/csrc/mdbn_capi.hip
--- a/mdbn_amd/csrc/mdbn_capi.hip
+++ b/mdbn_amd/csrc/mdbn_capi.hip
@@ -132,6 +132,7 @@
 #define g_opt_planes_mfma (t_opt->planes_mfma)
 #define g_opt_early_w (t_opt->early_w)
 #define g_opt_narrow_tiles (t_opt->narrow_tiles)
+#define g_opt_bias_partials (t_opt->bias_partials)
 #define g_opt_slab_tail (t_opt->slab_tail)
 #define g_opt_narrow_deep (t_opt->narrow_deep)
 #define g_opt_feed_copy_streams (t_opt->feed_copy_streams)
@@ -344,6 +345,8 @@
                         [&]() { return g.bal ? launch_gemm_planes_bal(la, lb, g, s) : launch_gemm_planes(la, lb, g, s); });
 }
 
+enum { BIAS_FORM_PAIRS = 1,
+       BIAS_FORM_QUARTERS = 2 };
 struct PlaneStep {
     unsigned short *Xp, *Pp, *hsp, *vsp;
     int64_t px, pp;
@@ -391,8 +394,9 @@
 
 int run_affine_planes(mdbn_ctx* ctx, int comm_cus, const unsigned short* A, int64_t lda, int64_t pa, int ap, int dir,
                       const unsigned short* Wp, int64_t V, int64_t H, int64_t ncols, int64_t rows, EpiArgs e, bool want_cost,
-                      const Workspace& ws, hipStream_t s, int* n_cost_out)
-{
+                      const Workspace& ws, hipStream_t s, int* n_cost_out, int* v_quarters = nullptr)
+{
+    if (v_quarters) *v_quarters = 0;
     const int64_t Kdim = dir == 0 ? V : H, Ndim = dir == 0 ? H : V;
     PlaneGemmArgs g{};
     g.A = A; g.lda = lda; g.pa = pa; g.ap = ap;
@@ -416,6 +420,10 @@
         g.fused = 1; g.ms = 16;
         g.deep = g_opt_narrow_deep && narrow_deep_ok(g, LAY_K, LAY_K);
         if (g.deep) ++ctx->narrow_deep_launches;
+        if (v_quarters && e.colsum && g_opt_bias_partials && quarter_sums_ok(rows)) {
+            e.colsum_q = e.colsum; e.colsum_per = fin_quarter_groups(row_groups(rows));
+            *v_quarters = 1;
+        }
     }
     const bool fuse = !bal && g_opt_fused_epilogue && g.splitk == 1;
     const int nb = fuse ? g.tiles_m * g.tiles_n : epilogue_blocks(rows, e.ld);
@@ -491,8 +499,10 @@
     return MDBN_OK;
 }
 
-int planes_forward(mdbn_ctx* ctx, hipStream_t s, const mdbn_cd_args* a, const Workspace& ws, const PlaneStep& pb, int* n_cost)
-{
+int planes_forward(mdbn_ctx* ctx, hipStream_t s, const mdbn_cd_args* a, const Workspace& ws, const PlaneStep& pb, int* n_cost, int* form)
+{
+    *form = 0;
+    const bool summed = g_opt_bias_partials && a->comm_cus <= 0 && g_opt_comm_cus <= 0 && g_opt_bal_blocks <= 0;
     const int64_t B = a->B, V = a->V, Hlive = a->H, ldv = V, ldh = a->ldh;
     const int64_t H = ldh;
     unsigned short* const Wp = pb.Wp;  const bool keep = pb.keep;
@@ -526,7 +536,10 @@
                     e.target_idx = a->indexes; e.target_idx64 = a->index_is_64;
                 }
             }
-            CHECK(run_affine_planes(ctx, a->comm_cus, pb.hsp, ldh, B * ldh, 1, 1, Wp, V, H, V, B, e, last, ws, s, last ? n_cost : nullptr));
+            int vq = 0;
+            CHECK(run_affine_planes(ctx, a->comm_cus, pb.hsp, ldh, B * ldh, 1, 1, Wp, V, H, V, B, e, last, ws, s, last ? n_cost : nullptr,
+                                    (last && summed) ? &vq : nullptr));
+            if (vq) *form |= BIAS_FORM_QUARTERS;
             if (a->trace_v && !a->gauss)
                 HIP_OK(hipMemcpyAsync(a->trace_v + (int64_t)(t - 1) * B * ldv, a->vs, sizeof(float) * B * ldv,
                                       hipMemcpyDeviceToDevice, s));
@@ -539,6 +552,7 @@
             e.mean_planes = pb.Pp + B * ldh; e.plane_stride = pb.pp;
             e.sample_plane = need_sample ? pb.hsp : nullptr;
             if (last) { e.colsum = ws.colPneg; e.colsum_kind = 0; }
+            if (last && summed) { e.colsum_add = ws.colPpos; *form |= BIAS_FORM_PAIRS; }
             if (a->gauss) CHECK(run_affine_planes(ctx, a->comm_cus, pb.Xp + B * ldv, ldv, pb.px, 3, 0, Wp, V, H, Hlive, B, e, false, ws, s, nullptr));
             else CHECK(run_affine_planes(ctx, a->comm_cus, pb.vsp, ldv, B * ldv, 1, 0, Wp, V, H, Hlive, B, e, false, ws, s, nullptr));
             if (a->trace_h && need_sample)
@@ -549,8 +563,13 @@
 }
 
 int planes_statistics(mdbn_ctx* ctx, hipStream_t s, const mdbn_cd_args* a, const Workspace& ws, const PlaneStep& pb, int n_cost,
-                      const mdbn_update_args* upd, const mdbn_update_args* defer)
-{
+                      int form, const mdbn_update_args* upd, const mdbn_update_args* defer)
+{
+    const float* const finP = (form & BIAS_FORM_PAIRS) ? ws.colPneg : ws.colPpos;
+    const float* const finN = (form & BIAS_FORM_PAIRS) ? nullptr : ws.colPneg;
+    const int finQ = (form & BIAS_FORM_QUARTERS) ? 1 : 0;
+    if (form & BIAS_FORM_PAIRS) ++ctx->bias_pair_steps;
+    if (form & BIAS_FORM_QUARTERS) ++ctx->bias_quarter_steps;
     const int64_t B = a->B, V = a->V, Hlive = a->H, ldv = V, ldh = a->ldh, H = ldh;
     const StatsView st(a->stats, V, ldv, ldh);
     const Plan sp = plan_stats(V, H, 2 * B, ldh, false);
@@ -581,8 +600,8 @@
         fill_bias_upd(bu, *upd, Hlive);
         g.fused = 2;
         g.fin_enabled = 1;
-        g.fin = make_fin_args(ws.colPpos, ws.colPneg, ws.colV, row_groups(B), ldh, ldv, ws.cost_partials, n_cost, st.s_h, st.s_v,
-                              st.cost, &bu);
+        g.fin = make_fin_args(finP, finN, ws.colV, row_groups(B), ldh, ldv, ws.cost_partials, n_cost, st.s_h, st.s_v,
+                              st.cost, &bu, finQ);
         fill_upd(g.upd, *upd, V, ldh, pb.Wp);
         g.upd.early = g_opt_early_w && upd->lambda_1 == 0.f && (upd->weightcost == 0.f || upd->W0 != nullptr) &&
                       2 * B / 32 >= 12 && g_opt_planes_mfma == 16 && !g_opt_bf16_inputs;
@@ -593,11 +612,11 @@
     }
     if (sp.splitk == 1 && g_opt_fused_finalize) {
         g.fin_enabled = 1;
-        g.fin = make_fin_args(ws.colPpos, ws.colPneg, ws.colV, row_groups(B), ldh, ldv, ws.cost_partials, n_cost, st.s_h, st.s_v,
-                              st.cost, nullptr);
+        g.fin = make_fin_args(finP, finN, ws.colV, row_groups(B), ldh, ldv, ws.cost_partials, n_cost, st.s_h, st.s_v,
+                              st.cost, nullptr, finQ);
     } else {
-        HIP_OK(launch_finalize_stats(ws.colPpos, ws.colPneg, ws.colV, row_groups(B), ldh, ldv, ws.cost_partials, n_cost, st.s_h,
-                                     st.s_v, st.cost, nullptr, s));
+        HIP_OK(launch_finalize_stats(finP, finN, ws.colV, row_groups(B), ldh, ldv, ws.cost_partials, n_cost, st.s_h,
+                                     st.s_v, st.cost, nullptr, s, finQ));
     }
     g.fused = 0; g.ldc = ldh; g.slab_stride = V * ldh;
     if (defer) {
@@ -869,6 +888,15 @@
     return MDBN_OK;
 }
 
+static bool set_bias_partials_option(mdbn_ctx* ctx, const char* name, int64_t value)
+{
+    if (strcmp(name, "bias_partials") == 0) {
+        ctx->opt.bias_partials = value != 0;
+        return true;
+    }
+    return false;
+}
+
 static bool set_plane_kernel_option(mdbn_ctx* ctx, const char* name, int64_t value)
 {
     if (strcmp(name, "slab_tail") == 0) {
@@ -883,6 +911,7 @@
     CtxScope ctx_scope(ctx);
     REQUIRE(ctx != nullptr && name != nullptr, "NULL argument");
     if (set_plane_kernel_option(ctx, name, value)) return MDBN_OK;
+    if (set_bias_partials_option(ctx, name, value)) return MDBN_OK;
     if (strcmp(name, "gemm_bk") == 0) {
         REQUIRE(value == 0 || value == 32 || value == 64, "gemm_bk must be 0 (auto), 32 or 64");
         ctx->opt.gemm_bk = (int)value;
@@ -1051,6 +1080,24 @@
 {
     REQUIRE(ctx && n_launches, "NULL argument");
     *n_launches = ctx->narrow_deep_launches;
+    return MDBN_OK;
+}
+
+int mdbn_bias_partial_steps(mdbn_ctx* ctx, int64_t* pair_sum_steps, int64_t* quarter_sum_steps)
+{
+    REQUIRE(ctx && pair_sum_steps && quarter_sum_steps, "NULL argument");
+    *pair_sum_steps = ctx->bias_pair_steps;
+    *quarter_sum_steps = ctx->bias_quarter_steps;
+    return MDBN_OK;
+}
+
+int mdbn_debug_finalize_units(void* stream, const float* posP, const float* negP, const float* partV, int32_t v_quarters,
+                              int32_t ngroups, int64_t ldh, int64_t ldv, float* s_h, float* s_v)
+{
+    REQUIRE(posP && partV && s_h && s_v, "NULL argument");
+    REQUIRE(ngroups > 0 && ldh > 0 && ldv > 0, "bad extents");
+    HIP_OK(launch_finalize_stats(posP, negP, partV, ngroups, ldh, ldv, nullptr, 0, s_h, s_v, nullptr, nullptr, (hipStream_t)stream,
+                                 v_quarters != 0));
     return MDBN_OK;
 }
 
@@ -1712,12 +1759,12 @@
         REQUIRE(aligned16(a->W_planes), "W_planes not 16-byte aligned");
         HIP_OK(launch_split_planes(a->W, V, ldh, reinterpret_cast<unsigned short*>(a->W_planes), V * ldh, s));
     }
-    int n_cost = 0;
+    int n_cost = 0, bias_form = 0;
     if (part == StepPart::Statistics) {
         REQUIRE(ctx->pending_stats == a->stats && ctx->pending_n_cost >= 0, "mdbn_cd_statistics must follow mdbn_cd_forward of the same step");
-        n_cost = ctx->pending_n_cost;
-    }
-    ctx->pending_n_cost = -1; ctx->pending_stats = nullptr;
+        n_cost = ctx->pending_n_cost; bias_form = ctx->pending_bias_form;
+    }
+    ctx->pending_n_cost = -1; ctx->pending_stats = nullptr; ctx->pending_bias_form = 0;
     if (defer) {
         REQUIRE(upd == nullptr && part != StepPart::Forward, "a deferred update goes with the statistics half of a step without its own update");
         REQUIRE(defer->W == a->W && defer->ldh == ldh && defer->ldv == ldv && defer->V == V && defer->H == H,
@@ -1735,20 +1782,21 @@
         switch (path) {
         case StepPath::OneLaunch:  CHECK(small_forward(s, a, ws, &n_cost)); break;
         case StepPath::Thin:       CHECK(thin_forward(s, a, ws, thin, &n_cost)); break;
-        case StepPath::Planes:     CHECK(planes_forward(ctx, s, a, ws, planes, &n_cost)); break;
+        case StepPath::Planes:     CHECK(planes_forward(ctx, s, a, ws, planes, &n_cost, &bias_form)); break;
         case StepPath::GroupChain: CHECK(gchain_forward(ctx, s, a, ws, gg, &n_cost)); break;
         case StepPath::Dense:      CHECK(dense_forward(s, a, ws, &n_cost)); break;
         }
     }
     if (part == StepPart::Forward) {
-        ctx->pending_n_cost = n_cost; ctx->pending_stats = a->stats;
-        return MDBN_OK;
-    }
+        ctx->pending_n_cost = n_cost; ctx->pending_stats = a->stats; ctx->pending_bias_form = bias_form;
+        return MDBN_OK;
+    }
+    REQUIRE(bias_form == 0 || path == StepPath::Planes, "the options changed between mdbn_cd_forward and mdbn_cd_statistics");
     if (defer && path != StepPath::Planes) HIP_OK(launch_whole_update(*defer, s));
     switch (path) {
     case StepPath::OneLaunch:  return small_statistics(s, a, ws, n_cost, upd);
     case StepPath::Thin:       return thin_statistics(s, a, ws, thin, n_cost, upd);
-    case StepPath::Planes:     return planes_statistics(ctx, s, a, ws, planes, n_cost, upd, defer);
+    case StepPath::Planes:     return planes_statistics(ctx, s, a, ws, planes, n_cost, bias_form, upd, defer);
     case StepPath::GroupChain:
     case StepPath::Dense:      break;
     }
diff --git a/mdbn_amd/csrc/mdbn_capi_internal.h b/mdbn_amd/csrc/mdbn_capi_internal.h
--- a/mdbn_amd/csrc/mdbn_capi_internal.h
+++ b/mdbn_amd/csrc/mdbn_capi_internal.h
@@ -35,6 +35,7 @@
     int early_w = 1;
     int narrow_tiles = 1;
     int slab_tail = 1;
+    int bias_partials = 1;
     int narrow_deep = 1;
     int feed_copy_streams = 1;
     int gather_ahead = 1;
@@ -66,6 +67,8 @@
     mdbn::capi::GemmTiming timing;
     int64_t narrow_deep_launches = 0;
     int pending_n_cost = -1;
+    int pending_bias_form = 0;
+    int64_t bias_pair_steps = 0, bias_quarter_steps = 0;
     const void* pending_stats = nullptr;
     void* comm = nullptr;
     int comm_ranks = 0;
diff --git a/mdbn_amd/csrc/mdbn_device.h b/mdbn_amd/csrc/mdbn_device.h
--- a/mdbn_amd/csrc/mdbn_device.h
+++ b/mdbn_amd/csrc/mdbn_device.h
@@ -106,12 +106,25 @@
     if (unit < n_units) {
         const int cl = lane >> 2, qd = lane & 3;
         const int64_t i = (int64_t)unit * 16 + cl;
-        const int per = (f.ngroups + 3) / 4;
-        const int gbeg = qd * per, gend = min(f.ngroups, gbeg + per);
+        const int gbeg = fin_quarter_begin(f.ngroups, qd), gend = fin_quarter_end(f.ngroups, qd);
         float a = 0.f;
 #ifndef MDBN_FIN_BATCH
 #define MDBN_FIN_BATCH 0
 #endif
+#ifndef FIN_PAIR_BATCH
+#define FIN_PAIR_BATCH 16
+#endif
+        if (i < f.ldh && !f.negP) {
+            for (int g0 = gbeg; g0 < gend; g0 += FIN_PAIR_BATCH) {
+                float p[FIN_PAIR_BATCH];
+#pragma unroll
+                for (int u = 0; u < FIN_PAIR_BATCH; ++u) p[u] = f.posP[(int64_t)min(g0 + u, gend - 1) * f.ldh + i];
+#pragma unroll
+                for (int u = 0; u < FIN_PAIR_BATCH; ++u) a += g0 + u < gend ? p[u] : 0.f;
+            }
+        } else if (i >= f.ldh && i < f.ldh + f.ldv && f.v_quarters) {
+            if (gbeg < gend) a = f.partV[(int64_t)qd * f.ldv + (i - f.ldh)];
+        } else
 #if !MDBN_FIN_BATCH
         if (i < f.ldh) {
 #pragma unroll 16
@@ -308,6 +321,7 @@
         philox_rows4(e.rng, e.rng.draw, g0, (uint32_t)col, wa);
         if (need_z) philox_rows4(e.rng, e.rng.draw | MDBN_NORMAL_BIT, g0, (uint32_t)col, wb);
     }
+    const float cadd = (e.colsum && e.colsum_add) ? e.colsum_add[(int64_t)(r0 >> 2) * e.ld + col] : 0.f;
     float csum = 0.f;
 #pragma unroll
     for (int j = 0; j < 4; ++j) {
@@ -346,7 +360,7 @@
             if (live) csum += e.colsum_kind == 0 ? ms : (e.colsum_kind == 1 ? tg - m : tg - sv);
         }
     }
-    if (e.colsum) e.colsum[(int64_t)(r0 >> 2) * e.ld + col] = csum;
+    if (e.colsum) e.colsum[(int64_t)(r0 >> 2) * e.ld + col] = e.colsum_add ? cadd + csum : csum;
 }
 
 template <int MODE = -1>
@@ -391,6 +405,7 @@
     const int cq = threadIdx.x & 15, rg = threadIdx.x >> 4;
     const int col0 = n0 + 4 * cq, r0 = m0 + 4 * rg;
     float cost = 0.f;
+    float4 cs = make_float4(0.f, 0.f, 0.f, 0.f);
     if (r0 < e.rows && col0 < (int)e.ld) {
         float4 tg[4];
         const bool want_tg = e.target != nullptr;
@@ -410,7 +425,6 @@
         }
         constexpr bool need_u = SAMPLE, need_z = SAMPLE && GAUSS;
         float4 ms[4], sv[4], pre[4];
-        float4 cs = make_float4(0.f, 0.f, 0.f, 0.f);
         if (stamps && threadIdx.x == 0) {
             asm volatile("s_waitcnt vmcnt(0) lgkmcnt(0)" ::: "memory");
             stamps[0] = wall_clock64();
@@ -469,10 +483,22 @@
                 *reinterpret_cast<uint2*>(e.sample_plane + off) = w;
             }
         }
-        if (e.colsum) *reinterpret_cast<float4*>(e.colsum + (int64_t)(r0 >> 2) * e.ld + col0) = cs;
+        if (e.colsum && !e.colsum_q) *reinterpret_cast<float4*>(e.colsum + (int64_t)(r0 >> 2) * e.ld + col0) = cs;
         if (stamps && threadIdx.x == 0) {
             asm volatile("s_waitcnt vmcnt(0)" ::: "memory");
             stamps[2] = wall_clock64();
+        }
+    }
+    if (e.colsum_q) {
+        float* Q = T + BM * LDT + 64;
+        const int per = e.colsum_per, nseg = 32 / per;
+        *reinterpret_cast<float4*>(Q + rg * BN + 4 * cq) = cs;
+        __syncthreads();
+        const int seg = threadIdx.x >> 6, c = threadIdx.x & 63;
+        if (seg < nseg && n0 + c < (int)e.ld) {
+            float a = 0.f;
+            for (int g = seg * per; g < seg * per + per; ++g) a += Q[g * BN + c];
+            e.colsum_q[(int64_t)quarter_of_segment(m0 >> 7, seg, per) * e.ld + n0 + c] = a;
         }
     }
     if (e.cost_partials) {
diff --git a/mdbn_amd/csrc/mdbn_kernels.h b/mdbn_amd/csrc/mdbn_kernels.h
--- a/mdbn_amd/csrc/mdbn_kernels.h
+++ b/mdbn_amd/csrc/mdbn_kernels.h
@@ -2,6 +2,7 @@
 #include <hip/hip_runtime.h>
 #include <stdint.h>
 #include "philox.h"
+#include "mdbn_quarters.h"
 #include "../../include/mdbn_hip.h"
 
 namespace mdbn {
@@ -33,6 +34,9 @@
     int64_t plane_stride;
     unsigned short* sample_plane;
     int bal_P, bal_S, bal_tiles_m, bal_tiles_n;
+    const float* colsum_add;
+    float* colsum_q;
+    int colsum_per;
 };
 
 struct UpdEpi {
@@ -65,6 +69,7 @@
 
 struct FinArgs {
     const float* posP; const float* negP; const float* partV;
+    int v_quarters;
     int ngroups;
     int64_t ldh, ldv;
     const float* cost_partials; int n_cost;
@@ -165,6 +170,7 @@
 void set_epilogue_threads(int t);
 inline int row_groups(int64_t B) { return (int)((B + 3) / 4); }
 
+
 hipError_t launch_gemm(int la, int lb, const GemmArgs& g, hipStream_t s);
 hipError_t launch_act_epilogue(const EpiArgs& e, hipStream_t s);
 hipError_t launch_sum_slabs(const float* slabs, int nsplit, int64_t slab_stride, int64_t n,
@@ -177,10 +183,11 @@
 hipError_t launch_colsum_groups(const float* X, const float* Y, int rows, int64_t ld, float* out, hipStream_t s);
 FinArgs make_fin_args(const float* posP, const float* negP, const float* partV, int ngroups, int64_t ldh, int64_t ldv,
                       const float* cost_partials, int n_cost, float* s_h, float* s_v, float* cost,
-                      const BiasUpd* bias_update);
+                      const BiasUpd* bias_update, int v_quarters = 0);
 hipError_t launch_finalize_stats(const float* posP, const float* negP, const float* partV, int ngroups,
                                  int64_t ldh, int64_t ldv, const float* cost_partials, int n_cost,
-                                 float* s_h, float* s_v, float* cost, const BiasUpd* bias_update, hipStream_t s);
+                                 float* s_h, float* s_v, float* cost, const BiasUpd* bias_update, hipStream_t s,
+                                 int v_quarters = 0);
 hipError_t launch_update(const mdbn_update_args& a, hipStream_t s, const float* slabs = nullptr, int nslab = 1,
                          int64_t slab_stride = 0, unsigned short* Wp = nullptr);
 hipError_t launch_free_energy(const float* slabs, int nsplit, int64_t slab_stride, int64_t ldh, int H,
diff --git a/mdbn_amd/csrc/mdbn_kernels.hip b/mdbn_amd/csrc/mdbn_kernels.hip
--- a/mdbn_amd/csrc/mdbn_kernels.hip
+++ b/mdbn_amd/csrc/mdbn_kernels.hip
@@ -970,6 +970,10 @@
 #pragma unroll
             for (int r = 0; r < 4; ++r) VecIO<CW>::load(e.target + srow[r] * e.ld_target + c0, tgt4[r]);
         }
+        float cadd[CW];
+#pragma unroll
+        for (int j = 0; j < CW; ++j) cadd[j] = 0.f;
+        if (e.colsum_add) VecIO<CW>::load(e.colsum_add + (int64_t)rg * e.ld + c0, cadd);
         if (NS > 0) {
             constexpr int RB = NS * CW >= 64 ? 1 : (NS * CW >= 32 ? 2 : 4);
 #pragma unroll
@@ -1088,6 +1092,10 @@
                 }
             }
         }
+        if (e.colsum_add) {
+#pragma unroll
+            for (int j = 0; j < CW; ++j) csum[j] = cadd[j] + csum[j];
+        }
         if (e.colsum) VecIO<CW>::store(e.colsum + (int64_t)rg * e.ld + c0, csum);
     }
     if (e.cost_partials) {
@@ -1264,11 +1272,11 @@
 
 FinArgs make_fin_args(const float* posP, const float* negP, const float* partV, int ngroups, int64_t ldh, int64_t ldv,
                       const float* cost_partials, int n_cost, float* s_h, float* s_v, float* cost,
-                      const BiasUpd* bias_update)
+                      const BiasUpd* bias_update, int v_quarters)
 {
     FinArgs f;
     memset(&f, 0, sizeof f);
-    f.posP = posP; f.negP = negP; f.partV = partV; f.ngroups = ngroups; f.ldh = ldh; f.ldv = ldv;
+    f.posP = posP; f.negP = negP; f.partV = partV; f.v_quarters = v_quarters; f.ngroups = ngroups; f.ldh = ldh; f.ldv = ldv;
     f.cost_partials = cost_partials; f.n_cost = n_cost; f.s_h = s_h; f.s_v = s_v; f.cost = cost;
     if (bias_update) { f.bu = *bias_update; f.do_bias = 1; }
     return f;
@@ -1276,10 +1284,11 @@
 
 hipError_t launch_finalize_stats(const float* posP, const float* negP, const float* partV, int ngroups,
                                  int64_t ldh, int64_t ldv, const float* cost_partials, int n_cost,
-                                 float* s_h, float* s_v, float* cost, const BiasUpd* bias_update, hipStream_t s)
+                                 float* s_h, float* s_v, float* cost, const BiasUpd* bias_update, hipStream_t s,
+                                 int v_quarters)
 {
     const FinArgs f = make_fin_args(posP, negP, partV, ngroups, ldh, ldv, cost_partials, n_cost, s_h, s_v, cost,
-                                    bias_update);
+                                    bias_update, v_quarters);
     const int units = (int)((ldh + ldv + 15) / 16) + 1;
     hipLaunchKernelGGL(finalize_stats_kernel, dim3((units + 3) / 4), dim3(256), 0, s, f);
     return hipGetLastError();
diff --git a/mdbn_amd/csrc/mdbn_planes.hip b/mdbn_amd/csrc/mdbn_planes.hip
--- a/mdbn_amd/csrc/mdbn_planes.hip
+++ b/mdbn_amd/csrc/mdbn_planes.hip
@@ -494,6 +494,11 @@
 #define PL_MAIN_BARRIER() __syncthreads()
 #endif
 #endif
+#ifdef MDBN_STAMP
+#define PL_SPLIT_BARRIER(IT) do { const long long t_ = clock64(); __syncthreads(); ((IT) < 20 ? bar_wait : bar_wait_late) += clock64() - t_; } while (0)
+#else
+#define PL_SPLIT_BARRIER(IT) PL_MAIN_BARRIER()
+#endif
 #define PL_CONSUME_CONSTS() PL_CONSUME_CONSTS_SW(false)
 #define PL_CONSUME_CONSTS_SW(SW)                                                              \
     constexpr bool PL_SWP = (SW);                                                             \
@@ -505,8 +510,8 @@
 __device__ __forceinline__ void pl_consume16(char* smem, int nt, int lane, int wm, int wn, pf32x4a (&acc)[4][2 * NBH],
                                              bool open_barrier = true, long long* bar_wait_out = nullptr)
 {
-    long long bar_wait = 0;
-    (void)bar_wait;
+    long long bar_wait = 0, bar_wait_late = 0;
+    (void)bar_wait; (void)bar_wait_late;
     int offA[4][2], offB[4][2];
     pl_offsets16<LA, LB>(lane, wm, wn, offA, offB);
     PL_CONSUME_CONSTS();
@@ -518,15 +523,15 @@
         {
             const char* base = smem + (it % PL_NSTAGE) * PL_STAGE;
             const char* next = smem + ((it + 1) % PL_NSTAGE) * PL_STAGE;
-            PL_STAGE_EVEN(base, next, PL_MAIN_BARRIER());
+            PL_STAGE_EVEN(base, next, PL_SPLIT_BARRIER(it));
         }
         if (it + 1 < nt) {
             const char* base = smem + ((it + 1) % PL_NSTAGE) * PL_STAGE;
             const char* next = smem + ((it + 2) % PL_NSTAGE) * PL_STAGE;
-            PL_STAGE_ODD(base, next, PL_MAIN_BARRIER());
-        }
-    }
-    if (bar_wait_out) *bar_wait_out = bar_wait;
+            PL_STAGE_ODD(base, next, PL_SPLIT_BARRIER(it + 1));
+        }
+    }
+    if (bar_wait_out) { bar_wait_out[0] = bar_wait; bar_wait_out[1] = bar_wait_late; }
 }
 
 template <int AP>
@@ -654,9 +659,9 @@
                 g.stamps[(int64_t)blockIdx.x * 16 + 13] = clock64();
 #endif
 #ifdef MDBN_STAMP
-            long long bw = 0;
-            if constexpr (KD == 64) pl_consume16_deep<AP>(smem, nt, lane, wm, wn, acc, &bw);
-            else pl_consume16<LA, LB, AP, NBH>(smem, nt, lane, wm, wn, acc, false, &bw);
+            long long bw[2] = {0, 0};
+            if constexpr (KD == 64) pl_consume16_deep<AP>(smem, nt, lane, wm, wn, acc, &bw[0]);
+            else pl_consume16<LA, LB, AP, NBH>(smem, nt, lane, wm, wn, acc, false, bw);
 #else
             if constexpr (KD == 64) pl_consume16_deep<AP>(smem, nt, lane, wm, wn, acc);
             else pl_consume16<LA, LB, AP, NBH>(smem, nt, lane, wm, wn, acc, false);
@@ -665,7 +670,11 @@
 #ifdef MDBN_STAMP
             if (PL_STAMP_COND && g.stamps && wave == 0 && lane == 0) {
                 g.stamps[(int64_t)blockIdx.x * 16 + 14] = clock64();
-                g.stamps[(int64_t)blockIdx.x * 16 + 15] = bw;
+                g.stamps[(int64_t)blockIdx.x * 16 + 15] = bw[0] + bw[1];
+#ifdef MDBN_STAMP_STATS
+                g.stamps[(int64_t)blockIdx.x * 16 + 5] = bw[0];
+                g.stamps[(int64_t)blockIdx.x * 16 + 6] = bw[1];
+#endif
             }
 #endif
             const int c16 = lane & 15, q4 = lane >> 4;
diff --git a/mdbn_amd/csrc/mdbn_quarters.h b/mdbn_amd/csrc/mdbn_quarters.h
--- /dev/null
+++ b/mdbn_amd/csrc/mdbn_quarters.h
@@ -0,0 +1,28 @@
+#pragma once
+#include <stdint.h>
+
+#if defined(__HIPCC__)
+#define MDBN_QHD __host__ __device__
+#else
+#define MDBN_QHD
+#endif
+
+namespace mdbn {
+
+MDBN_QHD inline int fin_quarter_groups(int ngroups) { return (ngroups + 3) / 4; }
+MDBN_QHD inline int fin_quarter_begin(int ngroups, int q) { return q * fin_quarter_groups(ngroups); }
+MDBN_QHD inline int fin_quarter_end(int ngroups, int q)
+{
+    const int e = fin_quarter_begin(ngroups, q) + fin_quarter_groups(ngroups);
+    return e < ngroups ? e : ngroups;
+}
+
+MDBN_QHD inline bool quarter_sums_ok(int64_t rows)
+{
+    if (rows <= 0 || rows % 128 != 0) return false;
+    const int per = fin_quarter_groups((int)(rows / 4));
+    return per <= 32 && 32 % per == 0;
+}
+MDBN_QHD inline int quarter_of_segment(int tile, int seg, int per) { return tile * (32 / per) + seg; }
+
+}
diff --git a/mdbn_amd/engine.py b/mdbn_amd/engine.py
--- a/mdbn_amd/engine.py
+++ b/mdbn_amd/engine.py
@@ -1297,6 +1297,20 @@
         _lib.check(self.lib.mdbn_narrow_deep_launches(self.ctx, C.byref(n)), "mdbn_narrow_deep_launches")
         return n.value
 
+    def bias_partial_steps(self):
+        p, q = C.c_int64(), C.c_int64()
+        _lib.check(self.lib.mdbn_bias_partial_steps(self.ctx, C.byref(p), C.byref(q)), "mdbn_bias_partial_steps")
+        return p.value, q.value
+
+    def debug_finalize_units(self, posP, negP, partV, v_quarters, ngroups, ldh, ldv):
+        import torch
+        s_h = torch.empty(ldh, dtype=torch.float32, device=posP.device)
+        s_v = torch.empty(ldv, dtype=torch.float32, device=posP.device)
+        _lib.check(self.lib.mdbn_debug_finalize_units(self._stream(), self._p(posP), self._p(negP) if negP is not None else None,
+                                                      self._p(partV), int(v_quarters), int(ngroups), int(ldh), int(ldv),
+                                                      self._p(s_h), self._p(s_v)), "mdbn_debug_finalize_units")
+        return s_h, s_v
+
     def kernel_timing_detail(self, cap=8192):
         ms, alg, pipe = (C.c_double * cap)(), (C.c_double * cap)(), (C.c_double * cap)()
         kind, n = (C.c_int32 * cap)(), C.c_int64()
```

After: 3.947 million samples/s. 0.984x the previous value.
